# Agricultural-Robotics-Bonn/pagnerf

Hardware: AMD Instinct MI355X
Metric: rays/sec (train step) on BUP20-shape scene (higher is better)
Workload: dtype bf16

## Files before the change

include/pagnerf_hip.h:

```cpp
#ifndef PAGNERF_HIP_H
#define PAGNERF_HIP_H

#include <stdint.h>

#ifdef __cplusplus
extern "C" {
#endif

#define PAG_ABI_VERSION 14

enum { PAG_F32 = 0, PAG_F16 = 1, PAG_BF16 = 2 };
enum { PAG_OK = 0, PAG_ERR_ARG = -1, PAG_ERR_LAUNCH = -2, PAG_ERR_UNSUPPORTED = -3 };
enum { PAG_ACT_NONE = 0, PAG_ACT_SIGMOID = 1, PAG_ACT_SOFTMAX = 2 };
enum { PAG_MLP_MFMA_BF16 = 0, PAG_MLP_FP32 = 1 };
enum { PAG_BG_BLACK = 0, PAG_BG_WHITE = 1 };
enum { PAG_LAYOUT_STRIDED = 0, PAG_LAYOUT_XCD8 = 1 };
enum { PAG_ENC_HALF_COORDS = 1 };
#define PAG_MAX_LEVELS 32
#define PAG_MAX_FEATS 64

int pag_abi_version(void);
const char *pag_last_error_string(void);


// ... 75 lines not shown
    const float *weights;
    const float *alpha;
    float *out;
    int64_t n_samples;
} pag_head_composite_args;
int pag_mlp_fwd(const pag_mlp_fwd_args *args, int64_t M, void *stream);
int pag_mlp_fwd_pair_supported(const pag_mlp_fwd_args *args, const pag_mlp_fwd_args *pair);
int pag_mlp_fwd_composite_supported(const pag_mlp_fwd_args *args, int64_t M);
int pag_mlp_fwd_producer_supported(const pag_mlp_fwd_args *args, const pag_mlp_fwd_args *producer, int64_t M);

typedef struct pag_mlp_bwd_args {
    const void *grad_out; const void *out; int out_dtype; int out_act;
    int k1; int in_dim; int n_layers; int out_dim;
    int x1_layout; int x1_levels; int x1_feats;
    const float *W[3];
    const void *hidden_save[2];
    void *dz[3];
    void *dx1; int dx1_dtype;
    int mode;
    const float *g_ray; const float *g_scale; const int32_t *g_index;
    const float *softmax_stats; const float *b_last;
    int dx1_accumulate;
    const float *dx1_col0_add;
    const float *dx1_col0_gate;
    const float *g_ray_scale;
    const void *x1; int x1_dtype; const float *x2; int k2p; const int32_t *x2_index;
    float *wgrad_workspace; int64_t wgrad_workspace_bytes;
    float *dW[3]; float *db[3];
    const float *b[3];
    const struct pag_mlp_bwd_args *pair;
    float *dz0_slots;
} pag_mlp_bwd_args;
int pag_mlp_bwd(const pag_mlp_bwd_args *args, int64_t M, void *stream);
int64_t pag_mlp_dz0_slots_bytes(int64_t M, int64_t R);
int pag_mlp_dz0_slots_sum(const int64_t *pack_start, int64_t R, const float *slots, float *out, void *stream);
int pag_mlp_bwd_fused_supported(const pag_mlp_bwd_args *args);
#define PAG_MLP_FUSED_WIDE_MAX_M ((int64_t)1 << 24)
int64_t pag_mlp_bwd_fused_workspace_bytes(const pag_mlp_bwd_args *args, int64_t M);
int pag_mlp_bwd_pair_supported(const pag_mlp_bwd_args *args, const pag_mlp_bwd_args *pair);

int pag_affine_xcd8_fwd(const void *x, int64_t M, int x_levels, int x_feats, const float *W, const float *b, int n_out, int in_dim,
                        float *out, void *stream);
int pag_affine_xcd8_bwd_dx(const float *grad_out, int64_t M, int x_levels, int x_feats, const float *W, int n_out, int in_dim, void *dx,
                           void *stream);

int pag_head_composite_fwd(const int64_t *pack_start, const int32_t *ray_of_pack, int64_t P,
                           const void *hidden, const float *W_last, const float *b_last, int out_dim,
                           const float *softmax_stats, const float *weights, const float *alpha,
                           float *out, int64_t n_samples, void *stream);

int pag_mlp_wgrad_blocks(int64_t M);
int pag_mlp_wgrad(const void *dz, int dz_cols, int n_out, const void *a1, int a1_dtype,
                  int a1_layout, int k1, const float *a2, int k2p, const int32_t *a2_index, int n_in,
                  float *slabs, int n_blocks, int64_t M, void *stream);

int pag_mlp_wgrad_finish(const float *slabs, int n_blocks, int n_out, int n_in, int a1_layout,
                         int a1_levels, int a1_feats, float *dW, float *db, void *stream);

typedef struct pag_wgrad_layer {
    const void *dz;
    int dz_cols, n_out;
    const void *a1;
    int a1_dtype, a1_layout, k1;
    const float *a2;
    int k2p;
    const int32_t *a2_index;
// ... 399 lines not shown
```

pagnerf_amd/_lib.py:

```python
import ctypes
import os

import torch

from . import build as _build

F32, F16, BF16 = 0, 1, 2
I32, I64 = 3, 4
ACT_NONE, ACT_SIGMOID, ACT_SOFTMAX = 0, 1, 2
MLP_MFMA_BF16, MLP_FP32 = 0, 1
BG_BLACK, BG_WHITE = 0, 1
LAYOUT_STRIDED, LAYOUT_XCD8 = 0, 1
ENC_HALF_COORDS = 1
ABI_VERSION = 14
MLP_FUSED_WIDE_MAX_M = 1 << 24

_DT = {torch.float32: F32, torch.float16: F16, torch.bfloat16: BF16}

c_i64, c_i32, c_u32, c_f32, c_vp = ctypes.c_int64, ctypes.c_int, ctypes.c_uint32, ctypes.c_float, ctypes.c_void_p
c_fp = ctypes.POINTER(ctypes.c_float)
c_ip = ctypes.POINTER(ctypes.c_int)


class HeadCompositeArgs(ctypes.Structure):
# ... 16 lines not shown
                ("softmax_stats", c_vp), ("x1_col0_relu", c_vp), ("pair", ctypes.POINTER(MlpFwdArgs)),
                ("composite", ctypes.POINTER(HeadCompositeArgs)), ("x1_producer", ctypes.POINTER(MlpFwdArgs))]


class WgradLayer(ctypes.Structure):
    _fields_ = [("dz", c_vp), ("dz_cols", c_i32), ("n_out", c_i32),
                ("a1", c_vp), ("a1_dtype", c_i32), ("a1_layout", c_i32), ("k1", c_i32),
                ("a2", c_vp), ("k2p", c_i32), ("a2_index", c_vp), ("n_in", c_i32),
                ("slabs", c_vp), ("n_blocks", c_i32), ("a1_levels", c_i32), ("a1_feats", c_i32),
                ("dW", c_vp), ("db", c_vp)]


class MlpBwdArgs(ctypes.Structure):
    pass


MlpBwdArgs._fields_ = [("grad_out", c_vp), ("out", c_vp), ("out_dtype", c_i32), ("out_act", c_i32),
                ("k1", c_i32), ("in_dim", c_i32), ("n_layers", c_i32), ("out_dim", c_i32),
                ("x1_layout", c_i32), ("x1_levels", c_i32), ("x1_feats", c_i32),
                ("W", c_vp * 3),
                ("hidden_save", c_vp * 2),
                ("dz", c_vp * 3),
                ("dx1", c_vp), ("dx1_dtype", c_i32),
                ("mode", c_i32),
                ("g_ray", c_vp), ("g_scale", c_vp), ("g_index", c_vp),
                ("softmax_stats", c_vp), ("b_last", c_vp), ("dx1_accumulate", c_i32), ("dx1_col0_add", c_vp),
                ("dx1_col0_gate", c_vp), ("g_ray_scale", c_vp),
                ("x1", c_vp), ("x1_dtype", c_i32), ("x2", c_vp), ("k2p", c_i32), ("x2_index", c_vp),
                ("wgrad_workspace", c_vp), ("wgrad_workspace_bytes", c_i64),
                ("dW", c_vp * 3), ("db", c_vp * 3), ("b", c_vp * 3),
                ("pair", ctypes.POINTER(MlpBwdArgs)), ("dz0_slots", c_vp)]


class DeepMlpArgs(ctypes.Structure):
    _fields_ = [("coords", c_vp), ("ray_d", c_vp), ("hidden", c_i32), ("num_classes", c_i32), ("channels", c_i32), ("save", c_i32),
                ("W", c_vp * 14), ("b", c_vp * 14), ("density", c_vp), ("rgb", c_vp), ("semantics", c_vp),
                ("workspace", c_vp), ("workspace_bytes", c_i64),
                ("g_density", c_vp), ("g_rgb", c_vp), ("g_semantics", c_vp), ("dW", c_vp * 14), ("db", c_vp * 14),
                ("bwd_workspace", c_vp), ("bwd_workspace_bytes", c_i64)]


MLP128_MAX_M = 1 << 26
MLP128_BATCH, MLP128_MAX_GRID = 256, 256


class Mlp128FwdArgs(ctypes.Structure):
    _fields_ = [("x1", c_vp), ("x1_dtype", c_i32), ("k1", c_i32), ("x1_layout", c_i32), ("x1_levels", c_i32), ("x1_feats", c_i32),
                ("x2", c_vp), ("k2p", c_i32), ("x2_index", c_vp),
                ("in_dim", c_i32), ("n_hidden", c_i32), ("hidden", c_i32), ("out_dim", c_i32),
                ("W", c_vp * 4), ("b", c_vp * 4), ("out_act", c_i32), ("out", c_vp), ("out_dtype", c_i32),
                ("workspace", c_vp), ("workspace_bytes", c_i64)]


class Mlp128BwdArgs(ctypes.Structure):
    _fields_ = [("grad_out", c_vp), ("out", c_vp), ("out_dtype", c_i32), ("out_act", c_i32),
                ("k1", c_i32), ("k2p", c_i32), ("in_dim", c_i32), ("n_hidden", c_i32), ("hidden", c_i32), ("out_dim", c_i32),
                ("x1_layout", c_i32), ("x1_levels", c_i32), ("x1_feats", c_i32),
                ("W", c_vp * 4), ("workspace", c_vp), ("workspace_bytes", c_i64), ("bwd_workspace", c_vp), ("bwd_workspace_bytes", c_i64),
                ("dx1", c_vp), ("dx1_dtype", c_i32), ("dx1_accumulate", c_i32), ("dW", c_vp * 4), ("db", c_vp * 4)]


class VmArgs(ctypes.Structure):
    _fields_ = [("density_plane", c_vp * 3), ("density_line", c_vp * 3), ("app_plane", c_vp * 3), ("app_line", c_vp * 3), ("basis", c_vp),
                ("density_n_comp", c_i32), ("app_n_comp", c_i32), ("app_dim", c_i32), ("res", c_i32),
                ("xyz", c_vp), ("sigma", c_vp), ("app", c_vp), ("g_sigma", c_vp), ("g_app", c_vp),
                ("g_density_plane", c_vp * 3), ("g_density_line", c_vp * 3), ("g_app_plane", c_vp * 3), ("g_app_line", c_vp * 3), ("g_basis", c_vp),
# ... 18 lines not shown
    _fields_ = [("verts", c_vp), ("part_vert_begin", c_vp), ("point_begin", c_vp), ("part_key_begin", c_vp), ("part_key_count", c_vp), ("keys", c_vp),
                ("ann_part_begin", c_vp), ("ann_label", c_vp), ("ann_cover", c_vp), ("cand", c_vp), ("frame_ann_begin", c_vp), ("frame_labelled", c_vp),
                ("n_verts", c_i32), ("n_parts", c_i32), ("n_anns", c_i32), ("n_cand", c_i32), ("B", c_i32), ("max_part_keys", c_i32)]


class Bup20PrepareArgs(ctypes.Structure):
    _fields_ = [("img", c_vp), ("depth", c_vp), ("sem", c_vp), ("inst", c_vp), ("sem_conf", c_vp), ("inst_conf", c_vp), ("counts", c_vp),
                ("B", c_i32), ("H0", c_i32), ("W0", c_i32), ("C0", c_i32), ("mip", c_i32), ("bg", c_i32), ("n_ids", c_i32),
                ("view_offset", c_i64), ("V", c_i64), ("imgs", c_vp), ("masks", c_vp), ("depths", c_vp), ("semantics_pred", c_vp),
                ("instance_pred", c_vp), ("sem_conf_out", c_vp), ("inst_conf_out", c_vp)]


COCO_MAX_PART_KEYS = 4096

VIS_PICTURES, VIS_LABELS, VIS_MAX_ID = 15, 6, 1023


class VisArgs(ctypes.Structure):
    _fields_ = [("H", c_i32), ("W", c_i32), ("rgb", c_vp), ("rgb_is_u8", c_i32), ("rgb_stride", c_i32), ("gt", c_vp), ("gt_stride", c_i32), ("phase", c_i32),
                ("depth", c_vp), ("labels", c_vp * VIS_LABELS), ("label_bytes", c_i32 * VIS_LABELS), ("conf", c_vp * 2), ("table", c_vp),
                ("max_id", c_i32), ("box_width", c_i32), ("blend_keep", c_f32), ("blend_alpha", c_f32), ("overlay_keep", c_f32), ("overlay_alpha", c_f32),
                ("conf_min", c_f32), ("conf_max", c_f32), ("workspace", c_vp), ("workspace_bytes", c_i64), ("out", c_vp * VIS_PICTURES)]


_SIGS = {
    "pag_abi_version": (c_i32, []),
    "pag_last_error_string": (ctypes.c_char_p, []),
    "pag_encode_bwd_workspace_bytes": (c_i64, [c_i64, c_i32, c_i32, c_i32, c_i64]),
    "pag_mlp_fwd": (c_i32, [ctypes.POINTER(MlpFwdArgs), c_i64, c_vp]),
    "pag_mlp_fwd_pair_supported": (c_i32, [ctypes.POINTER(MlpFwdArgs), ctypes.POINTER(MlpFwdArgs)]),
    "pag_mlp_fwd_composite_supported": (c_i32, [ctypes.POINTER(MlpFwdArgs), c_i64]),
    "pag_mlp_fwd_producer_supported": (c_i32, [ctypes.POINTER(MlpFwdArgs), ctypes.POINTER(MlpFwdArgs), c_i64]),
    "pag_mlp_bwd": (c_i32, [ctypes.POINTER(MlpBwdArgs), c_i64, c_vp]),
    "pag_mlp_bwd_fused_supported": (c_i32, [ctypes.POINTER(MlpBwdArgs)]),
    "pag_mlp_bwd_fused_workspace_bytes": (c_i64, [ctypes.POINTER(MlpBwdArgs), c_i64]),
    "pag_mlp_bwd_pair_supported": (c_i32, [ctypes.POINTER(MlpBwdArgs), ctypes.POINTER(MlpBwdArgs)]),
    "pag_head_composite_fwd": (c_i32, [c_vp, c_vp, c_i64, c_vp, c_vp, c_vp, c_i32, c_vp, c_vp, c_vp, c_vp, c_i64, c_vp]),
    "pag_mlp_wgrad_blocks": (c_i32, [c_i64]),
    "pag_mlp_wgrad_batch": (c_i32, [ctypes.POINTER(WgradLayer), c_i32, c_i64, c_vp]),
    "pag_mlp_wgrad_finish": (c_i32, [c_vp, c_i32, c_i32, c_i32, c_i32, c_i32, c_i32, c_vp, c_vp, c_vp]),
    "pag_mlp_wgrad": (c_i32, [c_vp, c_i32, c_i32, c_vp, c_i32, c_i32, c_i32, c_vp, c_i32, c_vp, c_i32, c_vp, c_i32, c_i64, c_vp]),
    "pag_raymarch_count": (c_i32, [c_vp, c_vp, c_i64, c_i32, c_vp, c_vp, c_f32, c_f32, c_vp, c_i32, c_vp, c_vp]),
    "pag_pack_offsets": (c_i32, [c_vp, c_i64, c_vp, c_vp, c_vp]),
    "pag_pad_packed": (c_i32, [c_vp, c_i64, c_i64, c_i32, c_vp, c_vp, c_vp, c_vp, c_vp, c_vp, c_vp, c_vp, c_vp, c_vp]),
    "pag_view_embed": (c_i32, [c_vp, c_i64, c_i32, c_i32, c_vp, c_vp]),
    "pag_raymarch_pack": (c_i32, [c_vp, c_vp, c_i64, c_i32, c_vp, c_vp, c_f32, c_f32, c_vp, c_i32, c_vp, c_vp, c_vp, c_vp, c_vp, c_vp, c_vp, c_vp, c_vp]),
    "pag_raymarch_voxel_count": (c_i32, [c_vp, c_vp, c_i64, c_i32, c_f32, c_f32, c_vp, c_vp, c_i32, c_f32, c_vp, c_vp]),
    "pag_raymarch_voxel_pack": (c_i32, [c_vp, c_vp, c_i64, c_i32, c_f32, c_f32, c_vp, c_vp, c_i32, c_f32, c_vp, c_vp, c_vp, c_vp, c_vp, c_vp, c_vp,
                                        c_vp, c_vp, c_vp]),
    "pag_raymarch_voxel_nugget_capacity": (c_i64, [c_i32]),
    "pag_raymarch_voxel_count_nuggets": (c_i32, [c_vp, c_vp, c_i64, c_i32, c_f32, c_f32, c_vp, c_vp, c_i32, c_f32, c_vp, c_vp, c_vp, c_vp]),
    "pag_raymarch_voxel_pack_nuggets": (c_i32, [c_vp, c_vp, c_i64, c_i32, c_vp, c_vp, c_vp, c_i32, c_vp, c_vp, c_vp, c_vp, c_vp, c_vp, c_vp, c_vp, c_vp]),
    "pag_ray_sample_grad": (c_i32, [c_vp, c_vp, c_i64, c_vp, c_vp, c_vp, c_vp]),
    "pag_affine_xcd8_fwd": (c_i32, [c_vp, c_i64, c_i32, c_i32, c_vp, c_vp, c_i32, c_i32, c_vp, c_vp]),
    "pag_affine_xcd8_bwd_dx": (c_i32, [c_vp, c_i64, c_i32, c_i32, c_vp, c_i32, c_i32, c_vp, c_vp]),
    "pag_occupancy_coarse_bytes": (c_i64, [c_i32]),
    "pag_occupancy_coarse": (c_i32, [c_vp, c_i32, c_vp, c_vp]),
    "pag_occupancy_update": (c_i32, [c_vp, c_i64, c_vp, c_vp, c_i64, c_f32, c_f32, c_vp]),
    "pag_label_sums": (c_i32, [c_vp, c_i32, c_i64, c_i64, c_i32, c_i32, c_vp, c_vp, c_vp, c_i32, c_vp, c_vp, c_vp]),
    "pag_assign_cost": (c_i32, [c_vp, c_i32, c_i64, c_i64, c_i64, c_i32, c_i32, c_vp, c_i32, c_vp, c_vp, c_vp, c_vp, c_vp, c_vp, ctypes.c_float, ctypes.c_float, c_i32,
                                c_vp, c_vp, c_vp, c_vp]),
    "pag_sparse_rows_mask": (c_i32, [c_vp, c_i32, c_i64, c_i32, c_vp, c_vp]),
    "pag_sparse_rows_plan": (c_i32, [c_vp, c_i32, c_i64, c_vp, c_vp, c_vp, c_vp]),
    "pag_sparse_rows_pack": (c_i32, [c_vp, c_i32, c_i64, c_i32, c_vp, c_vp, c_vp, c_vp, c_vp, c_vp]),
    "pag_sparse_rows_unpack": (c_i32, [c_vp, c_i32, c_i64, c_i32, c_vp, c_vp, c_vp, c_vp, c_vp, c_vp]),
    "pag_assign_solve": (c_i32, [c_vp, c_i32, c_i32, c_i32, c_vp, c_vp, c_vp, c_vp, c_vp]),
# ... 163 lines not shown
```

pagnerf_amd/build.py:

```python
import concurrent.futures
import hashlib
import os
import subprocess
import sys

HERE = os.path.dirname(os.path.abspath(__file__))
CSRC = os.path.join(HERE, "csrc")
LIBDIR = os.path.join(HERE, "lib")
LIB = os.path.join(LIBDIR, "libpagnerf_hip.so")
ARCH = "gfx950"

COMMON = ["--offload-arch=" + ARCH, "-O3", "-fPIC", "-std=c++17", "-munsafe-fp-atomics", "-Wno-unused-value"]
MLP = ["-mllvm", "-amdgpu-mfma-vgpr-form=1"]
SOURCES = {
    "mlp.hip": MLP,
    "mlp_deep.hip": MLP,
    "mlp_h128.hip": MLP,
    "encode.hip": ["-ffp-contract=off"],
    "mlp_wgrad.hip": MLP,
    "render.hip": ["-ffp-contract=off"],
    "mlp_affine.hip": MLP,
    "api.cpp": ["-x", "hip"],
    "assign.hip": ["-ffp-contract=off"],
    "loss.hip": ["-ffp-contract=off"],
    "optim.hip": ["-ffp-contract=off"],
    "pose.hip": ["-ffp-contract=off"],
    "regularizer.hip": ["-ffp-contract=off"],
    "supcon.hip": ["-ffp-contract=off"],
    "cluster.hip": ["-ffp-contract=off"],
    "panoptic.hip": ["-ffp-contract=off"],
    "map.hip": ["-ffp-contract=off"],
    "voxelmap.hip": ["-ffp-contract=off"],
    "vm.hip": ["-ffp-contract=off"],
    "triplanar.hip": ["-ffp-contract=off"],
    "sparse.hip": [],
    "sample.hip": [],
    "visualize.hip": ["-ffp-contract=off"],
    "prepare.hip": ["-ffp-contract=off"],
    "bup20.hip": ["-ffp-contract=off"],
}


def _jobs():
    n = min(16, os.cpu_count() or 4)
    try:
        n = min(n, int(os.environ.get("MAX_JOBS", "")))
    except ValueError:
        pass
    return max(1, n)


def _hipcc():
    for c in (os.environ.get("HIPCC"), "/opt/rocm/bin/hipcc", "hipcc"):
        if c and (os.path.isabs(c) and os.path.exists(c) or not os.path.isabs(c)):
# ... 68 lines not shown
```

pagnerf_amd/csrc/mlp.hip:

```cpp
#include "mlp_common.h"
#include "mlp_lds.h"

namespace {

struct FwdParams {
    const void *x1;
    const float *x2;
    const int32_t *x2_index;
    int k1, k2p, in_dim, in_pad, out_dim, act;
    const float *W[3];
    const float *b[3];
    void *out;
    void *hsave[2];
    int64_t M;
    int grp_L, grp_F;
    float *stats;
    float *col0_relu;
    const float *W2[2];
    const float *b2[2];
    void *out2;
    int out2_dim;
};

struct BwdParams {
    const void *grad_out;
    const float *g_ray;
    const float *g_scale;
    const float *g_ray_scale;
    const int32_t *g_index;
    const void *out;
    int k1, in_dim, in_pad, out_dim, act;
    const float *W[3];
    const void *hsave[2];
    void *dz[3];
    void *dx1;
    int64_t M;
    int grp_L, grp_F;
    const float *stats;
    const float *b_last;
    int dx1_acc;
    const float *dx_col0;
    const float *dx_col0_gate;
    const void *x1;
    const float *x2;
    const int32_t *x2_index;
    int k2p;
    float *slabs[3];
    const float *b[3];
    float *dz0_slots;
};

constexpr int STAGE_BATCH = 8;
__device__ void stage_weight(bf16_t *dst, int stride, int rows_pad, int cols_pad, const float *W, int n_out, int n_in,
                             bool permute, int grp_L = 0, int grp_F = 0) {
    const int total = rows_pad * cols_pad, step = (int)blockDim.x, last = n_out * n_in - 1;
    for (int e0 = threadIdx.x; e0 < total; e0 += STAGE_BATCH * step) {
        float v[STAGE_BATCH];
        int at[STAGE_BATCH];
#pragma unroll
        for (int k = 0; k < STAGE_BATCH; ++k) {
            const int e = e0 + k * step;
            const int o = udiv_uniform(e, cols_pad), a = e - o * cols_pad;
            const int col = grp_L ? grp_col(a, grp_L, grp_F) : a;
            const bool ok = e < total && o < n_out && col >= 0 && col < n_in;
            at[k] = e < total ? o * stride + (permute ? swap23(a) : a) : -1;
            v[k] = W[min(max(o * n_in + col, 0), last)];
            v[k] = ok ? v[k] : 0.0f;
        }
#pragma unroll
        for (int k = 0; k < STAGE_BATCH; ++k)
            if (at[k] >= 0) dst[at[k]] = (bf16_t)v[k];
    }
}
__device__ void stage_weight_t(bf16_t *dst, int stride, int rows_pad, int cols_pad, const float *W, int n_out, int n_in,
                               int grp_L = 0, int grp_F = 0) {
    const int total = rows_pad * cols_pad, step = (int)blockDim.x, last = n_out * n_in - 1;
    for (int e0 = threadIdx.x; e0 < total; e0 += STAGE_BATCH * step) {
        float v[STAGE_BATCH];
        int at[STAGE_BATCH];
#pragma unroll
        for (int k = 0; k < STAGE_BATCH; ++k) {
            const int e = e0 + k * step;
// ... 4 lines not shown
            v[k] = W[min(max(o * n_in + col, 0), last)];
            v[k] = ok ? v[k] : 0.0f;
        }
#pragma unroll
        for (int k = 0; k < STAGE_BATCH; ++k)
            if (at[k] >= 0) dst[at[k]] = (bf16_t)v[k];
    }
}

__device__ void stage_weight_both(bf16_t *dst_s, int stride_s, bool permute_s, bf16_t *dst_t, int stride_t, int out_pad, int in_pad, const float *W,
                                  int n_out, int n_in, int grp_L = 0, int grp_F = 0) {
    const int total = out_pad * in_pad, step = (int)blockDim.x, last = n_out * n_in - 1;
    for (int e0 = threadIdx.x; e0 < total; e0 += STAGE_BATCH * step) {
        float v[STAGE_BATCH];
        int as[STAGE_BATCH], at[STAGE_BATCH];
#pragma unroll
        for (int k = 0; k < STAGE_BATCH; ++k) {
            const int e = e0 + k * step;
            const int o = udiv_uniform(e, in_pad), a = e - o * in_pad;
            const int col = grp_L ? grp_col(a, grp_L, grp_F) : a;
            const bool ok = e < total && o < n_out && col >= 0 && col < n_in;
            as[k] = e < total ? o * stride_s + (permute_s ? swap23(a) : a) : -1;
            at[k] = a * stride_t + swap23(o);
            v[k] = W[min(max(o * n_in + col, 0), last)];
            v[k] = ok ? v[k] : 0.0f;
        }
#pragma unroll
        for (int k = 0; k < STAGE_BATCH; ++k)
            if (as[k] >= 0) {
                dst_s[as[k]] = (bf16_t)v[k];
                dst_t[at[k]] = (bf16_t)v[k];
            }
    }
}

__device__ __forceinline__ void pack_block(const f32x16 &acc, bf16x8 &lo, bf16x8 &hi) {
#pragma unroll
    for (int j = 0; j < 8; ++j) {
        lo[j] = (bf16_t)acc[j];
        hi[j] = (bf16_t)acc[8 + j];
    }
}

template <typename T>
__device__ __forceinline__ void store_block_full(T *row_ptr, int ch_base, int h, const f32x16 &acc);

template <typename T>
__device__ __forceinline__ void store_block(T *row_ptr, int ch_base, int h, const f32x16 &acc, int n_valid, bool vec_ok) {
    if (vec_ok && ch_base + 32 <= n_valid) {
        store_block_full(row_ptr, ch_base, h, acc);
    } else if (vec_ok) {
#pragma unroll
        for (int g = 0; g < 4; ++g) {
            const int c0 = ch_base + 8 * g + 4 * h;
            if (c0 < n_valid) {
                if constexpr (sizeof(T) == 4) {
                    f32x4 v = {acc[4 * g], acc[4 * g + 1], acc[4 * g + 2], acc[4 * g + 3]};
                    *reinterpret_cast<f32x4 *>(row_ptr + c0) = v;
                } else {
                    bf16x4 v = {(bf16_t)acc[4 * g], (bf16_t)acc[4 * g + 1], (bf16_t)acc[4 * g + 2], (bf16_t)acc[4 * g + 3]};
                    *reinterpret_cast<bf16x4 *>(row_ptr + c0) = v;
                }
            }
        }
    } else {
#pragma unroll
// ... 674 lines not shown
        } else {
            float mx = -INFINITY;
#pragma unroll
            for (int j = 0; j < 4; ++j)
                if (4 * h + j < p.out_dim) mx = fmaxf(mx, o[j]);
            mx = fmaxf(mx, __shfl_xor(mx, 32));
            const float mxs = mx * LOG2E;
            float e[4], sum = 0.0f;
#pragma unroll
            for (int j = 0; j < 4; ++j) {
                e[j] = (4 * h + j < p.out_dim) ? __builtin_amdgcn_exp2f(fmaf(o[j], LOG2E, -mxs)) : 0.0f;
                sum += e[j];
            }
            sum += __shfl_xor(sum, 32);
            const float inv = 1.0f / sum;
#pragma unroll
            for (int j = 0; j < 4; ++j) {
                const bf16_t y = (bf16_t)(e[j] * inv);
                __builtin_amdgcn_raw_buffer_store_b16(__builtin_bit_cast(unsigned short, y), rs_out, ooff[j] + obase, 0, 0);
            }
        }
    }
}

constexpr int CD_WAVES = 2;
__global__ __launch_bounds__(256, CD_WAVES) void mlp_fwd_density_colour(FwdParams pd, FwdParams pc) {
    extern __shared__ __attribute__((aligned(16))) unsigned char smem[];
    constexpr float LOG2E = 1.4426950408889634f;
    constexpr DensityColourLds L{};
    bf16_t *W0d = lds_at<bf16_t>(smem, L.W0d), *WLd = lds_at<bf16_t>(smem, L.WLd);
    bf16_t *W0c = lds_at<bf16_t>(smem, L.W0c), *W1c = lds_at<bf16_t>(smem, L.W1c), *WLc = lds_at<bf16_t>(smem, L.WLc);
    float *b0d = lds_at<float>(smem, L.b0d), *bLd = lds_at<float>(smem, L.bLd);
    float *b0c = lds_at<float>(smem, L.b0c), *b1c = lds_at<float>(smem, L.b1c), *bLc = lds_at<float>(smem, L.bLc);
    stage_weight(W0d, RS, 64, 64, pd.W[0], HID, pd.in_dim, false, pd.grp_L, pd.grp_F);
    stage_weight(WLd, RS, 32, 64, pd.W[1], pd.out_dim, HID, true);
    stage_weight(W0c, RS, 64, 64, pc.W[0], HID, pc.in_dim, false);
    stage_weight(W1c, RS, 64, 64, pc.W[1], HID, HID, true);
    stage_weight(WLc, RS, 32, 64, pc.W[2], pc.out_dim, HID, true);
    for (int e = threadIdx.x; e < 64; e += blockDim.x) {
        b0d[e] = pd.b[0][e];
        b0c[e] = pc.b[0][e];
        b1c[e] = pc.b[1][e];
    }
    for (int e = threadIdx.x; e < 32; e += blockDim.x) {
        bLd[e] = e < pd.out_dim ? pd.b[1][e] : 0.0f;
        bLc[e] = e < pc.out_dim ? pc.b[2][e] : 0.0f;
    }
    __syncthreads();

    const int lane = threadIdx.x & 63, wave = threadIdx.x >> 6;
    const int r = lane & 31, h = lane >> 5;
    const int64_t M = pd.M, ntiles = (M + 31) / 32;
    const int64_t tile_step = (int64_t)gridDim.x * 4;
    const auto rs_x = __builtin_amdgcn_make_buffer_rsrc(const_cast<void *>(pd.x1), 0, (int)(M * 128), 0x00020000);
    const auto rs_xi = __builtin_amdgcn_make_buffer_rsrc(const_cast<int32_t *>(pc.x2_index), 0, (int)(M * 4), 0x00020000);
    const auto rs_od = __builtin_amdgcn_make_buffer_rsrc(pd.out, 0, (int)(M * pd.out_dim * 2), 0x00020000);
    const auto rs_oc = __builtin_amdgcn_make_buffer_rsrc(pc.out, 0, (int)(M * pc.out_dim * 4), 0x00020000);
    const auto rs_c0 = __builtin_amdgcn_make_buffer_rsrc(pc.col0_relu, 0, (int)(M * 4), 0x00020000);
    unsigned xoff[4], ooff_d[4], ooff_c[4];
#pragma unroll
    for (int s = 0; s < 4; ++s) xoff[s] = (unsigned)(((int64_t)(2 * s + h) * M + r) * 16);
#pragma unroll
    for (int g = 0; g < 4; ++g) {
        ooff_d[g] = (8 * g + 4 * h < pd.out_dim) ? (unsigned)((r * pd.out_dim + 8 * g + 4 * h) * 2) : BUF_OOB;
        ooff_c[g] = (4 * h + g < pc.out_dim) ? (unsigned)((r * pc.out_dim + 4 * h + g) * 4) : BUF_OOB;
    }
    const unsigned c0off = h == 0 ? (unsigned)(r * 4) : BUF_OOB;
    auto row_live = [&](int64_t tile) __attribute__((always_inline)) { return tile * 32 + r < M; };
    auto load_x = [&](int64_t tile, int ray, bf16x8 (&xf)[4], bf16x8 (&pe)[2]) __attribute__((always_inline)) {
        const unsigned base = row_live(tile) ? (unsigned)(tile * 32) * 16u : BUF_OOB;
#pragma unroll
// ... 24 lines not shown
        hidden_layer_pinned<4>(W0d, b0d, xb, r, h, acc);
        relu_pack(acc, hb);
        out_block_pinned(WLd, bLd, 0, hb, r, h, o);
        typedef bf16_t bf16x2 __attribute__((ext_vector_type(2)));
        unsigned dw[8];
#pragma unroll
        for (int k = 0; k < 8; ++k) dw[k] = __builtin_bit_cast(unsigned, bf16x2{(bf16_t)o[2 * k], (bf16_t)o[2 * k + 1]});
        const unsigned obase_d = live ? row0 * (unsigned)(pd.out_dim * 2) : BUF_OOB_ROW;
#pragma unroll
        for (int g = 0; g < 4; ++g) __builtin_amdgcn_raw_buffer_store_b64(u32x2{dw[2 * g], dw[2 * g + 1]}, rs_od, ooff_d[g] + obase_d, 0, 0);
        {
            const auto s02 = __builtin_amdgcn_permlane32_swap(dw[0], dw[2], false, false);
            const auto s13 = __builtin_amdgcn_permlane32_swap(dw[1], dw[3], false, false);
            const u32x4 v = {s02[0], s13[0], s02[1], s13[1]};
            xc[0] = __builtin_bit_cast(bf16x8, v);
        }
        __builtin_amdgcn_raw_buffer_store_b32(__builtin_bit_cast(unsigned, fmaxf((float)xc[0][0], 0.0f)), rs_c0, live ? c0off + row0 * 4 : BUF_OOB, 0, 0);
        hidden_layer_pinned<3>(W0c, b0c, xc, r, h, acc);
        relu_pack(acc, hb);
        hidden_layer_pinned<4>(W1c, b1c, hb, r, h, acc);
        relu_pack(acc, hb);
        out_block_pinned(WLc, bLc, 0, hb, r, h, o);
        const unsigned obase_c = live ? row0 * (unsigned)(pc.out_dim * 4) : BUF_OOB_ROW;
#pragma unroll
        for (int j = 0; j < 4; ++j) {
            const float y = __builtin_amdgcn_rcpf(1.0f + __builtin_amdgcn_exp2f(-LOG2E * o[j]));
            __builtin_amdgcn_raw_buffer_store_b32(__builtin_bit_cast(unsigned, y), rs_oc, ooff_c[j] + obase_c, 0, 0);
        }
    }
}

constexpr int WIDE_FWD_PAIR_THREADS = 1024;
constexpr int wide_fwd_waves(bool pair) { return (pair ? WIDE_FWD_PAIR_THREADS : 256) / 64; }
template <bool SAVE0, bool PAIR>
__global__ __launch_bounds__(PAIR ? WIDE_FWD_PAIR_THREADS : 256, PAIR ? 1 : 2) void mlp_fwd_wide_stats(FwdParams p) {
    extern __shared__ __attribute__((aligned(16))) unsigned char smem[];
    constexpr int OB = 7;
    constexpr float LOG2E = 1.4426950408889634f;
    const int NW = blockDim.x >> 6;
    constexpr FwdLds L(3, OB, wide_fwd_waves(PAIR), PAIR);
    bf16_t *W0s = lds_at<bf16_t>(smem, L.W0), *W1s = lds_at<bf16_t>(smem, L.W1);
    bf16_t *WLs = lds_at<bf16_t>(smem, L.WL);
    bf16_t *W0s2 = lds_at<bf16_t>(smem, L.W0p), *WLs2 = lds_at<bf16_t>(smem, L.WLp);
    float *b0s = lds_at<float>(smem, L.b0), *b1s = lds_at<float>(smem, L.b1), *bLs = lds_at<float>(smem, L.bL);
    float *b0s2 = lds_at<float>(smem, L.b0p), *bLs2 = lds_at<float>(smem, L.bLp);
    bf16_t *stg = lds_at<bf16_t>(smem, L.stg) + (threadIdx.x >> 6) * (L.stg_stride / 2);
    stage_weight(W0s, RS, 64, 64, p.W[0], HID, p.in_dim, false, p.grp_L, p.grp_F);
    stage_weight(W1s, RS, 64, 64, p.W[1], HID, HID, true);
    stage_weight(WLs, RS, OB * 32, 64, p.W[2], p.out_dim, HID, true);
    if constexpr (PAIR) {
        stage_weight(W0s2, RS, 64, 64, p.W2[0], HID, p.in_dim, false, p.grp_L, p.grp_F);
        stage_weight(WLs2, RS, 32, 64, p.W2[1], p.out2_dim, HID, true);
        for (int e = threadIdx.x; e < 64; e += blockDim.x) b0s2[e] = p.b2[0][e];
        for (int e = threadIdx.x; e < 32; e += blockDim.x) bLs2[e] = e < p.out2_dim ? p.b2[1][e] : 0.0f;
    }
    for (int e = threadIdx.x; e < 64; e += blockDim.x) {
        b0s[e] = p.b[0][e];
        b1s[e] = p.b[1][e];
    }
    for (int e = threadIdx.x; e < OB * 32; e += blockDim.x) bLs[e] = e < p.out_dim ? p.b[2][e] : -1e30f;
    __syncthreads();

    const int lane = threadIdx.x & 63, wave = threadIdx.x >> 6;
    const int r = lane & 31, h = lane >> 5;
    const int64_t M = p.M, ntiles = (M + 31) / 32;
    const int64_t tile_step = (int64_t)gridDim.x * NW;
    const auto rs_x1 = __builtin_amdgcn_make_buffer_rsrc(const_cast<void *>(p.x1), 0, (int)(M * 128), 0x00020000);
    const auto rs_st = __builtin_amdgcn_make_buffer_rsrc(p.stats, 0, (int)(M * 8), 0x00020000);
    const auto rs_o2 = __builtin_amdgcn_make_buffer_rsrc(PAIR ? p.out2 : nullptr, 0, (int)(M * (PAIR ? p.out2_dim : 0) * 2), 0x00020000);
    unsigned ooff2[4];
#pragma unroll
    for (int j = 0; j < 4; ++j) ooff2[j] = (PAIR && 4 * h + j < p.out2_dim) ? (unsigned)((r * p.out2_dim + 4 * h + j) * 2) : BUF_OOB;
    const auto rs_h0 = __builtin_amdgcn_make_buffer_rsrc(SAVE0 ? p.hsave[0] : nullptr, 0, (int)(M * HID * 2), 0x00020000);
    const auto rs_h1 = __builtin_amdgcn_make_buffer_rsrc(p.hsave[1], 0, (int)(M * HID * 2), 0x00020000);
    unsigned xoff[4];
#pragma unroll
    for (int s = 0; s < 4; ++s) xoff[s] = (unsigned)(((int64_t)(2 * s + h) * M + r) * 16);
    const unsigned soff = h == 0 ? (unsigned)(r * 8) : BUF_OOB;
    auto row_live = [&](int64_t tile) __attribute__((always_inline)) { return tile * 32 + r < M; };
    auto load_x = [&](int64_t tile, bf16x8 (&xf)[4]) __attribute__((always_inline)) {
        const unsigned base = row_live(tile) ? (unsigned)(tile * 32) * 16u : BUF_OOB;
#pragma unroll
        for (int s = 0; s < 4; ++s) xf[s] = __builtin_bit_cast(bf16x8, __builtin_amdgcn_raw_buffer_load_b128(rs_x1, xoff[s] + base, 0, 0));
    };
    int64_t tile = (int64_t)blockIdx.x * NW + wave;
// ... 392 lines not shown
                        if (p.dx_col0 && mb == 0 && h == 0 && (!p.dx_col0_gate || p.dx_col0_gate[m] > 0.0f)) acc[0][0] += p.dx_col0[m];
                        store_block(dx + m * p.k1, 32 * mb, h, acc[mb], p.k1, true);
                    }
                    if (live && p.grp_L) {
                        bf16_t *dg = reinterpret_cast<bf16_t *>(p.dx1);
#pragma unroll
                        for (int g = 0; g < 4; ++g) {
                            bf16x4 *dst = reinterpret_cast<bf16x4 *>(dg + ((int64_t)(4 * mb + g) * p.M + m) * 8 + 4 * h);
                            if (p.dx1_acc) {
#pragma unroll
                                for (int j = 0; j < 4; ++j) acc[mb][4 * g + j] += (float)oldx[mb][g][j];
                            }
                            bf16x4 v = {(bf16_t)acc[mb][4 * g], (bf16_t)acc[mb][4 * g + 1], (bf16_t)acc[mb][4 * g + 2], (bf16_t)acc[mb][4 * g + 3]};
                            *dst = v;
                        }
                    }
                }
            }
        }
    }
}

constexpr int FUSED_WAVES = 1;
template <int NL, int KIND, bool DXACC, int OBL = 1 , int DZ0 = 0 >
__global__ __launch_bounds__(256, FUSED_WAVES) void mlp_bwd_fused(BwdParams p) {
    static_assert(OBL == 1 || KIND == 0, "a 64-wide output layer exists for the dense-gradient form only");
    constexpr bool GRP = KIND != 1;
    extern __shared__ __attribute__((aligned(16))) unsigned char smem[];
    constexpr FusedLds L(NL, OBL, DZ0);
    constexpr int RSL = L.rsl;
    bf16_t *WLt = lds_at<bf16_t>(smem, L.WLt);
    bf16_t *W1t = lds_at<bf16_t>(smem, L.W1t);
    bf16_t *W0t = lds_at<bf16_t>(smem, L.W0t);
    stage_weight_t(WLt, RSL, 64, OBL * 32, p.W[NL - 1], p.out_dim, HID);
    bf16_t *W0s = lds_at<bf16_t>(smem, L.W0s);
    bf16_t *W1s = lds_at<bf16_t>(smem, L.W1s);
    float *b0s = lds_at<float>(smem, L.b0), *b1s = lds_at<float>(smem, L.b1);
    stage_weight_both(W0s, RS, false, W0t, RS, 64, 64, p.W[0], HID, p.in_dim, p.grp_L, p.grp_F);
    if (NL == 3) stage_weight_both(W1s, RS, true, W1t, RS, 64, 64, p.W[1], HID, HID);
    for (int e = threadIdx.x; e < 64; e += blockDim.x) {
        b0s[e] = p.b[0][e];
        b1s[e] = NL == 3 ? p.b[1][e] : 0.0f;
    }
    const int wtile = (threadIdx.x >> 6) * L.tile_stride;
    bf16_t *Tx = lds_at<bf16_t>(smem, L.Tx + wtile), *Th0 = lds_at<bf16_t>(smem, L.Th0 + wtile), *Th1 = lds_at<bf16_t>(smem, L.Th1 + wtile), *Tz = lds_at<bf16_t>(smem, L.Tz + wtile);
    __syncthreads();

    const int lane = threadIdx.x & 63, wave = threadIdx.x >> 6;
    const int r = lane & 31, h = lane >> 5;
    const int64_t M = p.M, ntiles = (M + 31) / 32, nfull = M / 32;
    const int64_t tile_step = (int64_t)gridDim.x * 4;
    const bf16_t *x1b = reinterpret_cast<const bf16_t *>(p.x1);
    const int32_t *ridx = KIND == 1 ? p.x2_index : p.g_index;
    const auto rs_dz0 = __builtin_amdgcn_make_buffer_rsrc(DZ0 == 1 ? p.dz[0] : nullptr, 0, (int)(DZ0 == 1 ? M * HID * 2 : 0), 0x00020000);
    auto store_dz0 = [&](int64_t tile) __attribute__((always_inline)) {
        if constexpr (DZ0 == 1) {
            typedef unsigned int u32x2 __attribute__((ext_vector_type(2)));
            typedef unsigned int u32x4 __attribute__((ext_vector_type(4)));
            const unsigned voff = (unsigned)(tile * (32 * HID * 2)) + (unsigned)((lane >> 3) * (HID * 2) + (lane & 7) * 16);
#pragma unroll
            for (int k = 0; k < 4; ++k) {
                const int rowl = k * 8 + (lane >> 3), ch = (lane & 7) * 2;
                const u32x2 lo = *reinterpret_cast<const u32x2 *>(Tz + tw_off(rowl, ch));
                const u32x2 hi = *reinterpret_cast<const u32x2 *>(Tz + tw_off(rowl, ch + 1));
                __builtin_amdgcn_raw_buffer_store_b128(u32x4{lo[0], lo[1], hi[0], hi[1]}, rs_dz0, voff + k * (8 * HID * 2), 0, 0);
            }
        }
    };

    int *lray_s = lds_at<int>(smem, L.rays) + (threadIdx.x >> 6) * (L.rays_stride / 4), *rid_s = lray_s + 32;
    int ray_c = 0;
    unsigned heads_c = 0u;
// ... 349 lines not shown
        for (int q4 = 0; q4 < 4; ++q4) sv[q4] = (reinterpret_cast<const f32x4 *>(red) + (bb * 4 + q4) * 64 + lane)[0];
        auto srcv = [&](int q) __attribute__((always_inline)) { return sv[q >> 2][q & 3]; };
        if constexpr (bb < BM) {
            float *sl = p.slabs[NL - 1] + (int64_t)blockIdx.x * (OBL * 32) * WG_SLAB_COLS;
#pragma unroll
            for (int q = 0; q < 16; ++q) sl[(32 * (bb >> 1) + rho(q, h)) * WG_SLAB_COLS + 32 * (bb & 1) + r] = srcv(q);
        } else if constexpr (bb < B0) {
            float *sl = p.slabs[1] + (int64_t)blockIdx.x * 64 * WG_SLAB_COLS;
#pragma unroll
            for (int q = 0; q < 16; ++q) sl[(32 * ((bb - BM) >> 1) + rho(q, h)) * WG_SLAB_COLS + 32 * ((bb - BM) & 1) + r] = srcv(q);
        } else if constexpr (bb < NBLK - 1) {
            constexpr int ob = (bb - B0) >> 1, ib = (bb - B0) & 1;
            float *sl = p.slabs[0] + (int64_t)blockIdx.x * 64 * WG_SLAB_COLS;
#pragma unroll
            for (int q = 0; q < 16; ++q) {
                const float v = srcv(q);
                sl[(32 * ob + rho(q, h)) * WG_SLAB_COLS + 32 * ib + r] = v;
                if (ib == 1 && r == 31) sl[(32 * ob + rho(q, h)) * WG_SLAB_COLS + 64] = v;
            }
        } else {
#pragma unroll
            for (int q = 0; q < 16; ++q) {
                const float v = srcv(q);
                if (r < OBL) p.slabs[NL - 1][((int64_t)blockIdx.x * (OBL * 32) + 32 * r + rho(q, h)) * WG_SLAB_COLS + 64] = v;
                if (NL == 3 && r >= OBL && r < OBL + 2) p.slabs[1][((int64_t)blockIdx.x * 64 + 32 * (r - OBL) + rho(q, h)) * WG_SLAB_COLS + 64] = v;
            }
        }
    });
}

struct PairParams {
    BwdParams i, s;
};
__global__ __launch_bounds__(256, 1) void mlp_bwd_pair(PairParams pp) {
    const BwdParams &pi = pp.i, &ps = pp.s;
    extern __shared__ __attribute__((aligned(16))) unsigned char smem[];
    constexpr PairLds L{};
    constexpr int RSLI = L.rslI, RSLS = L.rslS;
    bf16_t *WLtI = lds_at<bf16_t>(smem, L.WLtI);
    bf16_t *W0tI = lds_at<bf16_t>(smem, L.W0tI);
    bf16_t *W0sI = lds_at<bf16_t>(smem, L.W0sI);
    bf16_t *WLtS = lds_at<bf16_t>(smem, L.WLtS);
    bf16_t *W0tS = lds_at<bf16_t>(smem, L.W0tS), *W0sS = lds_at<bf16_t>(smem, L.W0sS);
    float *b0I = lds_at<float>(smem, L.b0I), *b0S = lds_at<float>(smem, L.b0S);
    stage_weight_t(WLtI, RSLI, 64, 64, pi.W[1], pi.out_dim, HID);
    stage_weight_both(W0sI, RS, false, W0tI, RS, 64, 64, pi.W[0], HID, pi.in_dim, pi.grp_L, pi.grp_F);
    stage_weight_t(WLtS, RSLS, 64, 32, ps.W[1], ps.out_dim, HID);
    stage_weight_both(W0sS, RS, false, W0tS, RS, 64, 64, ps.W[0], HID, ps.in_dim, ps.grp_L, ps.grp_F);
    for (int e = threadIdx.x; e < 64; e += blockDim.x) {
        b0I[e] = pi.b[0][e];
        b0S[e] = ps.b[0][e];
    }
    const int wtile = (threadIdx.x >> 6) * L.tile_stride;
    bf16_t *Tx = lds_at<bf16_t>(smem, L.Tx + wtile), *ThI = lds_at<bf16_t>(smem, L.ThI + wtile), *ThS = lds_at<bf16_t>(smem, L.ThS + wtile), *Tz = lds_at<bf16_t>(smem, L.Tz + wtile);
    __syncthreads();

    const int lane = threadIdx.x & 63, wave = threadIdx.x >> 6;
    const int r = lane & 31, h = lane >> 5;
    const int64_t M = pi.M, ntiles = (M + 31) / 32, nfull = M / 32;
    const int64_t tile_step = (int64_t)gridDim.x * 4;
    const bf16_t *x1b = reinterpret_cast<const bf16_t *>(pi.x1);
    const int32_t *ridx = ps.g_index;

    bf16x8 xn[4];
    bf16x4 gz[2][4];
    float gs[4], gy[4], gsc = 0.0f;
    int ray1 = 0, ray2 = 0;
    auto row_of = [&](int64_t tile) __attribute__((always_inline)) { return min(min(tile, ntiles - 1) * 32 + r, M - 1); };
    auto prefetch = [&](int64_t tile_raw, int ray) __attribute__((always_inline)) {
        const int64_t tile = min(tile_raw, ntiles - 1);
        const int64_t m = min(tile * 32 + r, M - 1);
#pragma unroll
        for (int s = 0; s < 4; ++s) xn[s] = load8(x1b + ((int64_t)(2 * s + h) * M + m) * 8);
        const bf16_t *gop = reinterpret_cast<const bf16_t *>(pi.grad_out) + m * HID;
#pragma unroll
        for (int ob = 0; ob < 2; ++ob)
#pragma unroll
            for (int g = 0; g < 4; ++g) gz[ob][g] = *reinterpret_cast<const bf16x4 *>(gop + 32 * ob + 8 * g + 4 * h);
        gsc = __fmul_rn(ps.g_scale[m], ps.g_ray_scale[ray]);
        const float *grow = ps.g_ray + (int64_t)ray * ps.out_dim;
        const bf16_t *yop = reinterpret_cast<const bf16_t *>(ps.out) + m * ps.out_dim;
// ... 246 lines not shown
            float *sl = (S ? ps.slabs[0] : pi.slabs[0]) + (int64_t)blockIdx.x * 64 * WG_SLAB_COLS;
#pragma unroll
            for (int q = 0; q < 16; ++q) {
                const float v = srcv(q);
                sl[(32 * ob + rho(q, h)) * WG_SLAB_COLS + 32 * ib + r] = v;
                if (ib == 1 && r == 31) sl[(32 * ob + rho(q, h)) * WG_SLAB_COLS + 64] = v;
            }
        } else {
#pragma unroll
            for (int q = 0; q < 16; ++q) {
                const float v = srcv(q);
                if (r < 2) pi.slabs[1][((int64_t)blockIdx.x * 64 + 32 * r + rho(q, h)) * WG_SLAB_COLS + 64] = v;
                if (r == 2) ps.slabs[1][((int64_t)blockIdx.x * 32 + rho(q, h)) * WG_SLAB_COLS + 64] = v;
            }
        }
    });
}

template <int OB>
__global__ __launch_bounds__((OB + 1) * 64) void mlp_bwd_wide_blocks(BwdParams p) {
    extern __shared__ __attribute__((aligned(16))) unsigned char smem[];
    constexpr WideBlocksLds L(OB);
    constexpr int RSL = L.rsl;
    constexpr float LOG2E = 1.4426950408889634f;
    bf16_t *WLt = lds_at<bf16_t>(smem, L.WLt);
    bf16_t *WLs = lds_at<bf16_t>(smem, L.WLs);
    float *bLs = lds_at<float>(smem, L.bL);
    bf16_t *Th = lds_at<bf16_t>(smem, L.Th);
    bf16_t *Tp = lds_at<bf16_t>(smem, L.Tp);
    bf16_t *TzAll = lds_at<bf16_t>(smem, L.Tz);
    float *grow = lds_at<float>(smem, L.grow);
    float *dotbuf = lds_at<float>(smem, L.dot);
    bf16x8 *zbuf = lds_at<bf16x8>(smem, L.zbuf);
    stage_weight_both(WLs, RS, true, WLt, RSL, OB * 32, 64, p.W[0], p.out_dim, HID);
    for (int e = threadIdx.x; e < OB * 32; e += blockDim.x) bLs[e] = e < p.out_dim ? p.b_last[e] : -1e30f;
    for (int e = threadIdx.x; e < 2 * OB * 64; e += blockDim.x) dotbuf[e] = 0.0f;
    for (int e = threadIdx.x; e < 2 * OB * 2 * 64 * 4; e += blockDim.x) reinterpret_cast<float *>(zbuf)[e] = 0.0f;
    for (int e = threadIdx.x; e < 4 * TW_ELEMS / 2; e += blockDim.x) reinterpret_cast<float *>(Th)[e] = 0.0f;
    __syncthreads();

    const int lane = threadIdx.x & 63, wave = threadIdx.x >> 6;
    const int r = lane & 31, h = lane >> 5;
    const int64_t M = p.M, ntiles = (M + 31) / 32;
    const int64_t tile_step = gridDim.x;
    const bf16_t *hsrc = reinterpret_cast<const bf16_t *>(p.hsave[0]);
    bf16_t *dzh = reinterpret_cast<bf16_t *>(p.dz[0]);
    const bool is_block = wave < OB;
    const int ob = is_block ? wave : 0;
    bf16_t *Tz = TzAll + ob * (L.Tz_stride / 2);
    auto row_of = [&](int64_t tile) __attribute__((always_inline)) { return min(min(tile, ntiles - 1) * 32 + r, M - 1); };
    const auto rs_h = __builtin_amdgcn_make_buffer_rsrc(const_cast<bf16_t *>(hsrc), 0, (int)min(M * HID * 2, (int64_t)0xffffffffll), 0x00020000);
    const auto rs_i = __builtin_amdgcn_make_buffer_rsrc(const_cast<int32_t *>(p.g_index), 0, (int)min(M * 4, (int64_t)0xffffffffll), 0x00020000);
    const auto rs_d = __builtin_amdgcn_make_buffer_rsrc(dzh, 0, (int)min((ntiles + 1) * 32 * HID * 2, (int64_t)0xffffffffll), 0x00020000);
    const int voff_tile = (lane >> 3) * (HID * 2) + (lane & 7) * 16;
    auto load_rows = [&](float (&v)[4 * WB_RMAX], int ray_first, int ray_last) __attribute__((always_inline)) {
#pragma unroll
        for (int k = 0; k < WB_RMAX; ++k) {
            const int rr = min(ray_first + k, ray_last);
            const auto rs_row = __builtin_amdgcn_make_buffer_rsrc(const_cast<float *>(p.g_ray) + (int64_t)rr * p.out_dim, 0, p.out_dim * 4, 0x00020000);
#pragma unroll
            for (int j = 0; j < 4; ++j) v[4 * k + j] = __builtin_bit_cast(float, __builtin_amdgcn_raw_buffer_load_b32(rs_row, lane * 4, 256 * j, 0));
        }
    };
    auto put_rows = [&](float *dst, const float (&v)[4 * WB_RMAX]) __attribute__((always_inline)) {
#pragma unroll
        for (int k = 0; k < 4 * WB_RMAX; ++k) dst[(k >> 2) * WR_RS + 64 * (k & 3) + lane] = v[k];
    };
// ... 586 lines not shown
            if (ob < OB) {
                float v[16];
#pragma unroll
                for (int q = 0; q < 16; ++q) v[q] = acc[ob][q];
                PAG_DPP_ADD16(v, "row_shr:1 row_mask:0xf bank_mask:0xf bound_ctrl:1");
                PAG_DPP_ADD16(v, "row_shr:2 row_mask:0xf bank_mask:0xf bound_ctrl:1");
                PAG_DPP_ADD16(v, "row_shr:4 row_mask:0xf bank_mask:0xf bound_ctrl:1");
                PAG_DPP_ADD16(v, "row_shr:8 row_mask:0xf bank_mask:0xf bound_ctrl:1");
                PAG_DPP_ADD16(v, "row_bcast:15 row_mask:0xa bank_mask:0xf");
                if (r == 31) {
#pragma unroll
                    for (int q = 0; q < 16; ++q) red[wave * OB * 32 + 32 * ob + rho(q, h)] = v[q];
                }
            }
        }
        const int32_t ray = p.ray_of_pack[pk];
        const float al = p.alpha[ray];
        if (pw) {
            for (int c = lane; c < p.out_dim; c += 64) p.out[(int64_t)ray * p.out_dim + c] = al * red[wave * OB * 32 + c];
        } else {
            __syncthreads();
            for (int c = threadIdx.x; c < p.out_dim; c += blockDim.x)
                p.out[(int64_t)ray * p.out_dim + c] = al * (red[c] + red[OB * 32 + c] + red[2 * OB * 32 + c] + red[3 * OB * 32 + c]);
            __syncthreads();
        }
    }
}

template <bool PAIR>
__global__ __launch_bounds__(256, 1) void head_fwd_once_kernel(FwdParams p, HeadCompParams c) {
    extern __shared__ __attribute__((aligned(16))) unsigned char smem[];
    constexpr int OB = 7;
    constexpr float LOG2E = 1.4426950408889634f;
    constexpr FwdLds L(3, OB, 4, PAIR, true);
    bf16_t *W0s = lds_at<bf16_t>(smem, L.W0), *W1s = lds_at<bf16_t>(smem, L.W1);
    bf16_t *WLs = lds_at<bf16_t>(smem, L.WL);
    bf16_t *W0s2 = lds_at<bf16_t>(smem, L.W0p), *WLs2 = lds_at<bf16_t>(smem, L.WLp);
    float *b0s = lds_at<float>(smem, L.b0), *b1s = lds_at<float>(smem, L.b1), *bLs = lds_at<float>(smem, L.bL);
    float *b0s2 = lds_at<float>(smem, L.b0p), *bLs2 = lds_at<float>(smem, L.bLp);
    float *red = lds_at<float>(smem, L.red);
    bf16_t *stg = lds_at<bf16_t>(smem, L.stg) + (threadIdx.x >> 6) * (L.stg_stride / 2);
    stage_weight(W0s, RS, 64, 64, p.W[0], HID, p.in_dim, false, p.grp_L, p.grp_F);
    stage_weight(W1s, RS, 64, 64, p.W[1], HID, HID, true);
    stage_weight(WLs, RS, OB * 32, 64, p.W[2], p.out_dim, HID, true);
    if constexpr (PAIR) {
        stage_weight(W0s2, RS, 64, 64, p.W2[0], HID, p.in_dim, false, p.grp_L, p.grp_F);
        stage_weight(WLs2, RS, 32, 64, p.W2[1], p.out2_dim, HID, true);
        for (int e = threadIdx.x; e < 64; e += blockDim.x) b0s2[e] = p.b2[0][e];
        for (int e = threadIdx.x; e < 32; e += blockDim.x) bLs2[e] = e < p.out2_dim ? p.b2[1][e] : 0.0f;
    }
    for (int e = threadIdx.x; e < 64; e += blockDim.x) {
        b0s[e] = p.b[0][e];
        b1s[e] = p.b[1][e];
    }
    for (int e = threadIdx.x; e < OB * 32; e += blockDim.x) bLs[e] = e < p.out_dim ? p.b[2][e] : -1e30f;
    __syncthreads();

    const int lane = threadIdx.x & 63, wave = threadIdx.x >> 6;
    int r = lane & 31, h = lane >> 5;
    const int64_t M = p.M;
    const auto rs_x1 = __builtin_amdgcn_make_buffer_rsrc(const_cast<void *>(p.x1), 0, (int)(M * 128), 0x00020000);
    const auto rs_st = __builtin_amdgcn_make_buffer_rsrc(p.stats, 0, (int)(M * 8), 0x00020000);
    const auto rs_o2 = __builtin_amdgcn_make_buffer_rsrc(PAIR ? p.out2 : nullptr, 0, (int)(M * (PAIR ? p.out2_dim : 0) * 2), 0x00020000);
    const auto rs_h1 = __builtin_amdgcn_make_buffer_rsrc(p.hsave[1], 0, (int)(M * HID * 2), 0x00020000);
    const int pw = c.per_wave;
    const int64_t pk0 = pw ? (int64_t)blockIdx.x * 4 + wave : (int64_t)blockIdx.x, pk_step = pw ? (int64_t)gridDim.x * 4 : (int64_t)gridDim.x;
    const int t_first = pw ? 0 : wave, t_step = pw ? 1 : 4;
    bf16x8 xn[4];
    float wn = 0.0f;
    const auto rs_w = __builtin_amdgcn_make_buffer_rsrc(const_cast<float *>(c.weights), 0, (int)(M * 4), 0x00020000);
    unsigned xoff[4];
#pragma unroll
    for (int s = 0; s < 4; ++s) xoff[s] = (unsigned)(((int64_t)(2 * s + h) * M + r) * 16);
    auto fetch = [&](int64_t fbeg, int64_t fend, int64_t t) __attribute__((always_inline)) {
        const int64_t base = fbeg + 32 * t;
        const bool lv = base + r < fend;
        const unsigned off = lv ? (unsigned)base * 16u : BUF_OOB;
#pragma unroll
        for (int s = 0; s < 4; ++s) xn[s] = __builtin_bit_cast(bf16x8, __builtin_amdgcn_raw_buffer_load_b128(rs_x1, xoff[s] + off, 0, 0));
        wn = __builtin_bit_cast(float, __builtin_amdgcn_raw_buffer_load_b32(rs_w, lv ? (unsigned)(base + r) * 4u : BUF_OOB, 0, 0));
// ... 275 lines not shown
            }
        }
        __syncthreads();
        if (l > 0) {
            const float *hv = reinterpret_cast<const float *>(p.hsave[l - 1]) + mc * HID;
#pragma unroll
            for (int k = 0; k < 64; ++k) {
                float v = (live && hv[k] > 0.0f) ? acc[k] : 0.0f;
                zs[k * PT + t] = v;
                if (live) reinterpret_cast<float *>(p.dz[l - 1])[m * HID + k] = v;
            }
            n_out = HID;
        } else if (live) {
            DxT *dx = reinterpret_cast<DxT *>(p.dx1) + m * p.k1;
#pragma unroll
            for (int k = 0; k < 64; ++k)
                if (k < p.k1) pag_st(dx + k, acc[k]);
        }
    }
}

inline unsigned mlp_grid(int64_t M) {
    int64_t tiles = (M + 31) / 32;
    int64_t blocks = (tiles + 3) / 4;
    int64_t cap = 256 * 6;
    return (unsigned)(blocks < cap ? (blocks > 0 ? blocks : 1) : cap);
}

bool is_wide_stats_head(const pag_mlp_fwd_args *a) {
    return a->mode == PAG_MLP_MFMA_BF16 && a->x1_dtype == PAG_BF16 && a->x1_layout == PAG_LAYOUT_XCD8 && !a->out && a->n_layers == 3 && a->softmax_stats &&
           a->out_act == PAG_ACT_SOFTMAX && a->out_dim > 192 && a->out_dim <= 224 && a->hidden_save[1];
}

void set_pair_head(FwdParams &p, const pag_mlp_fwd_args *b) {
    p.W2[0] = b->W[0];
    p.W2[1] = b->W[1];
    p.b2[0] = b->b[0];
    p.b2[1] = b->b[1];
    p.out2 = b->out;
    p.out2_dim = b->out_dim;
}

template <typename X1T, typename OutT, int NL>
void launch_fwd_mfma_nl(const FwdParams &p, hipStream_t st) {
    const dim3 grid(mlp_grid(p.M)), block(256);
    const int OB = (p.out_dim + 31) / 32;
    const size_t lds = FwdLds(NL, OB).bytes;
    if (OB <= 1) hipLaunchKernelGGL((mlp_fwd_mfma<X1T, OutT, NL, 1>), grid, block, lds, st, p);
    else if (OB <= 2) hipLaunchKernelGGL((mlp_fwd_mfma<X1T, OutT, NL, 2>), grid, block, lds, st, p);
    else if (OB <= 4) hipLaunchKernelGGL((mlp_fwd_mfma<X1T, OutT, NL, 4>), grid, block, lds, st, p);
    else hipLaunchKernelGGL((mlp_fwd_mfma<X1T, OutT, NL, 7>), grid, block, lds, st, p);
}
template <typename X1T, typename OutT>
void launch_fwd_mfma(const FwdParams &p, int n_layers, hipStream_t st) {
    if (n_layers == 2) launch_fwd_mfma_nl<X1T, OutT, 2>(p, st);
    else launch_fwd_mfma_nl<X1T, OutT, 3>(p, st);
}

constexpr int FAST_FWD_GRID_CAP = 768;
template <int KIND>
void launch_fwd_fast(const FwdParams &p, int n_layers, bool save, hipStream_t st) {
    const dim3 grid(std::min<unsigned>(mlp_grid(p.M), FAST_FWD_GRID_CAP)), block(256);
    const size_t lds = FwdLds(n_layers, 1).bytes;
    if (n_layers == 2 && save) hipLaunchKernelGGL((mlp_fwd_fast<2, KIND, true>), grid, block, lds, st, p);
    else if (n_layers == 2) hipLaunchKernelGGL((mlp_fwd_fast<2, KIND, false>), grid, block, lds, st, p);
    else if (save) hipLaunchKernelGGL((mlp_fwd_fast<3, KIND, true>), grid, block, lds, st, p);
    else hipLaunchKernelGGL((mlp_fwd_fast<3, KIND, false>), grid, block, lds, st, p);
}
template <bool SAVE0, bool PAIR>
void launch_fwd_wide_stats(const FwdParams &p, unsigned grid, hipStream_t st) {
    constexpr int NW = wide_fwd_waves(PAIR);
    raise_lds_limit<mlp_fwd_wide_stats<SAVE0, PAIR>>(LDS_MAX_BYTES);
    hipLaunchKernelGGL((mlp_fwd_wide_stats<SAVE0, PAIR>), dim3(grid), dim3(NW * 64), FwdLds(3, OB_MAX, NW, PAIR).bytes, st, p);
// ... 59 lines not shown
    hipLaunchKernelGGL((mlp_bwd_wide_mfma<DxT, NL, NW>), dim3(grid), dim3(NW * 64), lds, st, p);
}

}

extern "C" int pag_mlp_fwd_pair_supported(const pag_mlp_fwd_args *a, const pag_mlp_fwd_args *b) {
    if (!a || !b || b->pair) return 0;
    const bool wide = is_wide_stats_head(a) && !a->hidden_save[0];
    const bool narrow = b->mode == PAG_MLP_MFMA_BF16 && b->x1 == a->x1 && b->x1_dtype == PAG_BF16 && b->x1_layout == PAG_LAYOUT_XCD8 && b->x1_levels == a->x1_levels &&
                        b->x1_feats == a->x1_feats && b->in_dim == a->in_dim && b->n_layers == 2 && b->out && b->out_dtype == PAG_BF16 &&
                        b->out_act == PAG_ACT_SOFTMAX && b->out_dim >= 1 && b->out_dim <= 8 && !b->hidden_save[0] && !b->hidden_save[1] && !b->x2 &&
                        !b->x1_col0_relu && b->W[0] && b->W[1] && b->b[0] && b->b[1];
    return wide && narrow ? 1 : 0;
}

extern "C" int pag_mlp_fwd_producer_supported(const pag_mlp_fwd_args *a, const pag_mlp_fwd_args *d, int64_t M) {
    if (!a || !d || M < 1 || M > PAG_MLP_FUSED_WIDE_MAX_M) return 0;
    const bool density = d->mode == PAG_MLP_MFMA_BF16 && d->x1_dtype == PAG_BF16 && d->x1_layout == PAG_LAYOUT_XCD8 && d->k1 == 64 && !d->x2 && d->n_layers == 2 &&
                         d->out && d->out_dtype == PAG_BF16 && d->out_act == PAG_ACT_NONE && d->out_dim == 16 && !d->hidden_save[0] && !d->hidden_save[1] &&
                         !d->softmax_stats && !d->x1_col0_relu && !d->pair && !d->composite && !d->x1_producer && d->W[0] && d->W[1] && d->b[0] && d->b[1] &&
                         d->in_dim == d->x1_levels * d->x1_feats && d->x1_feats >= 1 && ((d->x1_levels + 7) / 8) * d->x1_feats <= 8;
    const bool colour = a->mode == PAG_MLP_MFMA_BF16 && a->x1_dtype == PAG_BF16 && a->x1_layout != PAG_LAYOUT_XCD8 && a->k1 == 16 && a->x1 == d->out && a->x2 &&
                        a->k2p == 32 && a->x2_index && a->in_dim <= 48 && a->n_layers == 3 && a->out && a->out_dtype == PAG_F32 && a->out_act == PAG_ACT_SIGMOID &&
                        a->out_dim <= 4 && a->x1_col0_relu && !a->hidden_save[0] && !a->hidden_save[1] && !a->pair && !a->composite;
    return density && colour ? 1 : 0;
}

extern "C" int pag_mlp_fwd_composite_supported(const pag_mlp_fwd_args *a, int64_t M) {
    if (!a || M < 1 || M > PAG_MLP_FUSED_WIDE_MAX_M) return 0;
    const bool wide = is_wide_stats_head(a) && !a->hidden_save[0];
    return wide && (!a->pair || pag_mlp_fwd_pair_supported(a, a->pair) == 1) ? 1 : 0;
}

extern "C" int pag_mlp_fwd(const pag_mlp_fwd_args *a, int64_t M, void *stream) {
    PAG_CHECK_ARG(a, "pag_mlp_fwd: args is NULL");
    PAG_CHECK_ARG(M >= 0, "pag_mlp_fwd: M < 0");
    PAG_CHECK_ARG(a->n_layers == 2 || a->n_layers == 3, "pag_mlp_fwd: n_layers %d not in {2,3}", a->n_layers);
    PAG_CHECK_ARG(a->k1 > 0 && a->k1 % 8 == 0, "pag_mlp_fwd: k1 %d must be a positive multiple of 8", a->k1);
    PAG_CHECK_ARG(a->x2 == nullptr || (a->k2p > 0 && a->k2p % 8 == 0 && a->x2_index), "pag_mlp_fwd: x2 needs k2p %% 8 == 0 and x2_index");
    const int k2p = a->x2 ? a->k2p : 0;
    PAG_CHECK_ARG(a->in_dim > 0 && a->in_dim <= a->k1 + k2p && a->in_dim <= 64 && a->k1 + k2p <= 64,
                  "pag_mlp_fwd: in_dim %d / k1+k2p %d out of range (<= 64)", a->in_dim, a->k1 + k2p);
    PAG_CHECK_ARG(a->out_dim >= 1 && a->out_dim <= 224, "pag_mlp_fwd: out_dim %d not in [1,224]", a->out_dim);
    PAG_CHECK_ARG(a->x1_dtype == PAG_F32 || a->x1_dtype == PAG_BF16, "pag_mlp_fwd: x1 dtype must be F32 or BF16");
    PAG_CHECK_ARG(a->out_dtype == PAG_F32 || a->out_dtype == PAG_BF16, "pag_mlp_fwd: out dtype must be F32 or BF16");
    PAG_CHECK_ARG(a->out_act >= PAG_ACT_NONE && a->out_act <= PAG_ACT_SOFTMAX, "pag_mlp_fwd: bad out_act %d", a->out_act);
    PAG_CHECK_ARG(a->mode == PAG_MLP_MFMA_BF16 || a->mode == PAG_MLP_FP32, "pag_mlp_fwd: bad mode %d", a->mode);
    if (M == 0) return PAG_OK;
    for (int l = 0; l < a->n_layers; ++l) PAG_CHECK_ARG(a->W[l] && a->b[l], "pag_mlp_fwd: NULL weight/bias of layer %d", l);
    PAG_CHECK_ARG(a->x1, "pag_mlp_fwd: NULL x1");
    PAG_CHECK_ARG(a->out || (a->softmax_stats && a->mode == PAG_MLP_MFMA_BF16 && a->out_dim > 64 && a->out_act == PAG_ACT_SOFTMAX),
                  "pag_mlp_fwd: NULL out (allowed only for wide softmax heads that write softmax_stats)");
    FwdParams p;
    for (int l = 0; l < 3; ++l) p.b[l] = a->b[l];
    p.x1 = a->x1;
    p.x2 = a->x2;
    p.x2_index = a->x2_index;
    p.k1 = a->k1;
    p.k2p = k2p;
    p.in_dim = a->in_dim;
    p.in_pad = ((a->k1 + k2p + 15) / 16) * 16;
    p.out_dim = a->out_dim;
    p.act = a->out_act;
    p.stats = (a->mode == PAG_MLP_MFMA_BF16 && a->out_dim > 64) ? a->softmax_stats : nullptr;
    PAG_CHECK_ARG(!a->x1_col0_relu || (a->mode == PAG_MLP_MFMA_BF16 && a->x1_dtype == PAG_BF16 && a->x1_layout != PAG_LAYOUT_XCD8 && a->out_dim <= 64),
                  "pag_mlp_fwd: x1_col0_relu needs MFMA mode, a strided bf16 x1 and out_dim <= 64");
    p.col0_relu = a->x1_col0_relu;
    p.W2[0] = p.W2[1] = p.b2[0] = p.b2[1] = nullptr;
    p.out2 = nullptr;
    p.out2_dim = 0;
    for (int l = 0; l < 3; ++l) {
        p.W[l] = l < a->n_layers ? a->W[l] : nullptr;
        p.b[l] = l < a->n_layers ? a->b[l] : nullptr;
    }
    p.out = a->out;
    p.hsave[0] = a->hidden_save[0];
    p.hsave[1] = a->n_layers == 3 ? a->hidden_save[1] : nullptr;
    p.M = M;
    p.grp_L = a->x1_layout == PAG_LAYOUT_XCD8 ? a->x1_levels : 0;
    p.grp_F = a->x1_feats;
    if (p.grp_L) {
        PAG_CHECK_ARG(a->mode == PAG_MLP_MFMA_BF16 && a->x1_dtype == PAG_BF16 && a->k1 == 64 && a->x2 == nullptr && p.grp_F >= 1 &&
                          ((p.grp_L + 7) / 8) * p.grp_F <= 8 && a->in_dim == p.grp_L * p.grp_F,
                      "pag_mlp_fwd: XCD8 input needs MFMA mode, bf16, k1 = 64, no x2 and in_dim = levels*feats");
        p.in_pad = 64;
    }
    hipStream_t st = (hipStream_t)stream;
    if (a->mode == PAG_MLP_MFMA_BF16 && a->x1_dtype == PAG_BF16 && M <= PAG_MLP_FUSED_WIDE_MAX_M) {
        const bool grp = p.grp_L > 0;
        const bool save_all = a->hidden_save[0] && (a->n_layers == 2 || a->hidden_save[1]);
        const bool save_none = !a->hidden_save[0] && !a->hidden_save[1];
        int kind = -1;
        if (grp && a->out && a->out_dtype == PAG_BF16 && a->out_act == PAG_ACT_NONE && a->out_dim % 4 == 0 && a->out_dim <= 32) kind = 0;
        else if (!grp && a->k1 == 16 && a->x2 && a->k2p == 32 && a->in_dim <= 48 && a->out && a->out_dtype == PAG_F32 && a->out_act == PAG_ACT_SIGMOID &&
                 a->out_dim <= 4 && a->x1_col0_relu)
            kind = 1;
        else if (grp && a->out && a->out_dtype == PAG_BF16 && a->out_act == PAG_ACT_SOFTMAX && a->out_dim <= 8) kind = 2;
        else if (grp && is_wide_stats_head(a)) kind = 3;
        PAG_CHECK_ARG(!a->pair || (kind == 3 && pag_mlp_fwd_pair_supported(a, a->pair) == 1), "pag_mlp_fwd: pair is not supported for these arguments (pag_mlp_fwd_pair_supported)");
        PAG_CHECK_ARG(!a->composite || kind == 3, "pag_mlp_fwd: composite rides only in the statistics-only wide softmax head (pag_mlp_fwd_composite_supported)");
        if (kind == 3) {
            if (a->pair) set_pair_head(p, a->pair);
            if (a->composite) {
                const pag_head_composite_args *hc = a->composite;
                PAG_CHECK_ARG(hc->P >= 0 && (hc->P == 0 || (hc->pack_start && hc->ray_of_pack && hc->weights && hc->alpha && hc->out)),
                              "pag_mlp_fwd: composite: NULL input/output");
                PAG_CHECK_ARG(!a->hidden_save[0] && a->hidden_save[1] && a->softmax_stats, "pag_mlp_fwd: composite needs softmax_stats and hidden_save[1] only");
                if (hc->P == 0) return PAG_OK;
                HeadCompParams c{hc->pack_start, hc->ray_of_pack, hc->P, nullptr, nullptr, nullptr, a->out_dim, nullptr, 0, hc->weights, hc->alpha, hc->out};
                c.per_wave = ((hc->n_samples > 0 && hc->n_samples < 160 * hc->P) || hc->P >= HC_PER_WAVE_P) ? 1 : 0;
                constexpr int HEAD_ONCE_GRID = 256;
                const unsigned grid = (unsigned)std::min<int64_t>(c.per_wave ? (hc->P + 3) / 4 : hc->P, HEAD_ONCE_GRID);
                if (a->pair) launch_head_fwd_once<true>(p, c, grid, st);
                else launch_head_fwd_once<false>(p, c, grid, st);
                PAG_CHECK_LAUNCH("pag_mlp_fwd (wide head, decoder + per-ray sum)");
                return PAG_OK;
            }
            if (a->pair) {
                constexpr int NWP = wide_fwd_waves(true);
                constexpr int WIDE_FWD_PAIR_GRID = 256;
                const unsigned grid = std::min<unsigned>((mlp_grid(M) * 4 + NWP - 1) / NWP, WIDE_FWD_PAIR_GRID);
                launch_fwd_wide_stats<false, true>(p, grid, st);
            } else if (a->hidden_save[0]) {
                launch_fwd_wide_stats<true, false>(p, mlp_grid(M), st);
            } else {
                launch_fwd_wide_stats<false, false>(p, mlp_grid(M), st);
            }
            PAG_CHECK_LAUNCH("pag_mlp_fwd (wide head statistics)");
            return PAG_OK;
        }
        PAG_CHECK_ARG(!a->x1_producer || (kind == 1 && pag_mlp_fwd_producer_supported(a, a->x1_producer, M) == 1),
                      "pag_mlp_fwd: x1_producer is not supported for these arguments (pag_mlp_fwd_producer_supported)");
        if (a->x1_producer) {
            const pag_mlp_fwd_args *d = a->x1_producer;
            FwdParams pd = p;
            pd.x1 = d->x1;
            pd.x2 = nullptr;
            pd.x2_index = nullptr;
            pd.k1 = 64;
            pd.k2p = 0;
            pd.in_dim = d->in_dim;
            pd.in_pad = 64;
            pd.out_dim = d->out_dim;
            pd.act = d->out_act;
            pd.stats = nullptr;
            pd.col0_relu = nullptr;
            for (int l = 0; l < 3; ++l) {
                pd.W[l] = l < 2 ? d->W[l] : nullptr;
                pd.b[l] = l < 2 ? d->b[l] : nullptr;
            }
            pd.out = d->out;
            pd.hsave[0] = pd.hsave[1] = nullptr;
            pd.grp_L = d->x1_levels;
            pd.grp_F = d->x1_feats;
            hipLaunchKernelGGL(mlp_fwd_density_colour, dim3(std::min<unsigned>(mlp_grid(M), FAST_FWD_GRID_CAP)), dim3(256), DensityColourLds{}.bytes, st, pd, p);
            PAG_CHECK_LAUNCH("pag_mlp_fwd (density + colour)");
            return PAG_OK;
        }
        if (kind >= 0 && (save_all || save_none)) {
            if (kind == 0) launch_fwd_fast<0>(p, a->n_layers, save_all, st);
            else if (kind == 1) launch_fwd_fast<1>(p, a->n_layers, save_all, st);
            else launch_fwd_fast<2>(p, a->n_layers, save_all, st);
            PAG_CHECK_LAUNCH("pag_mlp_fwd (straight-line)");
            return PAG_OK;
        }
    }
    PAG_CHECK_ARG(!a->composite, "pag_mlp_fwd: composite rides only in the straight-line wide-head launch (pag_mlp_fwd_composite_supported)");
    PAG_CHECK_ARG(!a->x1_producer, "pag_mlp_fwd: x1_producer rides only in the straight-line colour launch (pag_mlp_fwd_producer_supported)");
    PAG_CHECK_ARG(!a->pair, "pag_mlp_fwd: pair rides only in the straight-line wide-head launch (M <= %lld)", (long long)PAG_MLP_FUSED_WIDE_MAX_M);
    if (a->mode == PAG_MLP_MFMA_BF16) {
        if (a->x1_dtype == PAG_F32 && a->out_dtype == PAG_F32) launch_fwd_mfma<float, float>(p, a->n_layers, st);
        else if (a->x1_dtype == PAG_F32) launch_fwd_mfma<float, bf16_t>(p, a->n_layers, st);
        else if (a->out_dtype == PAG_F32) launch_fwd_mfma<bf16_t, float>(p, a->n_layers, st);
        else launch_fwd_mfma<bf16_t, bf16_t>(p, a->n_layers, st);
    } else {
        const size_t lds = F32Lds(64).bytes;
        dim3 grid((unsigned)((M + PT - 1) / PT)), block(PT);
        if (a->x1_dtype == PAG_F32 && a->out_dtype == PAG_F32)
            hipLaunchKernelGGL((mlp_fwd_f32<float, float>), grid, block, lds, st, p, a->n_layers);
        else if (a->x1_dtype == PAG_F32)
            hipLaunchKernelGGL((mlp_fwd_f32<float, bf16_t>), grid, block, lds, st, p, a->n_layers);
        else if (a->out_dtype == PAG_F32)
            hipLaunchKernelGGL((mlp_fwd_f32<bf16_t, float>), grid, block, lds, st, p, a->n_layers);
        else
            hipLaunchKernelGGL((mlp_fwd_f32<bf16_t, bf16_t>), grid, block, lds, st, p, a->n_layers);
    }
    PAG_CHECK_LAUNCH("pag_mlp_fwd");
// ... 60 lines not shown
        if (a->k1 != 64 || a->x1_levels < 1 || a->x1_feats < 1 || ((a->x1_levels + 7) / 8) * a->x1_feats > 8 || !xcd8_has_bias_slot(a->x1_levels, a->x1_feats)) return -1;
        if (a->x2 || a->dx1_col0_add) return -1;
        if (!rank1 && a->grad_out && a->out_dtype == PAG_BF16 && a->out_act == PAG_ACT_NONE && a->out_dim % 4 == 0 && !a->dx1_accumulate) return 0;
        if (rank1 && a->g_scale && a->g_index && a->g_ray_scale && a->out && a->out_dtype == PAG_BF16 && a->out_act == PAG_ACT_SOFTMAX &&
            a->out_dim <= 8)
            return 2;
        return -1;
    }
    if (a->k1 == 16 && a->x2 && a->k2p == 32 && a->x2_index && a->in_dim <= 48 && !rank1 && a->grad_out && a->out && a->out_dtype == PAG_F32 &&
        a->out_act == PAG_ACT_SIGMOID && a->out_dim <= 4 && a->dx1_col0_add && a->dx1_col0_gate && !a->dx1_accumulate)
        return 1;
    return -1;
}

extern "C" int pag_mlp_bwd_fused_supported(const pag_mlp_bwd_args *a) { return fused_kind(a) >= 0 ? 1 : 0; }

extern "C" int pag_mlp_bwd_pair_supported(const pag_mlp_bwd_args *a, const pag_mlp_bwd_args *b) {
    if (!a || !b || fused_kind(a) != 3 || fused_kind(b) != 2 || b->n_layers != 2) return 0;
    return (b->x1 == a->x1 && b->x1_layout == PAG_LAYOUT_XCD8 && b->x1_levels == a->x1_levels && b->x1_feats == a->x1_feats && b->in_dim == a->in_dim &&
            a->dx1 && b->dx1 == a->dx1 && b->dx1_accumulate && !a->dx1_accumulate)
               ? 1
               : 0;
}

extern "C" int64_t pag_mlp_bwd_fused_workspace_bytes(const pag_mlp_bwd_args *a, int64_t M) {
    const int kind = fused_kind(a);
    if (kind < 0 || M < 1) return 0;
    const int64_t grid = fused_grid(M);
    if (kind == 3)
        return (grid * 224 + grid * 128) * WG_SLAB_COLS * (int64_t)sizeof(float) + ((M + 31) / 32 + 1) * 32 * HID * 2;
    return grid * ((int64_t)(a->n_layers - 1) * 64 + 32) * WG_SLAB_COLS * (int64_t)sizeof(float);
}

extern "C" int pag_mlp_bwd(const pag_mlp_bwd_args *a, int64_t M, void *stream) {
    PAG_CHECK_ARG(a, "pag_mlp_bwd: args is NULL");
    PAG_CHECK_ARG(M >= 0, "pag_mlp_bwd: M < 0");
    PAG_CHECK_ARG(a->n_layers == 2 || a->n_layers == 3, "pag_mlp_bwd: n_layers %d not in {2,3}", a->n_layers);
    PAG_CHECK_ARG(a->k1 > 0 && a->k1 % 8 == 0 && a->k1 <= 64, "pag_mlp_bwd: k1 %d must be a multiple of 8 in (0,64]", a->k1);
    PAG_CHECK_ARG(a->in_dim > 0 && a->in_dim <= 64, "pag_mlp_bwd: in_dim %d out of range", a->in_dim);
    PAG_CHECK_ARG(a->out_dim >= 1 && a->out_dim <= 224, "pag_mlp_bwd: out_dim %d not in [1,224]", a->out_dim);
    PAG_CHECK_ARG(a->out_act >= PAG_ACT_NONE && a->out_act <= PAG_ACT_SOFTMAX, "pag_mlp_bwd: bad out_act %d", a->out_act);
    PAG_CHECK_ARG(a->out_act == PAG_ACT_NONE || a->out || (a->softmax_stats && a->b_last),
                  "pag_mlp_bwd: activated output (or softmax_stats + b_last) needed for sigmoid/softmax");
    PAG_CHECK_ARG(a->out_dtype == PAG_F32 || a->out_dtype == PAG_BF16, "pag_mlp_bwd: out dtype must be F32 or BF16");
    PAG_CHECK_ARG(a->dx1 == nullptr || a->dx1_dtype == PAG_F32 || a->dx1_dtype == PAG_BF16, "pag_mlp_bwd: dx1 dtype must be F32 or BF16");
    PAG_CHECK_ARG(a->mode == PAG_MLP_MFMA_BF16 || a->mode == PAG_MLP_FP32, "pag_mlp_bwd: bad mode %d", a->mode);
    if (M == 0) return PAG_OK;
    PAG_CHECK_ARG(a->grad_out || (a->g_ray && a->g_scale && a->g_index), "pag_mlp_bwd: NULL grad_out (and no rank-1 gradient)");
    PAG_CHECK_ARG(!a->g_ray || (a->mode == PAG_MLP_MFMA_BF16 && (a->out || a->softmax_stats)),
                  "pag_mlp_bwd: rank-1 gradients need MFMA mode and the saved output");
    const bool fuse = a->wgrad_workspace != nullptr;
    const int kind = fuse ? fused_kind(a) : -1;
    if (fuse) {
        PAG_CHECK_ARG(kind >= 0, "pag_mlp_bwd: this decoder shape has no fused weight-gradient kernel (pag_mlp_bwd_fused_supported)");
        PAG_CHECK_ARG(a->wgrad_workspace_bytes >= pag_mlp_bwd_fused_workspace_bytes(a, M), "pag_mlp_bwd: wgrad_workspace too small");
        for (int l = 0; l < a->n_layers; ++l) PAG_CHECK_ARG(a->dW[l] && a->db[l], "pag_mlp_bwd: NULL dW/db of layer %d", l);
        for (int l = 0; l + 1 < a->n_layers; ++l) PAG_CHECK_ARG(a->b[l], "pag_mlp_bwd: fused mode recomputes the hidden activations: NULL bias b[%d]", l);
    }
    for (int l = 0; l < a->n_layers; ++l) PAG_CHECK_ARG(a->W[l] && (fuse || a->dz[l]), "pag_mlp_bwd: NULL weight/dz of layer %d", l);
    for (int l = 0; l + 1 < a->n_layers; ++l)
        PAG_CHECK_ARG(a->hidden_save[l] || (a->wgrad_workspace && (a->out_dim <= 32 || l + 2 < a->n_layers)), "pag_mlp_bwd: NULL hidden_save[%d]", l);
    BwdParams p;
    p.g_ray = a->g_ray;
    p.g_scale = a->g_scale;
    p.g_ray_scale = a->g_ray_scale;
    p.g_index = a->g_index;
    p.grad_out = a->grad_out ? a->grad_out : (const void *)a->out;
// ... 5 lines not shown
    p.act = a->out_act;
    for (int l = 0; l < 3; ++l) {
        p.W[l] = l < a->n_layers ? a->W[l] : nullptr;
        p.dz[l] = l < a->n_layers ? a->dz[l] : nullptr;
    }
    p.hsave[0] = a->hidden_save[0];
    p.hsave[1] = a->n_layers == 3 ? a->hidden_save[1] : nullptr;
    p.dx1 = a->dx1;
    p.M = M;
    p.grp_L = a->x1_layout == PAG_LAYOUT_XCD8 ? a->x1_levels : 0;
    p.grp_F = a->x1_feats;
    if (p.grp_L)
        PAG_CHECK_ARG(a->mode == PAG_MLP_MFMA_BF16 && (a->dx1 == nullptr || a->dx1_dtype == PAG_BF16) && a->k1 == 64 &&
                          ((p.grp_L + 7) / 8) * p.grp_F <= 8 && a->in_dim == p.grp_L * p.grp_F,
                      "pag_mlp_bwd: XCD8 dx1 needs MFMA mode, bf16, k1 = 64 and in_dim = levels*feats");
    hipStream_t st = (hipStream_t)stream;
    const bool out_f32 = a->out_dtype == PAG_F32;
    const bool dx_f32 = a->dx1 == nullptr || a->dx1_dtype == PAG_F32;
    p.stats = a->softmax_stats;
    p.b_last = a->b_last;
    p.dx1_acc = a->dx1_accumulate;
    p.dx_col0 = a->dx1_col0_add;
    p.dx_col0_gate = a->dx1_col0_gate;
    PAG_CHECK_ARG(!a->dx1_col0_gate || a->dx1_col0_add, "pag_mlp_bwd: dx1_col0_gate without dx1_col0_add");
    PAG_CHECK_ARG(!a->dx1_col0_add || (a->dx1 && !p.grp_L && a->mode == PAG_MLP_MFMA_BF16 && a->out_dim <= 64),
                  "pag_mlp_bwd: dx1_col0_add needs a strided dx1, MFMA mode and out_dim <= 64");
    PAG_CHECK_ARG(!a->dx1_accumulate || (p.grp_L && a->dx1), "pag_mlp_bwd: dx1_accumulate needs an XCD8 dx1");
    for (int l = 0; l < 3; ++l) p.b[l] = a->b[l];
    p.x1 = a->x1;
    p.x2 = a->x2;
    p.x2_index = a->x2_index;
    p.k2p = a->x2 ? a->k2p : 0;
    for (int l = 0; l < 3; ++l) p.slabs[l] = nullptr;
    if (fuse && kind == 3) {
        PAG_CHECK_ARG(M <= PAG_MLP_FUSED_WIDE_MAX_M, "pag_mlp_bwd: the fused wide-head backward addresses [M,64] bf16 tensors with 32-bit byte offsets: M %lld > %lld, split the batch",
                      (long long)M, (long long)PAG_MLP_FUSED_WIDE_MAX_M);
        const unsigned grid = fused_grid(M);
        float *ws = a->wgrad_workspace;
        float *slabA = ws;
        ws += (int64_t)grid * 224 * WG_SLAB_COLS;
        float *slabB0 = ws;
        ws += (int64_t)grid * 64 * WG_SLAB_COLS;
        float *slabB1 = ws;
        ws += (int64_t)grid * 64 * WG_SLAB_COLS;
        bf16_t *dzh = reinterpret_cast<bf16_t *>(ws);
        BwdParams pa = p;
        pa.W[0] = a->W[2];
        pa.hsave[0] = a->hidden_save[1];
        pa.dz[0] = dzh;
        pa.slabs[0] = slabA;
        const pag_mlp_bwd_args *b = a->pair;
        BwdParams ps{};
        float *slabS0 = nullptr, *slabS1 = nullptr;
        if (b) {
            PAG_CHECK_ARG(b->wgrad_workspace && fused_kind(b) == 2 && b->n_layers == 2 && !b->pair, "pag_mlp_bwd: pair must be a two-layer narrow softmax head with a fused workspace");
            PAG_CHECK_ARG(b->x1 == a->x1 && b->x1_layout == PAG_LAYOUT_XCD8 && b->x1_levels == a->x1_levels && b->x1_feats == a->x1_feats && b->in_dim == a->in_dim,
                          "pag_mlp_bwd: pair must read the same XCD8 input");
            PAG_CHECK_ARG(b->dx1 == a->dx1 && b->dx1_accumulate && a->dx1 && !a->dx1_accumulate, "pag_mlp_bwd: pair must accumulate into this decoder's dx1");
            PAG_CHECK_ARG(b->wgrad_workspace_bytes >= pag_mlp_bwd_fused_workspace_bytes(b, M), "pag_mlp_bwd: pair wgrad_workspace too small");
            PAG_CHECK_ARG(b->W[0] && b->W[1] && b->b[0] && b->dW[0] && b->dW[1] && b->db[0] && b->db[1] && b->out && b->g_ray && b->g_scale && b->g_index && b->g_ray_scale,
                          "pag_mlp_bwd: pair: NULL weight / bias / gradient / saved output");
            ps.g_ray = b->g_ray;
            ps.g_scale = b->g_scale;
            ps.g_ray_scale = b->g_ray_scale;
            ps.g_index = b->g_index;
            ps.out = b->out;
            ps.grad_out = b->out;
            ps.k1 = 64;
            ps.in_dim = b->in_dim;
            ps.in_pad = 64;
            ps.out_dim = b->out_dim;
            ps.act = PAG_ACT_SOFTMAX;
            ps.W[0] = b->W[0];
            ps.W[1] = b->W[1];
            ps.b[0] = b->b[0];
            ps.M = M;
            ps.grp_L = p.grp_L;
            ps.grp_F = p.grp_F;
            ps.x1 = a->x1;
            ps.dx1 = a->dx1;
            slabS0 = b->wgrad_workspace;
            slabS1 = slabS0 + (int64_t)grid * 64 * WG_SLAB_COLS;
            ps.slabs[0] = slabS0;
            ps.slabs[1] = slabS1;
        }
        launch_bwd_wide_blocks(pa, grid, st);
        PAG_CHECK_LAUNCH("pag_mlp_bwd (fused, wide head)");
        BwdParams pb = p;
        pb.grad_out = dzh;
        pb.out = dzh;
        pb.g_ray = nullptr;
        pb.out_dim = HID;
        pb.act = PAG_ACT_NONE;
        pb.W[0] = a->W[0];
        pb.W[1] = a->W[1];
        pb.W[2] = nullptr;
        pb.b[0] = a->b[0];
        pb.b[1] = nullptr;
        pb.hsave[0] = a->hidden_save[0];
        pb.hsave[1] = nullptr;
        pb.slabs[0] = slabB0;
        pb.slabs[1] = slabB1;
        FinishBatch fb{};
        fb.p[0] = FinishParams{slabB0, (int)grid, HID, 64, a->in_dim, p.grp_L, p.grp_F, a->dW[0], a->db[0]};
        fb.p[1] = FinishParams{slabB1, (int)grid, HID, 64, HID, 0, 0, a->dW[1], a->db[1]};
        fb.p[2] = FinishParams{slabA, (int)grid, a->out_dim, 224, HID, 0, 0, a->dW[2], a->db[2]};
        int n_fin = 3;
        if (b) {
            raise_lds_limit<mlp_bwd_pair>(LDS_MAX_BYTES);
            PairParams pp{pb, ps};
            hipLaunchKernelGGL(mlp_bwd_pair, dim3(grid), dim3(256), PairLds{}.bytes, st, pp);
            PAG_CHECK_LAUNCH("pag_mlp_bwd (fused, layers below the wide head + companion head)");
            fb.p[3] = FinishParams{slabS0, (int)grid, HID, 64, b->in_dim, p.grp_L, p.grp_F, b->dW[0], b->db[0]};
            fb.p[4] = FinishParams{slabS1, (int)grid, b->out_dim, 32, HID, 0, 0, b->dW[1], b->db[1]};
            n_fin = 5;
        } else {
            launch_bwd_fused<2, 0, false, 2>(pb, grid, st);
            PAG_CHECK_LAUNCH("pag_mlp_bwd (fused, layers below the wide head)");
        }
        launch_wgrad_finish(fb, a->out_dim, n_fin, st);
        PAG_CHECK_LAUNCH("pag_mlp_bwd (fused, finish)");
        return PAG_OK;
    }
    if (fuse) {
        const unsigned grid = fused_grid(M);
        float *ws = a->wgrad_workspace;
        for (int l = 0; l < a->n_layers; ++l) {
            p.slabs[l] = ws;
            ws += (int64_t)grid * (l + 1 < a->n_layers ? 64 : 32) * WG_SLAB_COLS;
        }
        p.dz[0] = kind == 1 ? a->dz[0] : nullptr;
        p.dz0_slots = kind == 1 ? a->dz0_slots : nullptr;
        const int dz0 = kind != 1 ? 0 : (a->dz0_slots ? 2 : (a->dz[0] ? 1 : 0));
        if (a->n_layers == 2) launch_bwd_fused_kind<2>(p, kind, a->dx1_accumulate != 0, dz0, grid, st);
        else launch_bwd_fused_kind<3>(p, kind, a->dx1_accumulate != 0, dz0, grid, st);
        PAG_CHECK_LAUNCH("pag_mlp_bwd (fused)");
        FinishBatch fb{};
        int max_out = 0;
        for (int l = 0; l < a->n_layers; ++l) {
            const int n_out = l + 1 < a->n_layers ? HID : a->out_dim;
            const int n_in = l == 0 ? a->in_dim : HID;
            fb.p[l] = FinishParams{p.slabs[l], (int)grid, n_out, (n_out + 31) / 32 * 32, n_in, l == 0 ? p.grp_L : 0, p.grp_F, a->dW[l], a->db[l]};
            max_out = std::max(max_out, n_out);
        }
        launch_wgrad_finish(fb, max_out, a->n_layers, st);
        PAG_CHECK_LAUNCH("pag_mlp_bwd (fused, finish)");
        return PAG_OK;
    }
    const bool wide_rebuild = a->mode == PAG_MLP_MFMA_BF16 && a->out_dim > 64 && a->out_act == PAG_ACT_SOFTMAX && a->softmax_stats &&
                              a->b_last && !out_f32 && (a->g_ray || (a->grad_out && a->out_dim % 8 == 0));
    if (wide_rebuild) {
        if (dx_f32 && a->n_layers == 2) launch_bwd_wide_mfma<float, 2>(p, st);
        else if (dx_f32) launch_bwd_wide_mfma<float, 3>(p, st);
        else if (a->n_layers == 2) launch_bwd_wide_mfma<bf16_t, 2>(p, st);
        else launch_bwd_wide_mfma<bf16_t, 3>(p, st);
    } else if (a->mode == PAG_MLP_MFMA_BF16) {
        if (out_f32 && dx_f32) launch_bwd_mfma<float, float>(p, a->n_layers, st);
        else if (out_f32) launch_bwd_mfma<float, bf16_t>(p, a->n_layers, st);
        else if (dx_f32) launch_bwd_mfma<bf16_t, float>(p, a->n_layers, st);
        else launch_bwd_mfma<bf16_t, bf16_t>(p, a->n_layers, st);
    } else {
        if (out_f32 && dx_f32) launch_bwd_f32<float, float>(p, a->n_layers, st);
        else if (out_f32) launch_bwd_f32<float, bf16_t>(p, a->n_layers, st);
        else if (dx_f32) launch_bwd_f32<bf16_t, float>(p, a->n_layers, st);
        else launch_bwd_f32<bf16_t, bf16_t>(p, a->n_layers, st);
    }
    PAG_CHECK_LAUNCH("pag_mlp_bwd");
    return PAG_OK;
}

namespace {
__global__ __launch_bounds__(256) void dz0_slots_sum_kernel(const int64_t *__restrict__ pack_start, int64_t R, const float *__restrict__ slots, float *__restrict__ out) {
    const int lane = threadIdx.x & 63;
    const int64_t ray = (int64_t)blockIdx.x * 4 + (threadIdx.x >> 6);
    if (ray >= R) return;
    const int64_t beg = pack_start[ray], end = pack_start[ray + 1];
    float a = 0.0f;
    if (end > beg)
        for (int64_t t = beg >> 5; t <= ((end - 1) >> 5); ++t) a += slots[(t + ray) * 64 + lane];
    out[ray * 64 + lane] = a;
}
}
extern "C" int64_t pag_mlp_dz0_slots_bytes(int64_t M, int64_t R) { return (M > 0 && R > 0) ? ((M + 31) / 32 + R) * 64 * (int64_t)sizeof(float) : 0; }
extern "C" int pag_mlp_dz0_slots_sum(const int64_t *pack_start, int64_t R, const float *slots, float *out, void *stream) {
    PAG_CHECK_ARG(R >= 0, "pag_mlp_dz0_slots_sum: R < 0");
    if (R == 0) return PAG_OK;
    PAG_CHECK_ARG(pack_start && slots && out, "pag_mlp_dz0_slots_sum: NULL input/output");
    hipLaunchKernelGGL(dz0_slots_sum_kernel, dim3((unsigned)((R + 3) / 4)), dim3(256), 0, (hipStream_t)stream, pack_start, R, slots, out);
    PAG_CHECK_LAUNCH("pag_mlp_dz0_slots_sum");
    return PAG_OK;
}

extern "C" int pag_head_composite_fwd(const int64_t *pack_start, const int32_t *ray_of_pack, int64_t P, const void *hidden,
                                      const float *W_last, const float *b_last, int out_dim, const float *softmax_stats,
                                      const float *weights, const float *alpha, float *out, int64_t samples_hint, void *stream) {
    PAG_CHECK_ARG(P >= 0, "pag_head_composite_fwd: P < 0");
    PAG_CHECK_ARG(out_dim > 64 && out_dim <= 224, "pag_head_composite_fwd: out_dim %d not in (64,224]", out_dim);
    if (P == 0) return PAG_OK;
    PAG_CHECK_ARG(pack_start && ray_of_pack && hidden && W_last && b_last && softmax_stats && weights && alpha && out,
                  "pag_head_composite_fwd: NULL input/output");
    HeadCompParams p{pack_start, ray_of_pack, P, (const bf16_t *)hidden, W_last, b_last, out_dim, softmax_stats, 0, weights, alpha, out};
// ... 11 lines not shown
```

pagnerf_amd/csrc/mlp_lds.h:

```cpp
#pragma once

namespace pagmlp {

constexpr int LDS_MAX_BYTES = 160 * 1024;
constexpr int OB_MAX = 7;
constexpr int HID = 64;
constexpr int RS = 72;
constexpr int ST_RS = 72;
constexpr int ST_BYTES = 32 * ST_RS * 2;
constexpr int TW_ELEMS = 32 * 64;
constexpr int WR_RS = 256;
constexpr int WB_RMAX = 4;
constexpr int WIDE_BWD_WAVES = 8;
constexpr int PT = 128;
constexpr int WG_RS = 72;

constexpr int W64 = 64 * RS * 2, W32 = 32 * RS * 2;
constexpr int TW_BYTES = TW_ELEMS * 2;

struct FwdLds {
    int W0, W1, WL, W0p, WLp, b0, b1, bL, b0p, bLp, red, stg, stg_stride, bytes;
    constexpr FwdLds(int n_layers, int ob, int waves = 4, bool pair = false, bool ray_sums = false)
        : W0(0), W1(W0 + W64), WL(W1 + (n_layers == 3 ? W64 : 0)), W0p(WL + ob * W32), WLp(W0p + (pair ? W64 : 0)), b0(WLp + (pair ? W32 : 0)),
          b1(b0 + 64 * 4), bL(b1 + 64 * 4), b0p(bL + ob * 32 * 4), bLp(b0p + (pair ? 64 * 4 : 0)), red(bLp + (pair ? 32 * 4 : 0)),
// ... 14 lines not shown
        : rsl(obl * 32 + 8), WLt(0), W1t(WLt + 64 * rsl * 2), W0t(W1t + (n_layers == 3 ? W64 : 0)), W0s(W0t + W64), W1s(W0s + W64),
          b0(W1s + (n_layers == 3 ? W64 : 0)), b1(b0 + 64 * 4), Tx(b1 + 64 * 4), Th0(Tx + TW_BYTES), Th1(Th0 + (n_layers == 3 ? TW_BYTES : 0)), Tz(Th1 + TW_BYTES),
          tile_stride((n_layers + 1) * TW_BYTES), rays(Tx + 4 * tile_stride), rays_stride(64 * 4), bytes(rays + (dz0 == 2 ? 4 * rays_stride : 0)) {}
};
struct PairLds {
    int rslI = 72, rslS = 40, WLtI = 0, W0tI = WLtI + 64 * rslI * 2, W0sI = W0tI + W64, WLtS = W0sI + W64, W0tS = WLtS + 64 * rslS * 2, W0sS = W0tS + W64, b0I = W0sS + W64, b0S = b0I + 64 * 4,
        Tx = b0S + 64 * 4, ThI = Tx + TW_BYTES, ThS = ThI + TW_BYTES, Tz = ThS + TW_BYTES, tile_stride = 4 * TW_BYTES, bytes = Tx + 4 * tile_stride;
};
struct WideBlocksLds {
    int rsl, WLt, WLs, bL, Th, Tp, Tz, Tz_stride, grow, dot, zbuf, bytes;
    constexpr WideBlocksLds(int ob)
        : rsl(ob * 32 + 8), WLt(0), WLs(WLt + 64 * rsl * 2), bL(WLs + ob * W32), Th(bL + ob * 32 * 4), Tp(Th + 4 * TW_BYTES), Tz(Tp + TW_BYTES), Tz_stride(TW_BYTES),
          grow(Tz + ob * Tz_stride), dot(grow + 2 * WB_RMAX * WR_RS * 4), zbuf(dot + 2 * ob * 64 * 4), bytes(zbuf + 2 * ob * 2 * 64 * 16) {}
};
struct WideMfmaLds {
    int rsl, WLt, WLs, W1t, W0t, bL, stg, stg_stride, grow, grow_stride, bytes;
    constexpr WideMfmaLds(int n_layers, int ob, int waves)
        : rsl(ob * 32 + 8), WLt(0), WLs(WLt + 64 * rsl * 2), W1t(WLs + ob * W32), W0t(W1t + (n_layers == 3 ? W64 : 0)), bL(W0t + W64), stg(bL + ob * 32 * 4),
          stg_stride(ST_BYTES), grow(stg + waves * stg_stride), grow_stride(ob * 32 * 4), bytes(grow + waves * grow_stride) {}
};
struct HeadCompLds {
    int WL, bL, red, stg, stg_stride, bytes;
    constexpr HeadCompLds(int ob) : WL(0), bL(WL + ob * W32), red(bL + ob * 32 * 4), stg(red + 4 * ob * 32 * 4), stg_stride(ST_BYTES), bytes(stg + 4 * stg_stride) {}
};
struct F32Lds {
    int cols, wt, bytes;
    constexpr F32Lds(int rows) : cols(0), wt(cols + rows * PT * 4), bytes(wt + 64 * 64 * 4) {}
};
struct WgradLds {
    int Zt, At, bytes;
    constexpr WgradLds(int ob, int ib) : Zt(0), At(Zt + ob * 32 * WG_RS * 2), bytes(At + ib * 32 * WG_RS * 2) {}
};

static_assert(FwdLds(3, OB_MAX, 16, true).bytes <= LDS_MAX_BYTES && FwdLds(3, OB_MAX, 4, true, true).bytes <= LDS_MAX_BYTES, "FwdLds");
static_assert(DensityColourLds{}.bytes <= LDS_MAX_BYTES, "DensityColourLds");
static_assert(BwdLds(3, OB_MAX).bytes <= LDS_MAX_BYTES, "BwdLds");
static_assert(FusedLds(3, 1, 2).bytes <= LDS_MAX_BYTES && FusedLds(2, 2, 0).bytes <= LDS_MAX_BYTES, "FusedLds");
static_assert(PairLds{}.bytes <= LDS_MAX_BYTES, "PairLds");
static_assert(WideBlocksLds(OB_MAX).bytes <= LDS_MAX_BYTES, "WideBlocksLds");
static_assert(WideMfmaLds(3, OB_MAX, WIDE_BWD_WAVES).bytes <= LDS_MAX_BYTES, "WideMfmaLds");
static_assert(HeadCompLds(OB_MAX).bytes <= LDS_MAX_BYTES, "HeadCompLds");
static_assert(F32Lds(224).bytes <= LDS_MAX_BYTES, "F32Lds");
static_assert(WgradLds(OB_MAX, 2).bytes <= LDS_MAX_BYTES, "WgradLds");

}
```

pagnerf_amd/nef.py:

```python
import copy
import inspect
import os

import numpy as np
import torch
import torch.nn as nn
import torch.nn.functional as F

from . import _lib as L
from . import ops
from .grids import HashGridHIP, PermutoGridHIP
from .triplanar import TriplanarGridHIP

_GRIDS = {"HashGridTorch": HashGridHIP, "HashGridTinyCudaNN": HashGridHIP, "HashGrid": HashGridHIP,
          "HashGridHIP": HashGridHIP, "PermutoGrid": PermutoGridHIP, "PermutoGridHIP": PermutoGridHIP,
          "TriplanarGrid": TriplanarGridHIP, "TriplanarGridHIP": TriplanarGridHIP}


class BasicDecoder(nn.Module):

    def __init__(self, input_dim, output_dim, num_layers=1, hidden_dim=64, bias=True):
        super().__init__()
        if hidden_dim not in (64, 128) or num_layers not in ((1, 2) if hidden_dim == 64 else (1, 2, 3)):
            raise NotImplementedError("fused decoders support hidden_dim=64 (1-2 hidden layers) and hidden_dim=128 (1-3 hidden layers); got %d x %d"
                                      % (num_layers, hidden_dim))
        if hidden_dim == 128 and (input_dim > 64 or output_dim > 224 or not bias):
            raise NotImplementedError("128-wide fused decoder: input_dim <= 64, output_dim <= 224, with biases; got %d -> %d" % (input_dim, output_dim))
        self.input_dim, self.output_dim, self.hidden_dim = input_dim, output_dim, hidden_dim
        self.layers = nn.ModuleList([nn.Linear(input_dim if i == 0 else hidden_dim, hidden_dim, bias=bias)
                                     for i in range(num_layers)])
        self.lout = nn.Linear(hidden_dim, output_dim, bias=bias)

    def weights(self):
        lins = list(self.layers) + [self.lout]
        return [l.weight for l in lins], [l.bias for l in lins]

    def forward(self, x1, x2=None, x2_index=None, out_act=L.ACT_NONE, mode=L.MLP_MFMA_BF16, out_dtype=torch.float32,
                x1_grouped=None, x2_packs=None, hold=None):
        W, b = self.weights()
        if self.hidden_dim == 128:
            if mode == L.MLP_MFMA_BF16 and x1.is_cuda:
                return ops.fused_mlp128(x1, W, b, x2=x2, x2_index=x2_index, in_dim=self.input_dim, out_act=out_act, mode=mode,
                                        out_dtype=out_dtype, x1_grouped=x1_grouped, x2_packs=x2_packs)
            if x1_grouped is not None:
                raise NotImplementedError("the tensor-op form of the 128-wide decoder reads strided features")
            n1 = min(x1.shape[1], self.input_dim)
            x = x1[:, :n1].float()
            if self.input_dim > n1:
                x = torch.cat([x, x2[x2_index.long(), :self.input_dim - n1].float()], -1)
            return ops.wide_mlp_reference(x, W, b, out_act).to(out_dtype)
        return ops.fused_mlp(x1, W, b, x2=x2, x2_index=x2_index, in_dim=self.input_dim, out_act=out_act, mode=mode,
                             out_dtype=out_dtype, x1_grouped=x1_grouped, x2_packs=x2_packs, hold=hold)


_PARAM_NAMES = {}


def _param_names(fn):
    key = getattr(fn, "__func__", fn)
    names = _PARAM_NAMES.get(key)
    if names is None:
        names = _PARAM_NAMES[key] = frozenset(inspect.signature(fn).parameters)
    return names


def positional_embed(x, num_freq):
    bands = 2.0 ** torch.linspace(0.0, num_freq - 1, num_freq, device=x.device)
    w = (x[:, None, :] * bands[None, :, None]).reshape(x.shape[0], num_freq * x.shape[-1])
    return torch.cat([x, torch.sin(w), torch.cos(w)], dim=-1)


class PanopticDeltaNeF(nn.Module):
    accepts_ray_index = True

    def __init__(self, grid_type="PermutoGrid", interpolation_type="linear", multiscale_type="cat", feature_dim=2,
                 num_lods=24, base_lod=2, hidden_dim=64, num_layers=1, activation_type="relu", layer_type="none",
                 embedder_type="positional", view_multires=4, pos_multires=4, position_input=False,
                 num_classes=-1, num_instances=-1,
                 sem_activation_type=None, sem_num_layers=None, sem_hidden_dim=None, sem_normalize=False,
                 sem_softmax=False, sem_sigmoid=False, sem_detach=True,
                 inst_num_layers=None, inst_hidden_dim=None, inst_normalize=False, inst_softmax=False,
                 inst_sigmoid=False, inst_detach=True, panoptic_features_type=None,
                 delta_num_layers=1, delta_hidden_dim=64, inst_soft_temperature=0.0,
                 raymarch_type="ray", precision="bf16", **kwargs):
        super().__init__()
# ... 123 lines not shown
                                        addend=addend)
        if self.multiscale_type == "sum":
            feats = self._pad8(feats.float().reshape(-1, self.num_lods, self.feature_dim).sum(-2), self.feat_dtype)
        return feats

    def prefetch_features(self, coords):
        if self.multiscale_type != "cat" or self.grid is None:
            return
        self._prefetched = (coords, self._interp(self.grid, coords), torch.is_grad_enabled())

    def _panoptic_feats(self, feats_detached, coords):
        t = self.panoptic_features_type
        if t == "pos_encoding":
            return self._pad8(positional_embed(coords.reshape(-1, 3).float(), self.pos_multires), self.feat_dtype)
        if t == "position":
            return self._pad8(coords.reshape(-1, 3).float(), self.feat_dtype)
        if t == "appearance":
            return feats_detached
        if t == "separate":
            return self._interp(self.delta_grid, coords.detach())
        if self._grouped() is not None:
            return self._interp(self.delta_grid, coords.detach(), addend=feats_detached)
        return feats_detached + self._interp(self.delta_grid, coords.detach())

    def rgb_semantics(self, coords, ray_d=None, compute_channels=None, pidx=None, lod_idx=None, ridx=None, ray_dirs=None,
                      ray_packs=None):
        out = {}
        if not compute_channels:
            return out
        if isinstance(compute_channels, str):
            compute_channels = {compute_channels}
        batch, num_samples, _ = coords.shape
        mode = self.mlp_mode
        pre = getattr(self, "_prefetched", None)
        self._prefetched = None
        if pre is not None and pre[0] is coords and pre[2] == torch.is_grad_enabled():
            feats = pre[1]
        else:
            feats = self._interp(self.grid, coords)
        self._feat_cache = (coords, feats if self._heads_read_live_features() else feats.detach())
        grp = self._grouped()
        wide = self.decoder_density.hidden_dim == 128 or self.decoder_color.hidden_dim == 128
        hold = ops.decoder_hold() if (ops.CD_FUSED and "rgb" in compute_channels and feats.is_cuda and not wide) else None
        try:
            density_feats = self.decoder_density(feats, mode=mode, out_dtype=self.feat_dtype, x1_grouped=grp, hold=hold)
            self._density_feats = density_feats.detach()
            if "rgb" in compute_channels:
                if num_samples != 1 and ridx is None:
                    ray_d = ray_d[:, None].repeat(1, num_samples, 1).reshape(-1, 3)
                pe, index = self._view_embedding(ray_d, ridx, ray_dirs)
                if wide:
                    rgb = self.decoder_color(density_feats, x2=pe, x2_index=index, out_act=L.ACT_SIGMOID, mode=mode,
                                             x2_packs=ray_packs if ridx is not None else None)
                    density = torch.relu(density_feats[:, 0:1].float()).reshape(batch, num_samples, 1)
                else:
                    W, b = self.decoder_color.weights()
                    rgb, sigma = ops.colour_and_density(density_feats, W, b, pe, index, self.decoder_color.input_dim, out_act=L.ACT_SIGMOID,
                                                        mode=mode, x2_packs=ray_packs if ridx is not None else None, producer=hold)
                    density = sigma.reshape(batch, num_samples, 1)
                out["rgb"] = rgb.reshape(batch, num_samples, 3)
            else:
                density = torch.relu(density_feats[:, 0:1].float()).reshape(batch, num_samples, 1)
        finally:
            ops.flush_hold(hold)
        if "density" in compute_channels:
            out["density"] = density
        if "semantics" in compute_channels or "inst_embedding" in compute_channels:
            (sem_in, sem_grp), (inst_in, inst_grp) = self._head_inputs(feats, coords, compute_channels)
            if "semantics" in compute_channels:
                plain = not (self.sem_sigmoid or self.sem_normalize)
                act = L.ACT_SOFTMAX if (self.sem_softmax and plain) else L.ACT_NONE
                s = self.decoder_semantics(sem_in, out_act=act, mode=mode, x1_grouped=sem_grp, out_dtype=self.feat_dtype)
                if not plain:
                    s = torch.sigmoid(s) if self.sem_sigmoid else s
                    s = F.normalize(s, dim=-1) if self.sem_normalize else s
                    s = F.softmax(s, dim=-1) if self.sem_softmax else s
                out["semantics"] = s
            if "inst_embedding" in compute_channels:
                out["inst_embedding"] = self._inst_head(inst_in, inst_grp, mode)
        return out

    def _inst_head(self, inst_in, inst_grp, mode):
        plain = not (self.inst_sigmoid or self.inst_normalize or self.inst_soft_temperature > 0.0)
        act = L.ACT_SOFTMAX if (self.inst_softmax and plain) else L.ACT_NONE
        e = self.decoder_inst(inst_in, out_act=act, mode=mode, x1_grouped=inst_grp, out_dtype=self.feat_dtype)
        if not plain:
            e = torch.sigmoid(e) if self.inst_sigmoid else e
            e = F.normalize(e, dim=-1) if self.inst_normalize else e
            e = e / self.inst_soft_temperature if self.inst_soft_temperature > 0.0 else e
            e = F.softmax(e, dim=-1) if self.inst_softmax else e
        return e

    def _heads_read_live_features(self):
        return False

    def _head_inputs(self, feats, coords, channels):
        pan = self._panoptic_feats(feats.detach(), coords)
        grp = self._pan_grouped()
        return (pan, grp), (pan, grp)

    WIDE_HEAD_PAD = os.environ.get("PAG_WIDE_HEAD_PAD", "1") != "0"

    def _wide_head_weights(self, dec, x):
        W, b = dec.weights()
        if not (self.WIDE_HEAD_PAD and len(W) == 2 and x.is_cuda and self.precision == "bf16" and W[0].shape[0] == 64 and 192 < W[1].shape[0] <= 224
                and b[0] is not None and b[1] is not None):
            return W, b
        pad = getattr(self, "_wide_pad", None)
        if pad is None or pad[0].device != W[0].device:
            pad = self._wide_pad = (torch.eye(64, device=W[0].device), torch.zeros(64, device=W[0].device))
        return [W[0], pad[0], W[1]], [b[0], pad[1], b[1]]

    def _wide_head_requested(self, channels):
        return any(dec.hidden_dim == 128 for ch, dec in (("semantics", self.decoder_semantics), ("inst_embedding", self.decoder_inst)) if ch in channels)

    def can_fuse_panoptic(self, channels):
        if self.precision != "bf16" or self._pan_grouped() is None or self._wide_head_requested(channels):
            return False
        ok = True
        if "semantics" in channels:
            ok &= self.sem_softmax and not (self.sem_sigmoid or self.sem_normalize)
        if "inst_embedding" in channels:
            ok &= self.inst_softmax and not (self.inst_sigmoid or self.inst_normalize or self.inst_soft_temperature > 0.0)
        return bool(ok)

    def panoptic_composited(self, coords, channels, w, alpha, ridx, pack_start, ray_of_pack, N):
        cache = getattr(self, "_feat_cache", None)
        self._feat_cache = None
        if cache is not None and cache[0] is coords:
            feats = cache[1]
        elif self._heads_read_live_features():
            feats = self._interp(self.grid, coords)
        else:
            with torch.no_grad():
                feats = self._interp(self.grid, coords)
        (sem_in, sem_grp), (inst_in, inst_grp) = self._head_inputs(feats, coords, channels)
        out = {}
        if "semantics" in channels and "inst_embedding" in channels and sem_in is inst_in and sem_grp is not None:
            heads = ((*self._wide_head_weights(self.decoder_inst, sem_in), self.decoder_inst.input_dim),
                     (*self.decoder_semantics.weights(), self.decoder_semantics.input_dim))
            out["inst_embedding"], out["semantics"] = ops.head_composite_pair(sem_in, heads, w, alpha, ridx, pack_start, ray_of_pack, N,
                                                                              out_dtype=self.feat_dtype, x1_grouped=sem_grp)
            return out
        for ch, dec, x, grp in (("semantics", self.decoder_semantics, sem_in, sem_grp), ("inst_embedding", self.decoder_inst, inst_in, inst_grp)):
            if ch in channels:
                W, b = self._wide_head_weights(dec, x) if ch == "inst_embedding" else dec.weights()
                out[ch] = ops.head_composite(x, W, b, w, alpha, ridx, pack_start, ray_of_pack, N, in_dim=dec.input_dim,
                                             out_act=L.ACT_SOFTMAX, out_dtype=self.feat_dtype, x1_grouped=grp)
        return out

    @torch.no_grad()
    def prune(self, jitter=None):
        if self.grid is None:
            return
        density_decay = 0.6
        min_density = (0.01 * 512) / np.sqrt(3)
        dev = self.device
        g = self.grid
        points = g.dense_points.to(dev)
        res = 2.0 ** g.blas_level
        if jitter is None:
            jitter = torch.rand(points.shape[0], 3, device=dev)
        samples = (points.float() + jitter) / res * 2.0 - 1.0
        views = torch.zeros(points.shape[0], 3, device=dev)
        views[:, 2] = 1.0
        with g.fp32_coords():
            density = self.forward(coords=samples[:, None], ray_d=views, channels="density")
        g.occupancy = g.occupancy.to(dev).float().contiguous()
        bits = torch.empty(max(1, (g.num_cells + 31) // 32), dtype=torch.int32, device=dev)
        ops.occupancy_update(density.reshape(-1), g.occupancy, bits, density_decay, min_density)
        for grid in [self.grid] + ([self.delta_grid] if hasattr(self, "delta_grid") else []):
            grid.blas_init_bits(bits)


class PanopticNeF(PanopticDeltaNeF):

    def __init__(self, *args, sem_detach=True, inst_detach=True, inst_direct_pos=False, panoptic_features_type=None, **kwargs):
        if panoptic_features_type == "pos_encoding":
            raise AttributeError("'PanopticNeF' object has no attribute 'pos_embed_dim'")
        super().__init__(*args, sem_detach=sem_detach, inst_detach=inst_detach,
                         panoptic_features_type="position" if panoptic_features_type == "position" else "appearance", **kwargs)
        self.panoptic_features_type = panoptic_features_type
        self.sem_detach, self.inst_detach, self.inst_direct_pos = bool(sem_detach), bool(inst_detach), bool(inst_direct_pos)
        if self.inst_soft_temperature > 0.0:
            raise NotImplementedError("inst_soft_temperature is an option of PanopticDeltaNeF only")

    def get_nef_type(self):
        return "panoptic_nef"

    def _pan_grouped(self):
        return self._grouped()

    def _heads_read_live_features(self):
        return not (self.sem_detach and (self.inst_detach or self.inst_direct_pos))

    def _head_inputs(self, feats, coords, channels):
        grp = self._grouped()
        if "semantics" in channels and self.panoptic_features_type == "position":
            raise RuntimeError("mat1 and mat2 shapes cannot be multiplied: PanopticNeF feeds its semantic head the grid features "
                               "(panoptic_nef.py:338) but panoptic_features_type='position' sized it for 3 inputs (:99-101)")
        det = feats.detach()
        sem = det if self.sem_detach else feats
        if self.inst_direct_pos:
            inst, inst_grp = self._pad8(coords.reshape(-1, 3).float(), self.feat_dtype), None
        else:
            inst = sem if self.inst_detach == self.sem_detach else (det if self.inst_detach else feats)
            inst_grp = grp
        return (sem, grp), (inst, inst_grp)

    def _inst_head(self, inst_in, inst_grp, mode):
        if self.inst_softmax:
            return self.decoder_inst(inst_in, out_act=L.ACT_SOFTMAX, mode=mode, x1_grouped=inst_grp, out_dtype=self.feat_dtype)
        e = self.decoder_inst(inst_in, out_act=L.ACT_NONE, mode=mode, x1_grouped=inst_grp, out_dtype=self.feat_dtype)
        e = torch.sigmoid(e) if self.inst_sigmoid else e
        return F.normalize(e, dim=-1) if self.inst_normalize else e

    def rgb_semantics(self, coords, ray_d=None, compute_channels=None, pidx=None, lod_idx=None, ridx=None, ray_dirs=None,
                      ray_packs=None):
        out = super().rgb_semantics(coords, ray_d=ray_d, compute_channels=compute_channels, pidx=pidx, lod_idx=lod_idx, ridx=ridx,
                                    ray_dirs=ray_dirs, ray_packs=ray_packs)
        if self.inst_direct_pos and "inst_embedding" in out:
            out["inst_embedding"] = out["inst_embedding"].reshape(coords.shape[0], coords.shape[1], -1)
        return out

    def can_fuse_panoptic(self, channels):
# ... 9 lines not shown
```

pagnerf_amd/ops.py:

```python
import ctypes
import os
import threading
import time

import torch

from . import _lib as L


_PROFILE = None


_PROFILE_ONLY = None


def profile_start(only=None):
    global _PROFILE, _PROFILE_ONLY
    _PROFILE = {}
    _PROFILE_ONLY = set(only) if only is not None else None


def profile_stop():
    global _PROFILE
    prof, _PROFILE = _PROFILE, None
    torch.cuda.synchronize()
    return {k: [a.elapsed_time(b) for a, b in v] for k, v in (prof or {}).items()}


def _call(name, *args):
    fn = getattr(L.load(), name)
    if _PROFILE is None or (_PROFILE_ONLY is not None and name not in _PROFILE_ONLY):
        L.check(fn(*args), name)
        return
    a, b = torch.cuda.Event(enable_timing=True), torch.cuda.Event(enable_timing=True)
    a.record()
    L.check(fn(*args), name)
    b.record()
    _PROFILE.setdefault(name, []).append((a, b))


def _check_gpu(*ts):
    for t in ts:
        if t is not None and not t.is_cuda:
            raise RuntimeError("pagnerf_amd ops need GPU tensors (no CPU fallback); got a tensor on %s" % t.device)


class _EncodeSpec:

    def __init__(self, kind, n_levels, n_feat, **kw):
        self.kind = kind
        self.L = int(n_levels)
        self.F = int(n_feat)
        if kind == "hash":
            self.kw = dict(log2_T=int(kw["log2_T"]), resolutions=_float_list(kw["resolutions"]), half_coords=bool(kw.get("half_coords", False)))
        elif kind == "permuto":
            self.kw = dict(capacity=int(kw["capacity"]), scale_factor=_float_list(kw["scale_factor"]), shift=_float_list(kw["shift"]),
                           half_coords=bool(kw.get("half_coords", False)))
        else:
            raise ValueError(kind)
        self._bind()

    def _bind(self):
        kw = self.kw
# ... 211 lines not shown
    try:
        return torch.mm(a, b, out_dtype=torch.float32)
    except (TypeError, RuntimeError):
        return (a @ b).float()


class _InferCtx:
    saved_tensors = ()

    def __init__(self, n):
        self.needs_input_grad = (False,) * n

    def save_for_backward(self, *tensors):
        pass

    def mark_non_differentiable(self, *tensors):
        pass

    def set_materialize_grads(self, value):
        pass


def _apply(fn, *args):
    if torch.is_grad_enabled():
        return fn.apply(*args)
    return fn.forward(_InferCtx(len(args)), *args)


def _need_grad(*tensors):
    return torch.is_grad_enabled() and any(t is not None and t.requires_grad for t in tensors)


class _Launch:
    __slots__ = ("entry", "bare", "args", "M", "keep", "taken", "fused", "out_ptr")

    def __init__(self, entry, bare=False):
        self.entry, self.bare = entry, bare
        self.args, self.M, self.keep, self.taken, self.fused, self.out_ptr = None, 0, (), False, False, 0

    def park(self, args, M, keep, fused=False, out_ptr=0):
        self.args, self.M, self.keep, self.fused, self.out_ptr = args, M, keep, fused, out_ptr

    @property
    def pending(self):
        return self.args is not None and not self.taken

    def issue(self):
        if self.pending:
            _call(self.entry, ctypes.byref(self.args), self.M, L.stream())
            self.taken = True


class _DecoderCall:
    __slots__ = ("in_dim", "out_act", "mode", "out_dtype", "grouped", "x2_packs", "need_grad", "col0_relu", "rank1", "stats_only", "composite", "park",
                 "pair", "producer", "n_rays")

    def __init__(self, in_dim, out_act, mode, out_dtype, grouped, x2_packs=None, need_grad=False, col0_relu=False, rank1=False, stats_only=False,
                 composite=None, park=None, pair=None, producer=None, n_rays=0):
        self.in_dim, self.out_act, self.mode, self.out_dtype = int(in_dim), out_act, mode, out_dtype
        self.grouped = grouped if grouped is None else tuple(grouped)
        self.x2_packs, self.need_grad, self.col0_relu, self.rank1, self.stats_only = x2_packs, need_grad, col0_relu, rank1, stats_only
        self.composite, self.park, self.pair, self.producer, self.n_rays = composite, park, pair, producer, n_rays


class _DecoderState:
    __slots__ = ("in_dim", "out_act", "mode", "out_dtype", "grouped", "x2_packs", "needs", "M", "k1", "n_layers", "n_hidden", "has_stats", "bc", "saved",
                 "col0_relu", "composited", "head", "hc", "x1_shape", "x1_dtype")

    def __init__(self, call, needs, M, k1, n_layers, saved, x1):
        self.in_dim, self.out_act, self.mode, self.out_dtype, self.grouped = call.in_dim, call.out_act, call.mode, call.out_dtype, call.grouped
        self.x2_packs = call.x2_packs
        self.needs = (bool(needs[0]), bool(needs[1]))
        self.M, self.k1, self.n_layers, self.saved = M, k1, n_layers, saved
        self.x1_shape, self.x1_dtype = tuple(x1.shape), x1.dtype
        self.n_hidden, self.has_stats, self.bc = 0, False, None
        self.col0_relu = None
        self.composited = False
        self.head = None
        self.hc = None


def _save(ctx, st):
    ctx.save_for_backward(*st.saved)
    st.saved = None
    ctx.state, ctx.x2_packs = st, st.x2_packs


def _operands(x1, x2, x2_index, Ws, bs, grouped):
    _check_gpu(x1, x2, x2_index, *Ws, *bs)
    if grouped is not None:
        M, k1 = x1.shape[1], 64
    else:
        M, k1 = x1.shape
    x1 = x1.detach()
    if not x1.is_contiguous():
        x1 = x1.contiguous()
    if x1.dtype not in (torch.float32, torch.bfloat16):
        x1 = x1.float()
    if x2 is not None:
        x2 = x2.detach().contiguous().float()
        x2_index = x2_index.detach().contiguous()
        if x2_index.dtype != torch.int32:
            x2_index = x2_index.int()
    return x1, x2, x2_index, [w.detach().contiguous().float() for w in Ws], [b.detach().contiguous().float() for b in bs], M, k1


def _fill_shape(a, k1, in_dim, out_dim, out_act, out_dtype, grouped):
    a.k1, a.in_dim, a.out_dim, a.out_act, a.out_dtype = k1, in_dim, out_dim, out_act, L._DT[out_dtype]
    if grouped is not None:
        a.x1_layout, a.x1_levels, a.x1_feats = L.LAYOUT_XCD8, grouped[0], grouped[1]


def _fill_operands(a, x1=None, x2=None, x2_index=None, W=(), b=()):
    if x1 is not None:
        a.x1, a.x1_dtype = L.ptr(x1), L.dtype_code(x1)
    if x2 is not None:
        a.x2, a.k2p, a.x2_index = L.ptr(x2), x2.shape[1], L.ptr(x2_index)
    for i, w in enumerate(W):
        a.W[i] = L.ptr(w)
    for i, v in enumerate(b):
        a.b[i] = L.ptr(v)


def _dx2(x2, x2_index, x2_packs, dz0, w_tail, seg=None):
    R, dev = x2.shape[0], x2.device
    if seg is not None:
        pass
    elif x2_packs is not None:
        pack_start, ray_of_pack = x2_packs
        seg = composite_feats(dz0, torch.ones(dz0.shape[0], device=dev), torch.ones(R, device=dev), pack_start, ray_of_pack, R)
    else:
        seg = torch.zeros(R, dz0.shape[1], device=dev).index_add_(0, x2_index.long(), dz0.float())
    dx2 = torch.zeros_like(x2)
    dx2[:, :w_tail.shape[1]] = seg @ w_tail
    return dx2


_NON_NULL = 1
_BWD_FUSABLE = {}


def _bwd_fusable(M, x1_dtype, needs, k1, k2p, in_dim, n_layers, out_dim, out_act, out_dtype, mode, grouped, rank1=False, has_stats=False,
                 stats_only=False, col0=False):
    if not (WGRAD_FUSED and 0 < M <= L.MLP_FUSED_WIDE_MAX_M and needs[0]) or (needs[1] and grouped is not None):
        return False
    key = (x1_dtype, k1, k2p, in_dim, n_layers, out_dim, out_act, out_dtype, mode, grouped, rank1, has_stats, stats_only, col0)
    if key in _BWD_FUSABLE:
        return _BWD_FUSABLE[key]
    a = L.MlpBwdArgs()
    _fill_shape(a, k1, in_dim, out_dim, out_act, out_dtype, grouped)
    a.n_layers, a.mode = n_layers, mode
    a.x1, a.x1_dtype, a.dx1, a.dx1_dtype = _NON_NULL, L._DT[x1_dtype], _NON_NULL, L._DT[x1_dtype]
    if k2p:
        a.x2, a.k2p, a.x2_index = _NON_NULL, k2p, _NON_NULL
# ... 33 lines not shown
        a.hidden_save[i] = L.ptr(h)
    _call("pag_mlp_fwd", ctypes.byref(a), M, L.stream())
    return full


def _mlp_forward(call, needs, x1, x2, x2_index, *wb):
    lib = L.load()
    n_layers = len(wb) // 2
    x1, x2, x2_index, Wc, bc, M, k1 = _operands(x1, x2, x2_index, wb[:n_layers], wb[n_layers:], call.grouped)
    in_dim, out_act, mode, out_dtype, grouped, need_grad = call.in_dim, call.out_act, call.mode, call.out_dtype, call.grouped, call.need_grad
    dev, out_dim = x1.device, Wc[-1].shape[0]
    mfma = mode == L.MLP_MFMA_BF16
    wide_softmax = mfma and out_act == L.ACT_SOFTMAX and out_dim > 64 and out_dtype == torch.bfloat16
    stats_only = call.stats_only and wide_softmax
    has_stats = wide_softmax and (need_grad or stats_only)
    col0 = bool(call.col0_relu and mfma and grouped is None and x1.dtype == torch.bfloat16 and out_dim <= 64 and M)
    out = None if stats_only else torch.empty(M, out_dim, device=dev, dtype=out_dtype)
    recompute = need_grad and _bwd_fusable(M, x1.dtype, needs, k1, x2.shape[1] if x2 is not None else 0, in_dim, n_layers, out_dim, out_act, out_dtype,
                                           mode, grouped, call.rank1, has_stats, stats_only, col0)
    hidden = []
    if need_grad or stats_only:
        for i in range(n_layers - 1):
            keep = (need_grad and not recompute) or (stats_only and i == n_layers - 2)
            hidden.append(torch.empty(M, 64, device=dev, dtype=torch.bfloat16 if mfma else torch.float32) if keep else None)
    a = L.MlpFwdArgs()
    _fill_shape(a, k1, in_dim, out_dim, out_act, out_dtype, grouped)
    _fill_operands(a, x1, x2, x2_index, Wc, bc)
    a.n_layers, a.mode, a.out = n_layers, mode, L.ptr(out)
    for i, h in enumerate(hidden):
        a.hidden_save[i] = L.ptr(h)
    stats = torch.empty(M, 2, device=dev) if has_stats else None
    a.softmax_stats = L.ptr(stats)
    st = _DecoderState(call, needs, M, k1, n_layers, (x1, x2, x2_index, out, *hidden, *Wc, *((stats, bc[-1]) if has_stats else ())), x1)
    st.n_hidden, st.has_stats, st.bc = len(hidden), has_stats, bc
    if col0:
        st.col0_relu = torch.empty(M, device=dev)
        a.x1_col0_relu = L.ptr(st.col0_relu)
    if stats_only:
        st.head = (hidden[-1], Wc[-1], bc[-1], stats)
    park = call.park
    if park is not None and park.bare and not (mfma and all(t is None for t in hidden) and stats is None and not col0):
        park = None
    producer = call.producer
    if producer is not None:
        if producer.pending and M and x1.data_ptr() == producer.out_ptr \
                and lib.pag_mlp_fwd_producer_supported(ctypes.byref(a), ctypes.byref(producer.args), M) == 1:
            a.x1_producer = ctypes.pointer(producer.args)
            producer.taken = True
        else:
            producer.issue()
    if M and park is not None:
        park.park(a, M, [x1, x2, x2_index, out, stats, st.col0_relu, *hidden, *Wc, *bc], out_ptr=out.data_ptr() if out is not None else 0)
    elif M:
        pair = call.pair
        if pair is not None and pair.pending and M <= L.MLP_FUSED_WIDE_MAX_M and lib.pag_mlp_fwd_pair_supported(ctypes.byref(a), ctypes.byref(pair.args)) == 1:
            a.pair = ctypes.pointer(pair.args)
            pair.taken = True
        if call.composite is not None and HEAD_FWD_ONCE and stats_only and lib.pag_mlp_fwd_composite_supported(ctypes.byref(a), M) == 1:
            a.composite = ctypes.pointer(call.composite)
            st.composited = True
        _call("pag_mlp_fwd", ctypes.byref(a), M, L.stream())
    return out, st


def _mlp_backward(st, saved, g, rank1=None, dx1_into=None, dx1_out=None, col0_add=None, col0_gate=None, wgrad_queue=None, hold=None, pair=None):
    lib = L.load()
    in_dim, out_act, mode, out_dtype, grouped, n_layers, k1, M = st.in_dim, st.out_act, st.mode, st.out_dtype, st.grouped, st.n_layers, st.k1, st.M
    x1, x2, x2_index, out = saved[:4]
    hidden = list(saved[4:4 + st.n_hidden])
    Wc = list(saved[4 + st.n_hidden:4 + st.n_hidden + n_layers])
    stats, b_last = (saved[-2], saved[-1]) if st.has_stats else (None, None)
    out_dim = Wc[-1].shape[0]
    dev = x1.device
    zdt = torch.bfloat16 if mode == L.MLP_MFMA_BF16 else torch.float32
    need_dx = st.needs[0]
    need_dx2 = st.needs[1] and x2 is not None
    dx1 = (dx1_into if dx1_into is not None else (dx1_out if dx1_out is not None else torch.empty(x1.shape, device=dev, dtype=x1.dtype))) \
        if need_dx else None
    a = L.MlpBwdArgs()
    if rank1 is None:
        g = g.contiguous().to(out_dtype)
        a.grad_out = L.ptr(g)
    else:
        a.g_ray, a.g_scale, a.g_index, a.g_ray_scale = (L.ptr(t) for t in rank1)
    _fill_shape(a, k1, in_dim, out_dim, out_act, out_dtype, grouped)
    _fill_operands(a, W=Wc, b=st.bc)
    a.out, a.n_layers, a.mode = L.ptr(out), n_layers, mode
    a.dx1, a.dx1_dtype = L.ptr(dx1), (L.dtype_code(dx1) if need_dx else 0)
    a.softmax_stats, a.b_last = L.ptr(stats), L.ptr(b_last)
    a.dx1_accumulate = 1 if (need_dx and dx1_into is not None) else 0
    fuse_col0 = col0_add is not None and need_dx and grouped is None and mode == L.MLP_MFMA_BF16 and out_dim <= 64
    if col0_gate is not None and not fuse_col0:
        col0_add, col0_gate = col0_add * (col0_gate > 0), None
    if fuse_col0:
        a.dx1_col0_add = L.ptr(col0_add)
        if col0_gate is not None:
            a.dx1_col0_gate = L.ptr(col0_gate)
    fused = False
    dz0_fused = dz0_slots = ws = None
    if WGRAD_FUSED and 0 < M <= L.MLP_FUSED_WIDE_MAX_M and mode == L.MLP_MFMA_BF16 and x1.dtype == torch.bfloat16 \
            and (not need_dx2 or grouped is None):
        _fill_operands(a, x1, x2, x2_index)
        fused = lib.pag_mlp_bwd_fused_supported(ctypes.byref(a)) == 1
        if fused and need_dx2:
            packs = st.x2_packs
            if DZ0_SLOTS and packs is not None and _one_pack_per_ray(packs[1], x2.shape[0]) and packs[0].shape[0] == x2.shape[0] + 1:
                dz0_slots = torch.empty(lib.pag_mlp_dz0_slots_bytes(M, x2.shape[0]) // 4, device=dev)
                a.dz0_slots = L.ptr(dz0_slots)
            else:
                dz0_fused = torch.empty(M, 64, device=dev, dtype=torch.bfloat16)
                a.dz[0] = L.ptr(dz0_fused)
    if not fused and any(h is None for h in hidden):
        hidden = _recompute_hidden(st, x1, x2, x2_index, Wc, hidden)
    for i, h in enumerate(hidden):
        a.hidden_save[i] = L.ptr(h)
    dz = None
    gW, gb = [], []
    if fused:
        ws_bytes = lib.pag_mlp_bwd_fused_workspace_bytes(ctypes.byref(a), M)
        ws = torch.empty(ws_bytes // 4, device=dev)
        a.wgrad_workspace, a.wgrad_workspace_bytes = L.ptr(ws), ws_bytes
        for l in range(n_layers):
            gW.append(torch.empty(Wc[l].shape[0], in_dim if l == 0 else 64, device=dev))
            gb.append(torch.empty(Wc[l].shape[0], device=dev))
            a.dW[l], a.db[l] = L.ptr(gW[l]), L.ptr(gb[l])
    else:
        dz = [torch.empty(M, 64, device=dev, dtype=zdt) for _ in range(n_layers - 1)] + [torch.empty(M, out_dim, device=dev, dtype=zdt)]
        for i in range(n_layers):
            a.dz[i] = L.ptr(dz[i])
    if M and hold is not None:
        hold.park(a, M, [x1, x2, x2_index, out, stats, b_last, g, dx1, col0_add, col0_gate, dz0_slots, dz0_fused, ws, *(rank1 or ()), *hidden, *Wc, *gW,
                         *gb, *(dz or ())], fused=fused)
    elif M:
        if pair is not None and fused and pair.pending and pair.fused and lib.pag_mlp_bwd_pair_supported(ctypes.byref(a), ctypes.byref(pair.args)) == 1:
            a.pair = ctypes.pointer(pair.args)
            pair.taken = True
        _call("pag_mlp_bwd", ctypes.byref(a), M, L.stream())
    if col0_add is not None and need_dx and not fuse_col0:
        dx1[:, 0] += col0_add.to(dx1.dtype)
    if fused:
        pass
    elif mode == L.MLP_MFMA_BF16 and M:
        specs = []
        for l in range(n_layers):
            n_out = Wc[l].shape[0]
            sp = dict(dz=dz[l], n_out=n_out, a2=None, k2p=0, a2_index=None, levels=0, feats=0)
            if l == 0 and grouped is not None:
                sp.update(a1=x1, a1_dtype=L.BF16, a1_layout=L.LAYOUT_XCD8, k1=64, n_in=64, levels=grouped[0], feats=grouped[1])
            elif l == 0:
                sp.update(a1=x1, a1_dtype=L.dtype_code(x1), a1_layout=L.LAYOUT_STRIDED, k1=k1, n_in=in_dim,
                          a2=x2, k2p=(x2.shape[1] if x2 is not None else 0), a2_index=x2_index)
            else:
                sp.update(a1=hidden[l - 1], a1_dtype=L.BF16, a1_layout=L.LAYOUT_STRIDED, k1=64, n_in=64)
            sp["w"] = torch.empty(n_out, in_dim if l == 0 else 64, device=dev)
            sp["b"] = torch.empty(n_out, device=dev)
            gW.append(sp["w"])
            gb.append(sp["b"])
            specs.append(sp)
        if wgrad_queue is not None:
            wgrad_queue.extend(specs)
        else:
            _launch_wgrad(specs, M)
    else:
        for l in range(n_layers):
            z = dz[l]
            if l == 0:
                n1 = min(k1, in_dim)
                w = _mm_f32(z.t(), x1[:, :n1].to(z.dtype))
                if in_dim > k1:
                    seg = torch.zeros(x2.shape[0], 64, device=dev, dtype=torch.float32)
# ... 89 lines not shown
        _save(ctx, st)
        return out

    @staticmethod
    def backward(ctx, g):
        return _decoder_grads(_mlp_backward(ctx.state, ctx.saved_tensors, g))


class _ColourDensity(torch.autograd.Function):

    @staticmethod
    def forward(ctx, call, x1, x2, x2_index, *wb):
        rgb, st = _mlp_forward(call, ctx.needs_input_grad[1:3], x1, x2, x2_index, *wb)
        _save(ctx, st)
        ctx.pre = None
        if st.col0_relu is not None:
            return rgb, st.col0_relu
        ctx.pre = x1.detach()[:, 0].float()
        return rgb, torch.relu(ctx.pre)

    @staticmethod
    def backward(ctx, g_rgb, g_sigma):
        st, saved = ctx.state, ctx.saved_tensors
        if g_rgb is None:
            g_rgb = torch.zeros_like(saved[3])
        if g_sigma is None:
            return _decoder_grads(_mlp_backward(st, saved, g_rgb))
        if ctx.pre is None:
            return _decoder_grads(_mlp_backward(st, saved, g_rgb, col0_add=g_sigma.float().contiguous(), col0_gate=st.col0_relu))
        return _decoder_grads(_mlp_backward(st, saved, g_rgb, col0_add=(g_sigma.float() * (ctx.pre > 0)).contiguous()))


def colour_and_density(x1, weights, biases, x2, x2_index, in_dim, out_act=L.ACT_SIGMOID, mode=L.MLP_MFMA_BF16,
                       out_dtype=torch.float32, x2_packs=None, producer=None):
    call = _DecoderCall(in_dim, out_act, mode, out_dtype, None, x2_packs=x2_packs, need_grad=_need_grad(x1, x2, x2_index, *weights, *biases),
                        col0_relu=True, producer=producer)
    return _apply(_ColourDensity, call, x1, x2, x2_index, *weights, *biases)


def fused_mlp(x1, weights, biases, x2=None, x2_index=None, in_dim=None, out_act=L.ACT_NONE, mode=L.MLP_MFMA_BF16,
              out_dtype=torch.float32, x1_grouped=None, x2_packs=None, hold=None):
    if in_dim is None:
        in_dim = weights[0].shape[1]
    call = _DecoderCall(in_dim, out_act, mode, out_dtype, x1_grouped, x2_packs=x2_packs, need_grad=_need_grad(x1, x2, x2_index, *weights, *biases),
                        park=hold)
    return _apply(_FusedMLP, call, x1, x2, x2_index, *weights, *biases)


def wide_mlp_reference(x, W, b, out_act=L.ACT_NONE, round_bf16=False):
    def r(t):
        return t + (t.detach().bfloat16().to(t.dtype) - t.detach()) if round_bf16 else t
    h = r(x)
    for i in range(len(W)):
        h = torch.nn.functional.linear(h, r(W[i]), None if b[i] is None else b[i])
        if i + 1 < len(W):
            h = r(torch.relu(h))
    if out_act == L.ACT_SIGMOID:
        h = torch.sigmoid(h)
    elif out_act == L.ACT_SOFTMAX:
        h = torch.softmax(h, -1)
    return h


def _native_plane(ws, col0, width, M):
    Mp = (M + L.MLP128_BATCH - 1) // L.MLP128_BATCH * L.MLP128_BATCH
    p = ws.view(torch.bfloat16)[Mp * col0:Mp * (col0 + width)].view(Mp // 32, width // 32, 4, 2, 32, 4)
    return p.permute(0, 4, 1, 2, 3, 5).reshape(Mp, width)[:M]


def _mlp128_forward(call, needs, x1, x2, x2_index, *wb):
    n_hidden = len(wb) // 2 - 1
    if any(v is None for v in wb[n_hidden + 1:]):
        raise NotImplementedError("fused_mlp128 needs biases")
    x1, x2, x2_index, Wc, bc, M, k1 = _operands(x1, x2, x2_index, wb[:n_hidden + 1], wb[n_hidden + 1:], call.grouped)
    out_dim = Wc[-1].shape[0]
    out = torch.empty(M, out_dim, device=x1.device, dtype=call.out_dtype)
    a = L.Mlp128FwdArgs()
    _fill_shape(a, k1, call.in_dim, out_dim, call.out_act, call.out_dtype, call.grouped)
# ... 722 lines not shown
        return (None, dx1, None, None, None, None, None, *gW, *gb)


class _HeadCompositePair(torch.autograd.Function):

    @staticmethod
    def forward(ctx, calls, x1, weights_w, alpha, ridx, pack_start, ray_of_pack, *wb):
        call_a, call_b, n_a = calls
        part_a, part_b = wb[:n_a], wb[n_a:]
        needs_x1 = ctx.needs_input_grad[1]
        probs_b, st_b = _mlp_forward(call_b, (needs_x1, False), x1, None, None, *part_b)
        out_a, st_a = _head_forward(call_a, needs_x1, x1, weights_w, alpha, ridx, pack_start, ray_of_pack, *part_a)
        call_b.park.issue()
        out_b = _head_composite(st_b, probs_b, x1.device, part_b[len(part_b) // 2 - 1].shape[0], weights_w, alpha, ridx, pack_start, ray_of_pack,
                                call_b.n_rays)
        ctx.states = (st_a, st_b)
        return out_a, out_b

    @staticmethod
    def backward(ctx, g_a, g_b):
        st_a, st_b = ctx.states
        queue = []
        x1 = st_a.saved[0]
        dx = torch.empty(x1.shape, device=x1.device, dtype=x1.dtype) if st_a.needs[0] else None
        hold = _Launch("pag_mlp_bwd")
        _, _, gW_b, gb_b = _head_backward(st_b, st_b.saved, g_b, dx1_into=dx, wgrad_queue=queue, hold=hold if dx is not None else None)
        dx1, _, gW_a, gb_a = _head_backward(st_a, st_a.saved, g_a, wgrad_queue=queue, dx1_out=dx, pair=hold)
        hold.issue()
        if queue:
            _launch_wgrad(queue, queue[0]["dz"].shape[0])
        return (None, dx1, None, None, None, None, None, *gW_a, *gb_a, *gW_b, *gb_b)


def head_composite_pair(x1, heads, w, alpha, ridx, pack_start, ray_of_pack, N, out_dtype=torch.bfloat16, x1_grouped=None):
    (wa, ba, ia), (wb_, bb, ib) = heads
    need_grad = _need_grad(x1, w, alpha, ridx, pack_start, ray_of_pack, *wa, *ba, *wb_, *bb)
    parked = _Launch("pag_mlp_fwd")
    calls = (_head_call(ia, L.ACT_SOFTMAX, out_dtype, x1_grouped, need_grad, n_rays=N, pair=parked),
             _head_call(ib, L.ACT_SOFTMAX, out_dtype, x1_grouped, need_grad, n_rays=N, park=parked), len(wa) + len(ba))
    return _apply(_HeadCompositePair, calls, x1, w, alpha, ridx, pack_start, ray_of_pack, *wa, *ba, *wb_, *bb)


def head_composite(x1, weights, biases, w, alpha, ridx, pack_start, ray_of_pack, N, in_dim=None, out_act=L.ACT_NONE,
                   out_dtype=torch.bfloat16, x1_grouped=None):
    if in_dim is None:
        in_dim = weights[0].shape[1]
    call = _head_call(in_dim, out_act, out_dtype, x1_grouped, _need_grad(x1, w, alpha, ridx, pack_start, ray_of_pack, *weights, *biases), n_rays=N)
    return _apply(_HeadComposite, call, x1, w, alpha, ridx, pack_start, ray_of_pack, *weights, *biases)


_LOSS_WS = {}


class NllTerm:

    def __init__(self, prob, target, weight=1.0, temperature=1.0, conf=None, mean_over="valid"):
        assert mean_over in ("valid", "all")
        self.prob, self.target, self.weight, self.temperature, self.conf, self.mean_over = prob, target, weight, temperature, conf, mean_over


class _RenderLoss(torch.autograd.Function):
    @staticmethod
    def forward(ctx, rgb, prob_a, prob_b, rgb_gt, rgb_weight, term_a, term_b, eps):
        src = rgb if rgb is not None else (prob_a if prob_a is not None else prob_b)
        _check_gpu(src)
        dev = src.device
        N = src.shape[0]
        f = lambda t: t.detach().contiguous().float() if t is not None else None
        rgb_c, gt_c = f(rgb), f(rgb_gt)
        if rgb_c is not None:
            rgb_c, gt_c = rgb_c.reshape(N, 3), gt_c.reshape(N, 3)
        targs, keep = [], [rgb_c, gt_c]
        for prob, t in ((prob_a, term_a), (prob_b, term_b)):
            if prob is None:
                targs += [None, 0, None, None, 0.0, 1.0, 0]
                continue
            p = f(prob).reshape(N, -1)
            tg = t.target.detach().reshape(-1).long().contiguous()
            cf = f(t.conf).reshape(-1) if t.conf is not None else None
            keep += [p, tg, cf]
# ... 496 lines not shown
```

pagnerf_amd/optim.py:

```python
import ctypes

import torch

from . import _lib as L
from . import ops


class _Plan:

    def __init__(self, opt, params):
        self.params = params
        self.ids = tuple(id(p) for p in params)
        for p in params:
            st = opt.state[p]
            if len(st) == 0:
                st["step"] = torch.tensor(0.0, dtype=torch.float32)
                st["exp_avg"] = torch.zeros_like(p, memory_format=torch.preserve_format)
                st["exp_avg_sq"] = torch.zeros_like(p, memory_format=torch.preserve_format)
        states = [opt.state[p] for p in params]
        self.steps = [st["step"] for st in states]
        self.state_ids = tuple((id(st["step"]), id(st["exp_avg"]), id(st["exp_avg_sq"])) for st in states)
        self.ok = all(isinstance(t, torch.Tensor) and not t.is_cuda for t in self.steps) and \
            all(st["exp_avg"].is_cuda and st["exp_avg"].dtype == torch.float32 and st["exp_avg"].is_contiguous() and
                st["exp_avg_sq"].dtype == torch.float32 and st["exp_avg_sq"].is_contiguous() for st in states)
# ... 53 lines not shown
            gg[i] = g.data_ptr()
        return plan

    @torch.no_grad()
    def step(self, closure=None):
        loss = None
        if closure is not None:
            with torch.enable_grad():
                loss = closure()
        fallback = []
        for gi, group in enumerate(self.param_groups):
            plan = self._plan(gi, group) if self._group_ok(group) else None
            if plan is False:
                continue
            if plan is None:
                if any(p.grad is not None for p in group["params"]):
                    fallback.append(gi)
                continue
            beta1, beta2 = group["betas"]
            hyper = (float(group["lr"]), float(beta1), float(beta2), float(group["eps"]), float(group["weight_decay"]))
            if plan.uniform:
                self._launch(plan, plan.pp, plan.gg, plan.mm, plan.vv, plan.nn, plan.n, hyper, plan.count + 1)
                plan.count += 1
            else:
                by = {}
                for i, t in enumerate(plan.steps):
                    by.setdefault(int(float(t)) + 1, []).append(i)
                for count, idx in sorted(by.items()):
                    n = len(idx)
                    sel = lambda a, ct: (ct * n)(*[a[i] for i in idx])
                    self._launch(plan, sel(plan.pp, ctypes.c_void_p), sel(plan.gg, ctypes.c_void_p), sel(plan.mm, ctypes.c_void_p),
                                 sel(plan.vv, ctypes.c_void_p), sel(plan.nn, ctypes.c_int64), n, hyper, count)
            torch._foreach_add_(plan.steps, 1)
        if fallback:
            self._torch_step(fallback)
        return loss

    @staticmethod
    def _launch(plan, pp, gg, mm, vv, nn, n, hyper, count):
        if plan.device.index is not None and plan.device.index != torch.cuda.current_device():
            with torch.cuda.device(plan.device):
                ops._call("pag_adam_step", n, pp, gg, mm, vv, nn, *hyper, count, L.stream())
        else:
            ops._call("pag_adam_step", n, pp, gg, mm, vv, nn, *hyper, count, L.stream())

    def _torch_step(self, group_ids):
        keep = self.param_groups
        inner = torch.optim.Adam.step
        if getattr(inner, "hooked", False) and hasattr(inner, "__wrapped__"):
            inner = inner.__wrapped__
        try:
            self.param_groups = [keep[i] for i in group_ids]
            inner(self)
        finally:
            self.param_groups = keep
        self._plans = {k: v for k, v in self._plans.items() if k not in group_ids}
```

Baseline: 1.220 million.

## Pre-pack MLP weights into bf16 LDS images once per step

Adds a weight-image packing kernel that converts the fp32 decoder weights once per optimizer step into bf16 blocks already laid out (and transposed) as the fused MLP kernels expect in LDS. Forward, backward, pair and head kernels then load these images with plain 16-byte vector copies instead of each block converting and transposing the weights during staging. The optimizer now bumps parameter versions so stale images are detected and rebuilt. This cuts per-block prologue work, at the cost of an extra pack launch, extra memory, and cache-invalidation logic that must stay correct under stream capture.

Result: no change. 1.225 million (median of 6 runs) (+0.4%).

```diff
diff --git a/include/pagnerf_hip.h b/include/pagnerf_hip.h
--- a/include/pagnerf_hip.h
+++ b/include/pagnerf_hip.h
@@ -131,6 +131,15 @@
     float *dz0_slots;
 } pag_mlp_bwd_args;
 int pag_mlp_bwd(const pag_mlp_bwd_args *args, int64_t M, void *stream);
+typedef struct pag_mlp_weight_images {
+    const float *W[3]; int n_layers; int in_dim; int out_dim;
+    int x1_layout; int x1_levels; int x1_feats;
+    void *image;
+} pag_mlp_weight_images;
+int64_t pag_mlp_weight_images_bytes(int n_layers, int out_dim);
+int pag_mlp_pack_weights(const pag_mlp_weight_images *decoders, int n_decoders, void *stream);
+int pag_mlp_fwd_packed(const pag_mlp_fwd_args *args, const void *images, const void *rider_images, int64_t M, void *stream);
+int pag_mlp_bwd_packed(const pag_mlp_bwd_args *args, const void *images, const void *rider_images, int64_t M, void *stream);
 int64_t pag_mlp_dz0_slots_bytes(int64_t M, int64_t R);
 int pag_mlp_dz0_slots_sum(const int64_t *pack_start, int64_t R, const float *slots, float *out, void *stream);
 int pag_mlp_bwd_fused_supported(const pag_mlp_bwd_args *args);
diff --git a/pagnerf_amd/_lib.py b/pagnerf_amd/_lib.py
--- a/pagnerf_amd/_lib.py
+++ b/pagnerf_amd/_lib.py
@@ -72,6 +72,11 @@
                 ("pair", ctypes.POINTER(MlpBwdArgs)), ("dz0_slots", c_vp)]
 
 
+class MlpWeightImages(ctypes.Structure):
+    _fields_ = [("W", c_vp * 3), ("n_layers", c_i32), ("in_dim", c_i32), ("out_dim", c_i32),
+                ("x1_layout", c_i32), ("x1_levels", c_i32), ("x1_feats", c_i32), ("image", c_vp)]
+
+
 class DeepMlpArgs(ctypes.Structure):
     _fields_ = [("coords", c_vp), ("ray_d", c_vp), ("hidden", c_i32), ("num_classes", c_i32), ("channels", c_i32), ("save", c_i32),
                 ("W", c_vp * 14), ("b", c_vp * 14), ("density", c_vp), ("rgb", c_vp), ("semantics", c_vp),
@@ -156,6 +161,10 @@
     "pag_mlp_fwd_composite_supported": (c_i32, [ctypes.POINTER(MlpFwdArgs), c_i64]),
     "pag_mlp_fwd_producer_supported": (c_i32, [ctypes.POINTER(MlpFwdArgs), ctypes.POINTER(MlpFwdArgs), c_i64]),
     "pag_mlp_bwd": (c_i32, [ctypes.POINTER(MlpBwdArgs), c_i64, c_vp]),
+    "pag_mlp_weight_images_bytes": (c_i64, [c_i32, c_i32]),
+    "pag_mlp_fwd_packed": (c_i32, [ctypes.POINTER(MlpFwdArgs), c_vp, c_vp, c_i64, c_vp]),
+    "pag_mlp_bwd_packed": (c_i32, [ctypes.POINTER(MlpBwdArgs), c_vp, c_vp, c_i64, c_vp]),
+    "pag_mlp_pack_weights": (c_i32, [ctypes.POINTER(MlpWeightImages), c_i32, c_vp]),
     "pag_mlp_bwd_fused_supported": (c_i32, [ctypes.POINTER(MlpBwdArgs)]),
     "pag_mlp_bwd_fused_workspace_bytes": (c_i64, [ctypes.POINTER(MlpBwdArgs), c_i64]),
     "pag_mlp_bwd_pair_supported": (c_i32, [ctypes.POINTER(MlpBwdArgs), ctypes.POINTER(MlpBwdArgs)]),
diff --git a/pagnerf_amd/build.py b/pagnerf_amd/build.py
--- a/pagnerf_amd/build.py
+++ b/pagnerf_amd/build.py
@@ -20,6 +20,7 @@
     "mlp_wgrad.hip": MLP,
     "render.hip": ["-ffp-contract=off"],
     "mlp_affine.hip": MLP,
+    "mlp_pack.hip": MLP,
     "api.cpp": ["-x", "hip"],
     "assign.hip": ["-ffp-contract=off"],
     "loss.hip": ["-ffp-contract=off"],
diff --git a/pagnerf_amd/csrc/mlp.hip b/pagnerf_amd/csrc/mlp.hip
--- a/pagnerf_amd/csrc/mlp.hip
+++ b/pagnerf_amd/csrc/mlp.hip
@@ -20,6 +20,8 @@
     const float *b2[2];
     void *out2;
     int out2_dim;
+    const bf16_t *img[3];
+    const bf16_t *img2[2];
 };
 
 struct BwdParams {
@@ -48,6 +50,8 @@
     float *slabs[3];
     const float *b[3];
     float *dz0_slots;
+    const bf16_t *img_s[3];
+    const bf16_t *img_t[3];
 };
 
 constexpr int STAGE_BATCH = 8;
@@ -118,6 +122,27 @@
                 dst_t[at[k]] = (bf16_t)v[k];
             }
     }
+}
+
+template <int BYTES, int THREADS>
+struct ImageCopy {
+    static_assert(BYTES % 16 == 0, "whole 16-byte pieces");
+    static constexpr int PIECES = BYTES / 16, STEPS = (PIECES + THREADS - 1) / THREADS;
+    f32x4 v[STEPS];
+    __device__ __forceinline__ void fetch(const bf16_t *img) {
+#pragma unroll
+        for (int k = 0; k < STEPS; ++k) v[k] = reinterpret_cast<const f32x4 *>(img)[min((int)threadIdx.x + k * THREADS, PIECES - 1)];
+    }
+    __device__ __forceinline__ void store(bf16_t *dst) const {
+#pragma unroll
+        for (int k = 0; k < STEPS; ++k) reinterpret_cast<f32x4 *>(dst)[min((int)threadIdx.x + k * THREADS, PIECES - 1)] = v[k];
+    }
+};
+
+template <int BYTES, int THREADS>
+__device__ __noinline__ void image_copy_call(bf16_t *dst, const bf16_t *img) {
+    ImageCopy<BYTES, THREADS> c;
+    c.fetch(img), c.store(dst);
 }
 
 __device__ __forceinline__ void pack_block(const f32x16 &acc, bf16x8 &lo, bf16x8 &hi) {
@@ -858,11 +883,18 @@
     bf16_t *W0c = lds_at<bf16_t>(smem, L.W0c), *W1c = lds_at<bf16_t>(smem, L.W1c), *WLc = lds_at<bf16_t>(smem, L.WLc);
     float *b0d = lds_at<float>(smem, L.b0d), *bLd = lds_at<float>(smem, L.bLd);
     float *b0c = lds_at<float>(smem, L.b0c), *b1c = lds_at<float>(smem, L.b1c), *bLc = lds_at<float>(smem, L.bLc);
-    stage_weight(W0d, RS, 64, 64, pd.W[0], HID, pd.in_dim, false, pd.grp_L, pd.grp_F);
-    stage_weight(WLd, RS, 32, 64, pd.W[1], pd.out_dim, HID, true);
-    stage_weight(W0c, RS, 64, 64, pc.W[0], HID, pc.in_dim, false);
-    stage_weight(W1c, RS, 64, 64, pc.W[1], HID, HID, true);
-    stage_weight(WLc, RS, 32, 64, pc.W[2], pc.out_dim, HID, true);
+    if (pd.img[0] && pc.img[0]) {
+        ImageCopy<W64, 256> c0d, c0c, c1c;
+        ImageCopy<W32, 256> cLd, cLc;
+        c0d.fetch(pd.img[0]), cLd.fetch(pd.img[1]), c0c.fetch(pc.img[0]), c1c.fetch(pc.img[1]), cLc.fetch(pc.img[2]);
+        c0d.store(W0d), cLd.store(WLd), c0c.store(W0c), c1c.store(W1c), cLc.store(WLc);
+    } else {
+        stage_weight(W0d, RS, 64, 64, pd.W[0], HID, pd.in_dim, false, pd.grp_L, pd.grp_F);
+        stage_weight(WLd, RS, 32, 64, pd.W[1], pd.out_dim, HID, true);
+        stage_weight(W0c, RS, 64, 64, pc.W[0], HID, pc.in_dim, false);
+        stage_weight(W1c, RS, 64, 64, pc.W[1], HID, HID, true);
+        stage_weight(WLc, RS, 32, 64, pc.W[2], pc.out_dim, HID, true);
+    }
     for (int e = threadIdx.x; e < 64; e += blockDim.x) {
         b0d[e] = pd.b[0][e];
         b0c[e] = pc.b[0][e];
@@ -953,12 +985,33 @@
 
 constexpr int WIDE_FWD_PAIR_THREADS = 1024;
 constexpr int wide_fwd_waves(bool pair) { return (pair ? WIDE_FWD_PAIR_THREADS : 256) / 64; }
+template <int OB, bool PAIR, int THREADS>
+__device__ __forceinline__ void stage_head_weights(const FwdParams &p, bf16_t *W0s, bf16_t *W1s, bf16_t *WLs, bf16_t *W0s2, bf16_t *WLs2) {
+    if (p.img[0] && (!PAIR || p.img2[0])) {
+        ImageCopy<W64, THREADS> c0, c1, c02;
+        ImageCopy<OB * W32, THREADS> cL;
+        ImageCopy<W32, THREADS> cL2;
+        c0.fetch(p.img[0]), c1.fetch(p.img[1]), cL.fetch(p.img[2]);
+        if constexpr (PAIR) c02.fetch(p.img2[0]), cL2.fetch(p.img2[1]);
+        c0.store(W0s), c1.store(W1s), cL.store(WLs);
+        if constexpr (PAIR) c02.store(W0s2), cL2.store(WLs2);
+    } else {
+        stage_weight(W0s, RS, 64, 64, p.W[0], HID, p.in_dim, false, p.grp_L, p.grp_F);
+        stage_weight(W1s, RS, 64, 64, p.W[1], HID, HID, true);
+        stage_weight(WLs, RS, OB * 32, 64, p.W[2], p.out_dim, HID, true);
+        if constexpr (PAIR) {
+            stage_weight(W0s2, RS, 64, 64, p.W2[0], HID, p.in_dim, false, p.grp_L, p.grp_F);
+            stage_weight(WLs2, RS, 32, 64, p.W2[1], p.out2_dim, HID, true);
+        }
+    }
+}
 template <bool SAVE0, bool PAIR>
 __global__ __launch_bounds__(PAIR ? WIDE_FWD_PAIR_THREADS : 256, PAIR ? 1 : 2) void mlp_fwd_wide_stats(FwdParams p) {
     extern __shared__ __attribute__((aligned(16))) unsigned char smem[];
     constexpr int OB = 7;
     constexpr float LOG2E = 1.4426950408889634f;
     const int NW = blockDim.x >> 6;
+    constexpr int HEAD_THREADS = wide_fwd_waves(PAIR) * 64;
     constexpr FwdLds L(3, OB, wide_fwd_waves(PAIR), PAIR);
     bf16_t *W0s = lds_at<bf16_t>(smem, L.W0), *W1s = lds_at<bf16_t>(smem, L.W1);
     bf16_t *WLs = lds_at<bf16_t>(smem, L.WL);
@@ -966,12 +1019,8 @@
     float *b0s = lds_at<float>(smem, L.b0), *b1s = lds_at<float>(smem, L.b1), *bLs = lds_at<float>(smem, L.bL);
     float *b0s2 = lds_at<float>(smem, L.b0p), *bLs2 = lds_at<float>(smem, L.bLp);
     bf16_t *stg = lds_at<bf16_t>(smem, L.stg) + (threadIdx.x >> 6) * (L.stg_stride / 2);
-    stage_weight(W0s, RS, 64, 64, p.W[0], HID, p.in_dim, false, p.grp_L, p.grp_F);
-    stage_weight(W1s, RS, 64, 64, p.W[1], HID, HID, true);
-    stage_weight(WLs, RS, OB * 32, 64, p.W[2], p.out_dim, HID, true);
+    stage_head_weights<OB, PAIR, HEAD_THREADS>(p, W0s, W1s, WLs, W0s2, WLs2);
     if constexpr (PAIR) {
-        stage_weight(W0s2, RS, 64, 64, p.W2[0], HID, p.in_dim, false, p.grp_L, p.grp_F);
-        stage_weight(WLs2, RS, 32, 64, p.W2[1], p.out2_dim, HID, true);
         for (int e = threadIdx.x; e < 64; e += blockDim.x) b0s2[e] = p.b2[0][e];
         for (int e = threadIdx.x; e < 32; e += blockDim.x) bLs2[e] = e < p.out2_dim ? p.b2[1][e] : 0.0f;
     }
@@ -1430,12 +1479,22 @@
     bf16_t *WLt = lds_at<bf16_t>(smem, L.WLt);
     bf16_t *W1t = lds_at<bf16_t>(smem, L.W1t);
     bf16_t *W0t = lds_at<bf16_t>(smem, L.W0t);
-    stage_weight_t(WLt, RSL, 64, OBL * 32, p.W[NL - 1], p.out_dim, HID);
+    const bool packed = p.img_s[0] != nullptr;
+    if (!packed) stage_weight_t(WLt, RSL, 64, OBL * 32, p.W[NL - 1], p.out_dim, HID);
     bf16_t *W0s = lds_at<bf16_t>(smem, L.W0s);
     bf16_t *W1s = lds_at<bf16_t>(smem, L.W1s);
     float *b0s = lds_at<float>(smem, L.b0), *b1s = lds_at<float>(smem, L.b1);
-    stage_weight_both(W0s, RS, false, W0t, RS, 64, 64, p.W[0], HID, p.in_dim, p.grp_L, p.grp_F);
-    if (NL == 3) stage_weight_both(W1s, RS, true, W1t, RS, 64, 64, p.W[1], HID, HID);
+    if (packed) {
+        ImageCopy<64 * RSL * 2, 256> cLt;
+        ImageCopy<W64, 256> c0s, c0t, c1s, c1t;
+        cLt.fetch(p.img_t[NL - 1]), c0s.fetch(p.img_s[0]), c0t.fetch(p.img_t[0]);
+        if constexpr (NL == 3) c1s.fetch(p.img_s[1]), c1t.fetch(p.img_t[1]);
+        cLt.store(WLt), c0s.store(W0s), c0t.store(W0t);
+        if constexpr (NL == 3) c1s.store(W1s), c1t.store(W1t);
+    } else {
+        stage_weight_both(W0s, RS, false, W0t, RS, 64, 64, p.W[0], HID, p.in_dim, p.grp_L, p.grp_F);
+        if (NL == 3) stage_weight_both(W1s, RS, true, W1t, RS, 64, 64, p.W[1], HID, HID);
+    }
     for (int e = threadIdx.x; e < 64; e += blockDim.x) {
         b0s[e] = p.b[0][e];
         b1s[e] = NL == 3 ? p.b[1][e] : 0.0f;
@@ -1851,6 +1910,7 @@
 struct PairParams {
     BwdParams i, s;
 };
+template <bool PACKED >
 __global__ __launch_bounds__(256, 1) void mlp_bwd_pair(PairParams pp) {
     const BwdParams &pi = pp.i, &ps = pp.s;
     extern __shared__ __attribute__((aligned(16))) unsigned char smem[];
@@ -1862,10 +1922,15 @@
     bf16_t *WLtS = lds_at<bf16_t>(smem, L.WLtS);
     bf16_t *W0tS = lds_at<bf16_t>(smem, L.W0tS), *W0sS = lds_at<bf16_t>(smem, L.W0sS);
     float *b0I = lds_at<float>(smem, L.b0I), *b0S = lds_at<float>(smem, L.b0S);
-    stage_weight_t(WLtI, RSLI, 64, 64, pi.W[1], pi.out_dim, HID);
-    stage_weight_both(W0sI, RS, false, W0tI, RS, 64, 64, pi.W[0], HID, pi.in_dim, pi.grp_L, pi.grp_F);
-    stage_weight_t(WLtS, RSLS, 64, 32, ps.W[1], ps.out_dim, HID);
-    stage_weight_both(W0sS, RS, false, W0tS, RS, 64, 64, ps.W[0], HID, ps.in_dim, ps.grp_L, ps.grp_F);
+    if constexpr (PACKED) {
+        image_copy_call<64 * RSLI * 2, 256>(WLtI, pi.img_t[1]), image_copy_call<W64, 256>(W0sI, pi.img_s[0]), image_copy_call<W64, 256>(W0tI, pi.img_t[0]);
+        image_copy_call<64 * RSLS * 2, 256>(WLtS, ps.img_t[1]), image_copy_call<W64, 256>(W0sS, ps.img_s[0]), image_copy_call<W64, 256>(W0tS, ps.img_t[0]);
+    } else {
+        stage_weight_t(WLtI, RSLI, 64, 64, pi.W[1], pi.out_dim, HID);
+        stage_weight_both(W0sI, RS, false, W0tI, RS, 64, 64, pi.W[0], HID, pi.in_dim, pi.grp_L, pi.grp_F);
+        stage_weight_t(WLtS, RSLS, 64, 32, ps.W[1], ps.out_dim, HID);
+        stage_weight_both(W0sS, RS, false, W0tS, RS, 64, 64, ps.W[0], HID, ps.in_dim, ps.grp_L, ps.grp_F);
+    }
     for (int e = threadIdx.x; e < 64; e += blockDim.x) {
         b0I[e] = pi.b[0][e];
         b0S[e] = ps.b[0][e];
@@ -2178,7 +2243,14 @@
     float *grow = lds_at<float>(smem, L.grow);
     float *dotbuf = lds_at<float>(smem, L.dot);
     bf16x8 *zbuf = lds_at<bf16x8>(smem, L.zbuf);
-    stage_weight_both(WLs, RS, true, WLt, RSL, OB * 32, 64, p.W[0], p.out_dim, HID);
+    if (p.img_s[0]) {
+        ImageCopy<OB * W32, (OB + 1) * 64> cs;
+        ImageCopy<64 * RSL * 2, (OB + 1) * 64> ct;
+        cs.fetch(p.img_s[0]), ct.fetch(p.img_t[0]);
+        cs.store(WLs), ct.store(WLt);
+    } else {
+        stage_weight_both(WLs, RS, true, WLt, RSL, OB * 32, 64, p.W[0], p.out_dim, HID);
+    }
     for (int e = threadIdx.x; e < OB * 32; e += blockDim.x) bLs[e] = e < p.out_dim ? p.b_last[e] : -1e30f;
     for (int e = threadIdx.x; e < 2 * OB * 64; e += blockDim.x) dotbuf[e] = 0.0f;
     for (int e = threadIdx.x; e < 2 * OB * 2 * 64 * 4; e += blockDim.x) reinterpret_cast<float *>(zbuf)[e] = 0.0f;
@@ -2831,6 +2903,7 @@
     extern __shared__ __attribute__((aligned(16))) unsigned char smem[];
     constexpr int OB = 7;
     constexpr float LOG2E = 1.4426950408889634f;
+    constexpr int HEAD_THREADS = 256;
     constexpr FwdLds L(3, OB, 4, PAIR, true);
     bf16_t *W0s = lds_at<bf16_t>(smem, L.W0), *W1s = lds_at<bf16_t>(smem, L.W1);
     bf16_t *WLs = lds_at<bf16_t>(smem, L.WL);
@@ -2839,12 +2912,8 @@
     float *b0s2 = lds_at<float>(smem, L.b0p), *bLs2 = lds_at<float>(smem, L.bLp);
     float *red = lds_at<float>(smem, L.red);
     bf16_t *stg = lds_at<bf16_t>(smem, L.stg) + (threadIdx.x >> 6) * (L.stg_stride / 2);
-    stage_weight(W0s, RS, 64, 64, p.W[0], HID, p.in_dim, false, p.grp_L, p.grp_F);
-    stage_weight(W1s, RS, 64, 64, p.W[1], HID, HID, true);
-    stage_weight(WLs, RS, OB * 32, 64, p.W[2], p.out_dim, HID, true);
+    stage_head_weights<OB, PAIR, HEAD_THREADS>(p, W0s, W1s, WLs, W0s2, WLs2);
     if constexpr (PAIR) {
-        stage_weight(W0s2, RS, 64, 64, p.W2[0], HID, p.in_dim, false, p.grp_L, p.grp_F);
-        stage_weight(WLs2, RS, 32, 64, p.W2[1], p.out2_dim, HID, true);
         for (int e = threadIdx.x; e < 64; e += blockDim.x) b0s2[e] = p.b2[0][e];
         for (int e = threadIdx.x; e < 32; e += blockDim.x) bLs2[e] = e < p.out2_dim ? p.b2[1][e] : 0.0f;
     }
@@ -3186,13 +3255,30 @@
            a->out_act == PAG_ACT_SOFTMAX && a->out_dim > 192 && a->out_dim <= 224 && a->hidden_save[1];
 }
 
-void set_pair_head(FwdParams &p, const pag_mlp_fwd_args *b) {
+void set_fwd_images(const bf16_t *(&img)[3], const void *block, int n_layers, int out_dim) {
+    const WeightImage I(n_layers, out_dim);
+    for (int l = 0; l < 3; ++l) img[l] = (block && l < n_layers) ? reinterpret_cast<const bf16_t *>(static_cast<const unsigned char *>(block) + I.s[l]) : nullptr;
+}
+void set_bwd_images(BwdParams &p, const void *block, int n_layers, int out_dim) {
+    const WeightImage I(n_layers, out_dim);
+    for (int l = 0; l < 3; ++l) {
+        const bool have = block && l < n_layers;
+        p.img_s[l] = have ? reinterpret_cast<const bf16_t *>(static_cast<const unsigned char *>(block) + I.s[l]) : nullptr;
+        p.img_t[l] = have ? reinterpret_cast<const bf16_t *>(static_cast<const unsigned char *>(block) + I.t[l]) : nullptr;
+    }
+}
+
+void set_pair_head(FwdParams &p, const pag_mlp_fwd_args *b, const void *images) {
     p.W2[0] = b->W[0];
     p.W2[1] = b->W[1];
     p.b2[0] = b->b[0];
     p.b2[1] = b->b[1];
     p.out2 = b->out;
     p.out2_dim = b->out_dim;
+    const bf16_t *img[3];
+    set_fwd_images(img, images, 2, b->out_dim);
+    p.img2[0] = img[0];
+    p.img2[1] = img[1];
 }
 
 template <typename X1T, typename OutT, int NL>
@@ -3318,7 +3404,7 @@
     return wide && (!a->pair || pag_mlp_fwd_pair_supported(a, a->pair) == 1) ? 1 : 0;
 }
 
-extern "C" int pag_mlp_fwd(const pag_mlp_fwd_args *a, int64_t M, void *stream) {
+static int mlp_fwd_run(const pag_mlp_fwd_args *a, const void *images, const void *rider_images, int64_t M, void *stream) {
     PAG_CHECK_ARG(a, "pag_mlp_fwd: args is NULL");
     PAG_CHECK_ARG(M >= 0, "pag_mlp_fwd: M < 0");
     PAG_CHECK_ARG(a->n_layers == 2 || a->n_layers == 3, "pag_mlp_fwd: n_layers %d not in {2,3}", a->n_layers);
@@ -3355,6 +3441,9 @@
     p.W2[0] = p.W2[1] = p.b2[0] = p.b2[1] = nullptr;
     p.out2 = nullptr;
     p.out2_dim = 0;
+    p.img2[0] = p.img2[1] = nullptr;
+    PAG_CHECK_ARG(((uintptr_t)images & 15) == 0 && ((uintptr_t)rider_images & 15) == 0, "pag_mlp_fwd_packed: the weight images must be 16-byte aligned");
+    set_fwd_images(p.img, a->mode == PAG_MLP_MFMA_BF16 ? images : nullptr, a->n_layers, a->out_dim);
     for (int l = 0; l < 3; ++l) {
         p.W[l] = l < a->n_layers ? a->W[l] : nullptr;
         p.b[l] = l < a->n_layers ? a->b[l] : nullptr;
@@ -3386,7 +3475,7 @@
         PAG_CHECK_ARG(!a->pair || (kind == 3 && pag_mlp_fwd_pair_supported(a, a->pair) == 1), "pag_mlp_fwd: pair is not supported for these arguments (pag_mlp_fwd_pair_supported)");
         PAG_CHECK_ARG(!a->composite || kind == 3, "pag_mlp_fwd: composite rides only in the statistics-only wide softmax head (pag_mlp_fwd_composite_supported)");
         if (kind == 3) {
-            if (a->pair) set_pair_head(p, a->pair);
+            if (a->pair) set_pair_head(p, a->pair, rider_images);
             if (a->composite) {
                 const pag_head_composite_args *hc = a->composite;
                 PAG_CHECK_ARG(hc->P >= 0 && (hc->P == 0 || (hc->pack_start && hc->ray_of_pack && hc->weights && hc->alpha && hc->out)),
@@ -3439,6 +3528,7 @@
             pd.hsave[0] = pd.hsave[1] = nullptr;
             pd.grp_L = d->x1_levels;
             pd.grp_F = d->x1_feats;
+            set_fwd_images(pd.img, rider_images, 2, d->out_dim);
             hipLaunchKernelGGL(mlp_fwd_density_colour, dim3(std::min<unsigned>(mlp_grid(M), FAST_FWD_GRID_CAP)), dim3(256), DensityColourLds{}.bytes, st, pd, p);
             PAG_CHECK_LAUNCH("pag_mlp_fwd (density + colour)");
             return PAG_OK;
@@ -3565,7 +3655,7 @@
     return grid * ((int64_t)(a->n_layers - 1) * 64 + 32) * WG_SLAB_COLS * (int64_t)sizeof(float);
 }
 
-extern "C" int pag_mlp_bwd(const pag_mlp_bwd_args *a, int64_t M, void *stream) {
+static int mlp_bwd_run(const pag_mlp_bwd_args *a, const void *images, const void *rider_images, int64_t M, void *stream) {
     PAG_CHECK_ARG(a, "pag_mlp_bwd: args is NULL");
     PAG_CHECK_ARG(M >= 0, "pag_mlp_bwd: M < 0");
     PAG_CHECK_ARG(a->n_layers == 2 || a->n_layers == 3, "pag_mlp_bwd: n_layers %d not in {2,3}", a->n_layers);
@@ -3637,6 +3727,8 @@
     p.x2_index = a->x2_index;
     p.k2p = a->x2 ? a->k2p : 0;
     for (int l = 0; l < 3; ++l) p.slabs[l] = nullptr;
+    PAG_CHECK_ARG(((uintptr_t)images & 15) == 0 && ((uintptr_t)rider_images & 15) == 0, "pag_mlp_bwd_packed: the weight images must be 16-byte aligned");
+    set_bwd_images(p, fuse ? images : nullptr, a->n_layers, a->out_dim);
     if (fuse && kind == 3) {
         PAG_CHECK_ARG(M <= PAG_MLP_FUSED_WIDE_MAX_M, "pag_mlp_bwd: the fused wide-head backward addresses [M,64] bf16 tensors with 32-bit byte offsets: M %lld > %lld, split the batch",
                       (long long)M, (long long)PAG_MLP_FUSED_WIDE_MAX_M);
@@ -3651,6 +3743,8 @@
         bf16_t *dzh = reinterpret_cast<bf16_t *>(ws);
         BwdParams pa = p;
         pa.W[0] = a->W[2];
+        pa.img_s[0] = p.img_s[2];
+        pa.img_t[0] = p.img_t[2];
         pa.hsave[0] = a->hidden_save[1];
         pa.dz[0] = dzh;
         pa.slabs[0] = slabA;
@@ -3678,6 +3772,7 @@
             ps.act = PAG_ACT_SOFTMAX;
             ps.W[0] = b->W[0];
             ps.W[1] = b->W[1];
+            set_bwd_images(ps, rider_images, 2, b->out_dim);
             ps.b[0] = b->b[0];
             ps.M = M;
             ps.grp_L = p.grp_L;
@@ -3712,9 +3807,14 @@
         fb.p[2] = FinishParams{slabA, (int)grid, a->out_dim, 224, HID, 0, 0, a->dW[2], a->db[2]};
         int n_fin = 3;
         if (b) {
-            raise_lds_limit<mlp_bwd_pair>(LDS_MAX_BYTES);
             PairParams pp{pb, ps};
-            hipLaunchKernelGGL(mlp_bwd_pair, dim3(grid), dim3(256), PairLds{}.bytes, st, pp);
+            if (pb.img_s[0] && ps.img_s[0]) {
+                raise_lds_limit<mlp_bwd_pair<true>>(LDS_MAX_BYTES);
+                hipLaunchKernelGGL(mlp_bwd_pair<true>, dim3(grid), dim3(256), PairLds{}.bytes, st, pp);
+            } else {
+                raise_lds_limit<mlp_bwd_pair<false>>(LDS_MAX_BYTES);
+                hipLaunchKernelGGL(mlp_bwd_pair<false>, dim3(grid), dim3(256), PairLds{}.bytes, st, pp);
+            }
             PAG_CHECK_LAUNCH("pag_mlp_bwd (fused, layers below the wide head + companion head)");
             fb.p[3] = FinishParams{slabS0, (int)grid, HID, 64, b->in_dim, p.grp_L, p.grp_F, b->dW[0], b->db[0]};
             fb.p[4] = FinishParams{slabS1, (int)grid, b->out_dim, 32, HID, 0, 0, b->dW[1], b->db[1]};
@@ -3772,6 +3872,15 @@
     }
     PAG_CHECK_LAUNCH("pag_mlp_bwd");
     return PAG_OK;
+}
+
+extern "C" int pag_mlp_fwd(const pag_mlp_fwd_args *a, int64_t M, void *stream) { return mlp_fwd_run(a, nullptr, nullptr, M, stream); }
+extern "C" int pag_mlp_fwd_packed(const pag_mlp_fwd_args *a, const void *images, const void *rider_images, int64_t M, void *stream) {
+    return mlp_fwd_run(a, images, rider_images, M, stream);
+}
+extern "C" int pag_mlp_bwd(const pag_mlp_bwd_args *a, int64_t M, void *stream) { return mlp_bwd_run(a, nullptr, nullptr, M, stream); }
+extern "C" int pag_mlp_bwd_packed(const pag_mlp_bwd_args *a, const void *images, const void *rider_images, int64_t M, void *stream) {
+    return mlp_bwd_run(a, images, rider_images, M, stream);
 }
 
 namespace {
diff --git a/pagnerf_amd/csrc/mlp_lds.h b/pagnerf_amd/csrc/mlp_lds.h
--- a/pagnerf_amd/csrc/mlp_lds.h
+++ b/pagnerf_amd/csrc/mlp_lds.h
@@ -70,6 +70,22 @@
     constexpr WgradLds(int ob, int ib) : Zt(0), At(Zt + ob * 32 * WG_RS * 2), bytes(At + ib * 32 * WG_RS * 2) {}
 };
 
+struct WeightImage {
+    int ob, rsl, s[3], t[3], s_bytes[3], t_bytes[3], bytes;
+    constexpr WeightImage(int n_layers, int out_dim)
+        : ob((out_dim + 31) / 32), rsl(ob * 32 + 8), s{0, 0, 0}, t{0, 0, 0}, s_bytes{0, 0, 0}, t_bytes{0, 0, 0}, bytes(0) {
+        for (int l = 0; l < n_layers; ++l) {
+            const bool last = l == n_layers - 1;
+            s_bytes[l] = last ? ob * W32 : W64;
+            t_bytes[l] = last ? 64 * rsl * 2 : W64;
+            s[l] = bytes;
+            t[l] = s[l] + s_bytes[l];
+            bytes = t[l] + t_bytes[l];
+        }
+    }
+};
+static_assert(WeightImage(3, 224).bytes % 16 == 0 && WeightImage(2, 1).t[1] % 16 == 0 && W32 % 16 == 0, "weight images are copied in 16-byte pieces");
+
 static_assert(FwdLds(3, OB_MAX, 16, true).bytes <= LDS_MAX_BYTES && FwdLds(3, OB_MAX, 4, true, true).bytes <= LDS_MAX_BYTES, "FwdLds");
 static_assert(DensityColourLds{}.bytes <= LDS_MAX_BYTES, "DensityColourLds");
 static_assert(BwdLds(3, OB_MAX).bytes <= LDS_MAX_BYTES, "BwdLds");
diff --git a/pagnerf_amd/csrc/mlp_pack.hip b/pagnerf_amd/csrc/mlp_pack.hip
--- /dev/null
+++ b/pagnerf_amd/csrc/mlp_pack.hip
@@ -0,0 +1,84 @@
+#include "mlp_common.h"
+#include "mlp_lds.h"
+
+namespace {
+
+constexpr int PACK_MAX = 8;
+constexpr int PACK_BLOCKS = 25;
+
+struct PackDecoder {
+    const float *W[3];
+    int n_layers, in_dim, out_dim, grp_L, grp_F;
+    bf16_t *image;
+};
+struct PackBatch {
+    PackDecoder d[PACK_MAX];
+};
+
+__global__ __launch_bounds__(256) void mlp_pack_kernel(PackBatch batch) {
+    const PackDecoder &D = batch.d[blockIdx.y];
+    const WeightImage I(D.n_layers, D.out_dim);
+    const int pieces = I.bytes / 16;
+    for (int pc = (int)(blockIdx.x * blockDim.x + threadIdx.x); pc < pieces; pc += (int)(gridDim.x * blockDim.x)) {
+        const int byte = pc * 16;
+        int l = 0;
+        while (l + 1 < D.n_layers && byte >= I.s[l + 1]) ++l;
+        const bool last = l == D.n_layers - 1, tr = byte >= I.t[l];
+        const int stride = (tr && last) ? I.rsl : RS;
+        const int e0 = (byte - (tr ? I.t[l] : I.s[l])) / 2;
+        const int row = e0 / stride, c0 = e0 - row * stride;
+        const int n_out = last ? D.out_dim : HID, n_in = l == 0 ? D.in_dim : HID, out_pad = last ? I.ob * 32 : HID;
+        const float *W = D.W[l];
+        float w[8];
+        bool ok[8];
+#pragma unroll
+        for (int j = 0; j < 8; ++j) {
+            const int c = c0 + j;
+            const int o = tr ? swap23(c) : row;
+            const int a = tr ? row : (l > 0 ? swap23(c) : c);
+            const int col = (l == 0 && D.grp_L) ? grp_col(a, D.grp_L, D.grp_F) : a;
+            ok[j] = c < (tr ? out_pad : HID) && o < n_out && col >= 0 && col < n_in;
+            w[j] = W[min(max(o * n_in + col, 0), n_out * n_in - 1)];
+        }
+        bf16x8 v;
+#pragma unroll
+        for (int j = 0; j < 8; ++j) v[j] = (bf16_t)(ok[j] ? w[j] : 0.0f);
+        *reinterpret_cast<bf16x8 *>(reinterpret_cast<unsigned char *>(D.image) + byte) = v;
+    }
+}
+
+}
+
+extern "C" int64_t pag_mlp_weight_images_bytes(int n_layers, int out_dim) {
+    if ((n_layers != 2 && n_layers != 3) || out_dim < 1 || out_dim > 224) return 0;
+    return WeightImage(n_layers, out_dim).bytes;
+}
+
+extern "C" int pag_mlp_pack_weights(const pag_mlp_weight_images *decoders, int n_decoders, void *stream) {
+    PAG_CHECK_ARG(n_decoders >= 0 && n_decoders <= PACK_MAX, "pag_mlp_pack_weights: n_decoders %d not in [0,%d]", n_decoders, PACK_MAX);
+    if (n_decoders == 0) return PAG_OK;
+    PAG_CHECK_ARG(decoders, "pag_mlp_pack_weights: decoders is NULL");
+    PackBatch batch{};
+    for (int i = 0; i < n_decoders; ++i) {
+        const pag_mlp_weight_images &d = decoders[i];
+        PAG_CHECK_ARG(d.n_layers == 2 || d.n_layers == 3, "pag_mlp_pack_weights: decoder %d: n_layers %d not in {2,3}", i, d.n_layers);
+        PAG_CHECK_ARG(d.in_dim >= 1 && d.in_dim <= 64 && d.out_dim >= 1 && d.out_dim <= 224, "pag_mlp_pack_weights: decoder %d: in_dim %d / out_dim %d out of range", i,
+                      d.in_dim, d.out_dim);
+        const bool grp = d.x1_layout == PAG_LAYOUT_XCD8;
+        PAG_CHECK_ARG(!grp || (d.x1_levels >= 1 && d.x1_feats >= 1 && ((d.x1_levels + 7) / 8) * d.x1_feats <= 8 && d.in_dim == d.x1_levels * d.x1_feats),
+                      "pag_mlp_pack_weights: decoder %d: XCD8 input needs in_dim = levels*feats", i);
+        PAG_CHECK_ARG(d.image && ((uintptr_t)d.image & 15) == 0, "pag_mlp_pack_weights: decoder %d: image is NULL or not 16-byte aligned", i);
+        for (int l = 0; l < d.n_layers; ++l) PAG_CHECK_ARG(d.W[l], "pag_mlp_pack_weights: decoder %d: NULL weight of layer %d", i, l);
+        PackDecoder &D = batch.d[i];
+        for (int l = 0; l < 3; ++l) D.W[l] = l < d.n_layers ? d.W[l] : nullptr;
+        D.n_layers = d.n_layers;
+        D.in_dim = d.in_dim;
+        D.out_dim = d.out_dim;
+        D.grp_L = grp ? d.x1_levels : 0;
+        D.grp_F = d.x1_feats;
+        D.image = reinterpret_cast<bf16_t *>(d.image);
+    }
+    hipLaunchKernelGGL(mlp_pack_kernel, dim3(PACK_BLOCKS, n_decoders), dim3(256), 0, (hipStream_t)stream, batch);
+    PAG_CHECK_LAUNCH("pag_mlp_pack_weights");
+    return PAG_OK;
+}
diff --git a/pagnerf_amd/nef.py b/pagnerf_amd/nef.py
--- a/pagnerf_amd/nef.py
+++ b/pagnerf_amd/nef.py
@@ -30,6 +30,7 @@
         self.layers = nn.ModuleList([nn.Linear(input_dim if i == 0 else hidden_dim, hidden_dim, bias=bias)
                                      for i in range(num_layers)])
         self.lout = nn.Linear(hidden_dim, output_dim, bias=bias)
+        self.images = ops.WeightImages() if hidden_dim == 64 else None
 
     def weights(self):
         lins = list(self.layers) + [self.lout]
@@ -50,7 +51,7 @@
                 x = torch.cat([x, x2[x2_index.long(), :self.input_dim - n1].float()], -1)
             return ops.wide_mlp_reference(x, W, b, out_act).to(out_dtype)
         return ops.fused_mlp(x1, W, b, x2=x2, x2_index=x2_index, in_dim=self.input_dim, out_act=out_act, mode=mode,
-                             out_dtype=out_dtype, x1_grouped=x1_grouped, x2_packs=x2_packs, hold=hold)
+                             out_dtype=out_dtype, x1_grouped=x1_grouped, x2_packs=x2_packs, hold=hold, images=self.images)
 
 
 _PARAM_NAMES = {}
@@ -240,6 +241,7 @@
             compute_channels = {compute_channels}
         batch, num_samples, _ = coords.shape
         mode = self.mlp_mode
+        self.pack_weight_images()
         pre = getattr(self, "_prefetched", None)
         self._prefetched = None
         if pre is not None and pre[0] is coords and pre[2] == torch.is_grad_enabled():
@@ -264,7 +266,8 @@
                 else:
                     W, b = self.decoder_color.weights()
                     rgb, sigma = ops.colour_and_density(density_feats, W, b, pe, index, self.decoder_color.input_dim, out_act=L.ACT_SIGMOID,
-                                                        mode=mode, x2_packs=ray_packs if ridx is not None else None, producer=hold)
+                                                        mode=mode, x2_packs=ray_packs if ridx is not None else None, producer=hold,
+                                                        images=self.decoder_color.images)
                     density = sigma.reshape(batch, num_samples, 1)
                 out["rgb"] = rgb.reshape(batch, num_samples, 3)
             else:
@@ -319,6 +322,22 @@
             pad = self._wide_pad = (torch.eye(64, device=W[0].device), torch.zeros(64, device=W[0].device))
         return [W[0], pad[0], W[1]], [b[0], pad[1], b[1]]
 
+    def _inst_grouped(self):
+        return self._pan_grouped()
+
+    def pack_weight_images(self):
+        if self.precision != "bf16" or not ops.WEIGHT_IMAGES:
+            return
+        jobs = []
+        for dec, grp in ((self.decoder_density, self._grouped()), (self.decoder_color, None), (self.decoder_semantics, self._pan_grouped()),
+                         (self.decoder_inst, self._inst_grouped())):
+            if dec.images is None or not dec.lout.weight.is_cuda:
+                continue
+            W = self._wide_head_weights(dec, dec.lout.weight)[0] if dec is self.decoder_inst else dec.weights()[0]
+            jobs.append((dec.images, W, dec.input_dim, grp))
+        if jobs:
+            ops.pack_weight_images(jobs)
+
     def _wide_head_requested(self, channels):
         return any(dec.hidden_dim == 128 for ch, dec in (("semantics", self.decoder_semantics), ("inst_embedding", self.decoder_inst)) if ch in channels)
 
@@ -338,8 +357,10 @@
         if cache is not None and cache[0] is coords:
             feats = cache[1]
         elif self._heads_read_live_features():
+            self.pack_weight_images()
             feats = self._interp(self.grid, coords)
         else:
+            self.pack_weight_images()
             with torch.no_grad():
                 feats = self._interp(self.grid, coords)
         (sem_in, sem_grp), (inst_in, inst_grp) = self._head_inputs(feats, coords, channels)
@@ -348,13 +369,14 @@
             heads = ((*self._wide_head_weights(self.decoder_inst, sem_in), self.decoder_inst.input_dim),
                      (*self.decoder_semantics.weights(), self.decoder_semantics.input_dim))
             out["inst_embedding"], out["semantics"] = ops.head_composite_pair(sem_in, heads, w, alpha, ridx, pack_start, ray_of_pack, N,
-                                                                              out_dtype=self.feat_dtype, x1_grouped=sem_grp)
+                                                                              out_dtype=self.feat_dtype, x1_grouped=sem_grp,
+                                                                              images=(self.decoder_inst.images, self.decoder_semantics.images))
             return out
         for ch, dec, x, grp in (("semantics", self.decoder_semantics, sem_in, sem_grp), ("inst_embedding", self.decoder_inst, inst_in, inst_grp)):
             if ch in channels:
                 W, b = self._wide_head_weights(dec, x) if ch == "inst_embedding" else dec.weights()
                 out[ch] = ops.head_composite(x, W, b, w, alpha, ridx, pack_start, ray_of_pack, N, in_dim=dec.input_dim,
-                                             out_act=L.ACT_SOFTMAX, out_dtype=self.feat_dtype, x1_grouped=grp)
+                                             out_act=L.ACT_SOFTMAX, out_dtype=self.feat_dtype, x1_grouped=grp, images=dec.images)
         return out
 
     @torch.no_grad()
@@ -399,6 +421,9 @@
     def _pan_grouped(self):
         return self._grouped()
 
+    def _inst_grouped(self):
+        return None if self.inst_direct_pos else self._grouped()
+
     def _heads_read_live_features(self):
         return not (self.sem_detach and (self.inst_detach or self.inst_direct_pos))
 
diff --git a/pagnerf_amd/ops.py b/pagnerf_amd/ops.py
--- a/pagnerf_amd/ops.py
+++ b/pagnerf_amd/ops.py
@@ -27,8 +27,11 @@
     return {k: [a.elapsed_time(b) for a, b in v] for k, v in (prof or {}).items()}
 
 
+_PACKED_FORM = {("pag_mlp_fwd", 5): "pag_mlp_fwd_packed", ("pag_mlp_bwd", 5): "pag_mlp_bwd_packed"}
+
+
 def _call(name, *args):
-    fn = getattr(L.load(), name)
+    fn = getattr(L.load(), _PACKED_FORM.get((name, len(args)), name))
     if _PROFILE is None or (_PROFILE_ONLY is not None and name not in _PROFILE_ONLY):
         L.check(fn(*args), name)
         return
@@ -306,14 +309,14 @@
 
 
 class _Launch:
-    __slots__ = ("entry", "bare", "args", "M", "keep", "taken", "fused", "out_ptr")
+    __slots__ = ("entry", "bare", "args", "M", "keep", "taken", "fused", "out_ptr", "images")
 
     def __init__(self, entry, bare=False):
         self.entry, self.bare = entry, bare
-        self.args, self.M, self.keep, self.taken, self.fused, self.out_ptr = None, 0, (), False, False, 0
-
-    def park(self, args, M, keep, fused=False, out_ptr=0):
-        self.args, self.M, self.keep, self.fused, self.out_ptr = args, M, keep, fused, out_ptr
+        self.args, self.M, self.keep, self.taken, self.fused, self.out_ptr, self.images = None, 0, (), False, False, 0, None
+
+    def park(self, args, M, keep, fused=False, out_ptr=0, images=None):
+        self.args, self.M, self.keep, self.fused, self.out_ptr, self.images = args, M, keep, fused, out_ptr, images
 
     @property
     def pending(self):
@@ -321,25 +324,33 @@
 
     def issue(self):
         if self.pending:
-            _call(self.entry, ctypes.byref(self.args), self.M, L.stream())
+            _decoder_call(self.entry, self.args, self.images, None, self.M)
             self.taken = True
+
+
+def _decoder_call(entry, args, images, rider_images, M):
+    if images or rider_images:
+        _call(entry, ctypes.byref(args), images, rider_images, M, L.stream())
+    else:
+        _call(entry, ctypes.byref(args), M, L.stream())
 
 
 class _DecoderCall:
     __slots__ = ("in_dim", "out_act", "mode", "out_dtype", "grouped", "x2_packs", "need_grad", "col0_relu", "rank1", "stats_only", "composite", "park",
-                 "pair", "producer", "n_rays")
+                 "pair", "producer", "n_rays", "images")
 
     def __init__(self, in_dim, out_act, mode, out_dtype, grouped, x2_packs=None, need_grad=False, col0_relu=False, rank1=False, stats_only=False,
-                 composite=None, park=None, pair=None, producer=None, n_rays=0):
+                 composite=None, park=None, pair=None, producer=None, n_rays=0, images=None):
         self.in_dim, self.out_act, self.mode, self.out_dtype = int(in_dim), out_act, mode, out_dtype
         self.grouped = grouped if grouped is None else tuple(grouped)
         self.x2_packs, self.need_grad, self.col0_relu, self.rank1, self.stats_only = x2_packs, need_grad, col0_relu, rank1, stats_only
         self.composite, self.park, self.pair, self.producer, self.n_rays = composite, park, pair, producer, n_rays
+        self.images = images
 
 
 class _DecoderState:
     __slots__ = ("in_dim", "out_act", "mode", "out_dtype", "grouped", "x2_packs", "needs", "M", "k1", "n_layers", "n_hidden", "has_stats", "bc", "saved",
-                 "col0_relu", "composited", "head", "hc", "x1_shape", "x1_dtype")
+                 "col0_relu", "composited", "head", "hc", "x1_shape", "x1_dtype", "images")
 
     def __init__(self, call, needs, M, k1, n_layers, saved, x1):
         self.in_dim, self.out_act, self.mode, self.out_dtype, self.grouped = call.in_dim, call.out_act, call.mode, call.out_dtype, call.grouped
@@ -352,6 +363,7 @@
         self.composited = False
         self.head = None
         self.hc = None
+        self.images = None
 
 
 def _save(ctx, st):
@@ -394,6 +406,106 @@
         a.W[i] = L.ptr(w)
     for i, v in enumerate(b):
         a.b[i] = L.ptr(v)
+
+
+WEIGHT_IMAGES = os.environ.get("PAG_WEIGHT_IMAGES", "1") != "0"
+
+
+def _swap23(a):
+    return (a & ~12) | ((a & 4) << 1) | ((a & 8) >> 1)
+
+
+def weight_image_layout(n_layers, out_dim):
+    ob = (out_dim + 31) // 32
+    layers, off = [], 0
+    for l in range(n_layers):
+        last = l == n_layers - 1
+        s_rows, t_stride = (ob * 32, ob * 32 + 8) if last else (64, 72)
+        layers.append((off, s_rows, 72, off + s_rows * 72, t_stride))
+        off += s_rows * 72 + 64 * t_stride
+    return layers, off
+
+
+def weight_images_reference(weights, in_dim, grouped=None):
+    import numpy as np
+    Ws = [np.asarray(w, dtype=np.float32) for w in weights]
+    layers, total = weight_image_layout(len(Ws), Ws[-1].shape[0])
+    img = np.zeros(total, np.float32)
+    for l, (W, (s_off, s_rows, s_stride, t_off, t_stride)) in enumerate(zip(Ws, layers)):
+        n_out, n_in = W.shape[0], (in_dim if l == 0 else 64)
+        cols = xcd8_columns(*grouped) if (l == 0 and grouped is not None) else list(range(64))
+        for o in range(n_out):
+            for k in range(64):
+                c = cols[k]
+                if 0 <= c < n_in:
+                    img[s_off + o * s_stride + (k if l == 0 else _swap23(k))] = W[o, c]
+                    img[t_off + k * t_stride + _swap23(o)] = W[o, c]
+    return img
+
+
+class WeightImages:
+
+    def __init__(self):
+        self.buf = None
+        self.shape = None
+        self.built = None
+        self.captured = False
+
+    def __getstate__(self):
+        return {}
+
+    def __setstate__(self, state):
+        self.__init__()
+
+    def serves(self, n_layers, in_dim, out_dim, grouped, Wc):
+        if self.built is None or self.shape != (n_layers, in_dim, out_dim, grouped) or len(Wc) != len(self.built):
+            return False
+        if any(w.data_ptr() != b[0] or w._version != b[1] for w, b in zip(Wc, self.built)):
+            return False
+        return self.captured or not torch.cuda.is_current_stream_capturing()
+
+
+def pack_weight_images(images):
+    if not WEIGHT_IMAGES:
+        return
+    capturing = torch.cuda.is_current_stream_capturing()
+    jobs, keep = [], []
+    for im, weights, in_dim, grouped in images:
+        if not (weights[0].is_cuda and 2 <= len(weights) <= 3 and all(w.shape == (o, i) for w, o, i in zip(
+                weights, [64] * (len(weights) - 1) + [weights[-1].shape[0]], [in_dim] + [64] * (len(weights) - 1)))):
+            im.built = None
+            continue
+        if not (1 <= in_dim <= 64 and 1 <= weights[-1].shape[0] <= 224) or \
+                (grouped is not None and (in_dim != grouped[0] * grouped[1] or not xcd8_supported(*grouped))):
+            im.built = None
+            continue
+        key = tuple((w.data_ptr(), w._version) for w in weights)
+        shape = (len(weights), int(in_dim), int(weights[-1].shape[0]), None if grouped is None else tuple(grouped))
+        if not capturing and im.built == key and im.shape == shape and im.buf is not None and im.buf.device == weights[0].device:
+            continue
+        Wc = [w.detach().contiguous().float() for w in weights]
+        if any(c.data_ptr() != w.data_ptr() for c, w in zip(Wc, weights)):
+            im.built = None
+            continue
+        need = L.load().pag_mlp_weight_images_bytes(shape[0], shape[2])
+        if im.buf is None or im.buf.numel() * 2 != need or im.buf.device != Wc[0].device:
+            if capturing and im.buf is not None:
+                raise RuntimeError("pagnerf_amd: a decoder's weight-image block changed size inside a stream capture")
+            im.buf = torch.empty(need // 2, device=Wc[0].device, dtype=torch.bfloat16)
+        im.shape, im.built, im.captured = shape, key, capturing
+        jobs.append((im, Wc))
+        keep.append(Wc)
+    for c0 in range(0, len(jobs), 8):
+        part = jobs[c0:c0 + 8]
+        arr = (L.MlpWeightImages * len(part))()
+        for d, (im, Wc) in zip(arr, part):
+            for i, w in enumerate(Wc):
+                d.W[i] = L.ptr(w)
+            d.n_layers, d.in_dim, d.out_dim = im.shape[:3]
+            if im.shape[3] is not None:
+                d.x1_layout, d.x1_levels, d.x1_feats = L.LAYOUT_XCD8, im.shape[3][0], im.shape[3][1]
+            d.image = L.ptr(im.buf)
+        _call("pag_mlp_pack_weights", arr, len(part), L.stream())
 
 
 def _dx2(x2, x2_index, x2_packs, dz0, w_tail, seg=None):
@@ -493,6 +605,10 @@
     stats = torch.empty(M, 2, device=dev) if has_stats else None
     a.softmax_stats = L.ptr(stats)
     st = _DecoderState(call, needs, M, k1, n_layers, (x1, x2, x2_index, out, *hidden, *Wc, *((stats, bc[-1]) if has_stats else ())), x1)
+    images, img, rider = call.images, None, None
+    if images is not None and mfma and images.serves(n_layers, in_dim, out_dim, grouped, Wc):
+        img = L.ptr(images.buf)
+        st.images = images
     st.n_hidden, st.has_stats, st.bc = len(hidden), has_stats, bc
     if col0:
         st.col0_relu = torch.empty(M, device=dev)
@@ -507,20 +623,20 @@
         if producer.pending and M and x1.data_ptr() == producer.out_ptr \
                 and lib.pag_mlp_fwd_producer_supported(ctypes.byref(a), ctypes.byref(producer.args), M) == 1:
             a.x1_producer = ctypes.pointer(producer.args)
-            producer.taken = True
+            producer.taken, rider = True, producer.images
         else:
             producer.issue()
     if M and park is not None:
-        park.park(a, M, [x1, x2, x2_index, out, stats, st.col0_relu, *hidden, *Wc, *bc], out_ptr=out.data_ptr() if out is not None else 0)
+        park.park(a, M, [x1, x2, x2_index, out, stats, st.col0_relu, *hidden, *Wc, *bc], out_ptr=out.data_ptr() if out is not None else 0, images=img)
     elif M:
         pair = call.pair
         if pair is not None and pair.pending and M <= L.MLP_FUSED_WIDE_MAX_M and lib.pag_mlp_fwd_pair_supported(ctypes.byref(a), ctypes.byref(pair.args)) == 1:
             a.pair = ctypes.pointer(pair.args)
-            pair.taken = True
+            pair.taken, rider = True, pair.images
         if call.composite is not None and HEAD_FWD_ONCE and stats_only and lib.pag_mlp_fwd_composite_supported(ctypes.byref(a), M) == 1:
             a.composite = ctypes.pointer(call.composite)
             st.composited = True
-        _call("pag_mlp_fwd", ctypes.byref(a), M, L.stream())
+        _decoder_call("pag_mlp_fwd", a, img, rider, M)
     return out, st
 
 
@@ -547,6 +663,9 @@
     _fill_shape(a, k1, in_dim, out_dim, out_act, out_dtype, grouped)
     _fill_operands(a, W=Wc, b=st.bc)
     a.out, a.n_layers, a.mode = L.ptr(out), n_layers, mode
+    img = rider = None
+    if st.images is not None and st.images.serves(n_layers, in_dim, out_dim, grouped, Wc):
+        img = L.ptr(st.images.buf)
     a.dx1, a.dx1_dtype = L.ptr(dx1), (L.dtype_code(dx1) if need_dx else 0)
     a.softmax_stats, a.b_last = L.ptr(stats), L.ptr(b_last)
     a.dx1_accumulate = 1 if (need_dx and dx1_into is not None) else 0
@@ -591,12 +710,12 @@
             a.dz[i] = L.ptr(dz[i])
     if M and hold is not None:
         hold.park(a, M, [x1, x2, x2_index, out, stats, b_last, g, dx1, col0_add, col0_gate, dz0_slots, dz0_fused, ws, *(rank1 or ()), *hidden, *Wc, *gW,
-                         *gb, *(dz or ())], fused=fused)
+                         *gb, *(dz or ())], fused=fused, images=img)
     elif M:
         if pair is not None and fused and pair.pending and pair.fused and lib.pag_mlp_bwd_pair_supported(ctypes.byref(a), ctypes.byref(pair.args)) == 1:
             a.pair = ctypes.pointer(pair.args)
-            pair.taken = True
-        _call("pag_mlp_bwd", ctypes.byref(a), M, L.stream())
+            pair.taken, rider = True, pair.images
+        _decoder_call("pag_mlp_bwd", a, img, rider, M)
     if col0_add is not None and need_dx and not fuse_col0:
         dx1[:, 0] += col0_add.to(dx1.dtype)
     if fused:
@@ -752,18 +871,18 @@
 
 
 def colour_and_density(x1, weights, biases, x2, x2_index, in_dim, out_act=L.ACT_SIGMOID, mode=L.MLP_MFMA_BF16,
-                       out_dtype=torch.float32, x2_packs=None, producer=None):
+                       out_dtype=torch.float32, x2_packs=None, producer=None, images=None):
     call = _DecoderCall(in_dim, out_act, mode, out_dtype, None, x2_packs=x2_packs, need_grad=_need_grad(x1, x2, x2_index, *weights, *biases),
-                        col0_relu=True, producer=producer)
+                        col0_relu=True, producer=producer, images=images)
     return _apply(_ColourDensity, call, x1, x2, x2_index, *weights, *biases)
 
 
 def fused_mlp(x1, weights, biases, x2=None, x2_index=None, in_dim=None, out_act=L.ACT_NONE, mode=L.MLP_MFMA_BF16,
-              out_dtype=torch.float32, x1_grouped=None, x2_packs=None, hold=None):
+              out_dtype=torch.float32, x1_grouped=None, x2_packs=None, hold=None, images=None):
     if in_dim is None:
         in_dim = weights[0].shape[1]
     call = _DecoderCall(in_dim, out_act, mode, out_dtype, x1_grouped, x2_packs=x2_packs, need_grad=_need_grad(x1, x2, x2_index, *weights, *biases),
-                        park=hold)
+                        park=hold, images=images)
     return _apply(_FusedMLP, call, x1, x2, x2_index, *weights, *biases)
 
 
@@ -1552,20 +1671,21 @@
         return (None, dx1, None, None, None, None, None, *gW_a, *gb_a, *gW_b, *gb_b)
 
 
-def head_composite_pair(x1, heads, w, alpha, ridx, pack_start, ray_of_pack, N, out_dtype=torch.bfloat16, x1_grouped=None):
+def head_composite_pair(x1, heads, w, alpha, ridx, pack_start, ray_of_pack, N, out_dtype=torch.bfloat16, x1_grouped=None, images=(None, None)):
     (wa, ba, ia), (wb_, bb, ib) = heads
     need_grad = _need_grad(x1, w, alpha, ridx, pack_start, ray_of_pack, *wa, *ba, *wb_, *bb)
     parked = _Launch("pag_mlp_fwd")
-    calls = (_head_call(ia, L.ACT_SOFTMAX, out_dtype, x1_grouped, need_grad, n_rays=N, pair=parked),
-             _head_call(ib, L.ACT_SOFTMAX, out_dtype, x1_grouped, need_grad, n_rays=N, park=parked), len(wa) + len(ba))
+    calls = (_head_call(ia, L.ACT_SOFTMAX, out_dtype, x1_grouped, need_grad, n_rays=N, pair=parked, images=images[0]),
+             _head_call(ib, L.ACT_SOFTMAX, out_dtype, x1_grouped, need_grad, n_rays=N, park=parked, images=images[1]), len(wa) + len(ba))
     return _apply(_HeadCompositePair, calls, x1, w, alpha, ridx, pack_start, ray_of_pack, *wa, *ba, *wb_, *bb)
 
 
 def head_composite(x1, weights, biases, w, alpha, ridx, pack_start, ray_of_pack, N, in_dim=None, out_act=L.ACT_NONE,
-                   out_dtype=torch.bfloat16, x1_grouped=None):
+                   out_dtype=torch.bfloat16, x1_grouped=None, images=None):
     if in_dim is None:
         in_dim = weights[0].shape[1]
-    call = _head_call(in_dim, out_act, out_dtype, x1_grouped, _need_grad(x1, w, alpha, ridx, pack_start, ray_of_pack, *weights, *biases), n_rays=N)
+    call = _head_call(in_dim, out_act, out_dtype, x1_grouped, _need_grad(x1, w, alpha, ridx, pack_start, ray_of_pack, *weights, *biases), n_rays=N,
+                      images=images)
     return _apply(_HeadComposite, call, x1, w, alpha, ridx, pack_start, ray_of_pack, *weights, *biases)
 
 
diff --git a/pagnerf_amd/optim.py b/pagnerf_amd/optim.py
--- a/pagnerf_amd/optim.py
+++ b/pagnerf_amd/optim.py
@@ -109,6 +109,7 @@
                     self._launch(plan, sel(plan.pp, ctypes.c_void_p), sel(plan.gg, ctypes.c_void_p), sel(plan.mm, ctypes.c_void_p),
                                  sel(plan.vv, ctypes.c_void_p), sel(plan.nn, ctypes.c_int64), n, hyper, count)
             torch._foreach_add_(plan.steps, 1)
+            torch.autograd.graph.increment_version(plan.params)
         if fallback:
             self._torch_step(fallback)
         return loss
```
